# do-mpc/do-mpc

Hardware: AMD Instinct MI355X
Metric: MPC steps/sec (make_step wall-time), industrial_poly robust multi-stage (higher is better)
Workload: dtype f64

## Files before the change

do_mpc_amd/csrc/dompc_driver.h:

```cpp

DOMPC_DEV inline int epsg_off(const KArgs& A) { return A.node_eps_off[0]; }
DOMPC_DEV inline int epsg_n(const KArgs& A) { return A.n_opt_x - A.node_eps_off[0]; }
DOMPC_DEV inline void epsg_grad(const Thr& T, const Prob& Q) {
  const KArgs& A = *Q.A;
  const int o = epsg_off(A), nv = epsg_n(A);
  for (int j = T.tid; j < nv; j += T.nt) {
    double g = 0.0, r = 0.0;
    for (int e = 0; e < A.n_edges; ++e) {
      const int q = j - (A.node_eps_off[A.edge_parent[e]] - o);
      if (q < 0 || q >= NSE) continue;
      g += Q.sf * DOMPC_EPS_PEN[q];
      const double* yd = Q.lam + A.edge_row0[e] + NW + NX;
      for (int i = 0; i < NE; ++i)
        if (nl_slack(i) == q) r -= yd[i] * Q.sgn[e * NE1 + i];
    }
    Q.gf[o + j] = g;
    Q.rd[o + j] = g + r - Q.zl[o + j] + Q.zu[o + j];
  }
  T.sync();
}
DOMPC_DEV inline double epsg_rowsum(const Prob& Q, int j, const double* v, const double* v0) {
  const KArgs& A = *Q.A;
  const int o = epsg_off(A);
  double t = 0.0;
  for (int e = 0; e < A.n_edges; ++e) {
    const int q = j - (A.node_eps_off[A.edge_parent[e]] - o);
    if (q < 0 || q >= NSE) continue;
    const int r0 = A.edge_row0[e] + NW + NX;
    for (int i = 0; i < NE; ++i)
      if (nl_slack(i) == q) t += (v[r0 + i] - (v0 ? v0[r0 + i] : 0.0)) * Q.sgn[e * NE1 + i];
  }
  return t;
}
DOMPC_DEV inline void epsg_residual(const Thr& T, const Prob& Q, const double* v, int j1) {
  const KArgs& A = *Q.A;
  const int o = epsg_off(A);
  for (int e = T.tid; e < A.n_edges; e += T.nt) {
    const int jo = A.node_eps_off[A.edge_parent[e]] - o;
    const int r0 = A.edge_row0[e] + NW + NX;
    for (int i = 0; i < NE; ++i) {
      const int q = nl_slack(i);
      if (q < 0) continue;
      const double ve = v ? v[jo + q] : ((jo + q == j1) ? 1.0 : 0.0);
      Q.c[r0 + i] = Q.ct[r0 + i] - ve * Q.sgn[e * NE1 + i];
    }
  }
  T.sync();
}

DOMPC_DEV inline void solve_problem(const Thr& T, const KArgs& A, int b, int slot) {
  const dompc_options& O = A.opt;
  Prob Q = make_prob(A, slot, A.p + (int64_t)b * A.n_opt_p);
  const double* x0 = A.x0 + (int64_t)b * A.n_opt_x;
  const int nX = A.n_opt_x, nSl = A.n_edges * NE;
  int status = 2, it = 0, n_reg = 0, n_ls_fail = 0, n_sweeps = 0, n_trials = 0, n_soc = 0;

  double cnt[2] = {0.0, 0.0};
  bool singular0;
  {
    double fr[1] = {0.0};
    for (int d = T.tid; d < A.n_dummy; d += T.nt) {
      const int g = A.dummy_idx[d];
      if (!(A.lbx[g] > -INFINITY) && !(A.ubx[g] < INFINITY)) fr[0] += 1.0;
    }
    const int ops[1] = {R_SUM};
    wg_reduce(T, fr, ops);
    singular0 = fr[0] > 0.0;
  }
  for (int g = T.tid; g < nX; g += T.nt) {
    double l = A.lbx[g], u = A.ubx[g];
    if (l > -INFINITY) l -= fmin(O.constr_viol_tol, O.bound_relax_factor * fmax(1.0, fabs(l)));
    if (u < INFINITY) u += fmin(O.constr_viol_tol, O.bound_relax_factor * fmax(1.0, fabs(u)));
    double xv = x0[g];
    const bool hl = l > -INFINITY, hu = u < INFINITY;
    double pl = hl ? O.bound_push * fmax(1.0, fabs(l)) : 0.0;
    double pu = hu ? O.bound_push * fmax(1.0, fabs(u)) : 0.0;
    if (hl && hu) { pl = fmin(pl, O.bound_frac * (u - l)); pu = fmin(pu, O.bound_frac * (u - l)); }
    if (hl) xv = fmax(xv, l + pl);
    if (hu) xv = fmin(xv, u - pu);
    Q.lb_own[g] = l; Q.ub_own[g] = u; Q.x[g] = xv;
    Q.zl[g] = hl ? 1.0 : 0.0; Q.zu[g] = hu ? 1.0 : 0.0;
    if (sh_cnt(A, mk_x(A, g))) cnt[0] += (hl ? 1.0 : 0.0) + (hu ? 1.0 : 0.0);
  }
  for (int r = T.tid; r < A.n_g; r += T.nt) Q.lam[r] = 0.0;
  T.sync();
  for (int d = T.tid; d < A.n_dummy; d += T.nt) {
    const int g = A.dummy_idx[d];
    if (singular0) continue;
    if (sh_cnt(A, mk_x(A, g))) cnt[0] -= (Q.lb_own[g] > -INFINITY ? 1.0 : 0.0) + (Q.ub_own[g] < INFINITY ? 1.0 : 0.0);
    Q.x[g] = fmin(fmax(x0[g], A.lbx[g]), A.ubx[g]);
    Q.lb_own[g] = -INFINITY; Q.ub_own[g] = INFINITY; Q.zl[g] = 0.0; Q.zu[g] = 0.0;
  }
  T.sync();
  if (A.lb_sh) {
    for (int g = T.tid; g < nX; g += T.nt) { A.lb_sh[g] = Q.lb_own[g]; A.ub_sh[g] = Q.ub_own[g]; }
    T.sync();
  }
  auto init_slacks = [&](bool rescale) {
    for (int e = T.tid; e < A.n_edges; e += T.nt) {
      for (int i = 0; i < NE; ++i) { Q.s[e * NE1 + i] = 0.0; if (!rescale) Q.sgn[e * NE1 + i] = 1.0; }
      if (DENSE_EDGE) dae_edge_f(Q, e, Q.x, Q.s, Q.ct); else eval_edge_f(Q, e, Q.x, Q.s, Q.ct);
      for (int i = 0; i < NE; ++i) {
        const int row = A.edge_row0[e] + NW + NX + i, si = e * NE1 + i;
        double l = A.lbg[row], u = A.ubg[row];
        if (l > -INFINITY) l -= fmin(O.constr_viol_tol, O.bound_relax_factor * fmax(1.0, fabs(l)));
        if (u < INFINITY) u += fmin(O.constr_viol_tol, O.bound_relax_factor * fmax(1.0, fabs(u)));
        l *= Q.sgn[si]; u *= Q.sgn[si];
        const bool hl = l > -INFINITY, hu = u < INFINITY;
        double pl = hl ? O.bound_push * fmax(1.0, fabs(l)) : 0.0;
        double pu = hu ? O.bound_push * fmax(1.0, fabs(u)) : 0.0;
        if (hl && hu) { pl = fmin(pl, O.bound_frac * (u - l)); pu = fmin(pu, O.bound_frac * (u - l)); }
        double sv = Q.ct[row];
        if (hl) sv = fmax(sv, l + pl);
        if (hu) sv = fmin(sv, u - pu);
        Q.s[si] = sv; Q.sl[si] = l; Q.su[si] = u;
        Q.zsl[si] = hl ? 1.0 : 0.0; Q.zsu[si] = hu ? 1.0 : 0.0;
        if (!rescale && sh_cnt(A, mk_e(A, e))) cnt[1] += (hl ? 1.0 : 0.0) + (hu ? 1.0 : 0.0);
      }
    }
    T.sync();
  };
  if (NE > 0) init_slacks(false);
  {
    const int ops[2] = {R_SUM, R_SUM};
    wg_reduce(T, cnt, ops);
  }
  const double n_bounds = cnt[0] + cnt[1];
  const double n_dual = (double)(A.n_g - DOMPC_XROW_MASKED) + n_bounds;

  double mu = O.mu_init;
  Q.sf = 1.0;
  long long c_sweep = 0, c_bwd = 0, c_fwd = 0, c_ls = 0, c_meas = 0, c_ftb = 0, c_acc = 0, c_t = 0; const long long c_start = prof_clock();
  unsigned g_sweep = 0, g_bwd = 0, g_fwd = 0, g_ls = 0, g_meas = 0, g_ftb = 0, g_acc = 0, g_t = 0; const unsigned g_start = T.gen;
  if (T.tid == 0) T.fset(6, abort_requested(A));
  auto delta_after = [&](double last) { return last == 0.0 ? O.delta_w_0 : fmax(O.delta_w_min, O.kappa_w_minus * last); };
  const bool ls_init = NE == 0 && O.constr_mult_init_max > 0.0;
  if (ls_init) {
    for (int g = T.tid; g < nX; g += T.nt) {
      if (Q.lb_own[g] > -INFINITY) Q.lb_own[g] = Q.x[g] - 1.0;
      if (Q.ub_own[g] < INFINITY) Q.ub_own[g] = Q.x[g] + 1.0;
      Q.zl[g] = 0.0; Q.zu[g] = 0.0;
    }
    for (int r = T.tid; r < A.n_g; r += T.nt) Q.c[r] = 0.0;
    T.sync();
  }
  auto first_sweep = [&]() {
    ++n_sweeps;
    const int rc = ls_init ? run_sweep(T, Q, b, slot, 1.0, 3, 1.0) : run_sweep(T, Q, b, slot, mu, 0, singular0 ? delta_after(0.0) : 0.0);
    if (EPS_GLOBAL) epsg_grad(T, Q);
    return rc;
  };
  auto epsg_build = [&](double delta) -> int {
    const int o = epsg_off(A), nv = epsg_n(A);
    double* G = Q.gsc;
    for (int g = T.tid; g < A.n_g; g += T.nt) { Q.dlam_e[g] = Q.dlam[g]; Q.ct[g] = Q.c[g]; }
    T.sync();
    int rc = 0;
    for (int j = 0; j < nv && !rc; ++j) {
      epsg_residual(T, Q, nullptr, j);
      ++n_sweeps;
      rc = run_sweep(T, Q, b, slot, mu, 1, delta);
      if (!rc) rc = run_backward(T, Q, b, slot, mu, delta);
      if (!rc) {
        run_forward(T, Q, b, slot, mu, delta);
        for (int jp = T.tid; jp < nv; jp += T.nt) G[jp * NVG_MAX + j] = -epsg_rowsum(Q, jp, Q.dlam, Q.dlam_e);
      }
    }
    epsg_residual(T, Q, nullptr, -1);
    if (T.tid == 0) {
      int ok = rc ? 0 : 1;
      for (int j = 0; j < nv && ok; ++j) {
        const int g = o + j;
        G[j * NVG_MAX + j] += sigma_of(Q.x[g], Q.lb[g], Q.ub[g], Q.zl[g], Q.zu[g]) + delta;
      }
      for (int j = 0; j < nv && ok; ++j) {
        double dj = G[j * NVG_MAX + j];
        for (int k = 0; k < j; ++k) dj -= G[j * NVG_MAX + k] * G[j * NVG_MAX + k];
        if (!(dj > 0.0)) { ok = 0; break; }
        dj = sqrt(dj);
        G[j * NVG_MAX + j] = dj;
        for (int i = j + 1; i < nv; ++i) {
          double t = 0.5 * (G[i * NVG_MAX + j] + G[j * NVG_MAX + i]);
          for (int k = 0; k < j; ++k) t -= G[i * NVG_MAX + k] * G[j * NVG_MAX + k];
          G[i * NVG_MAX + j] = t / dj;
        }
      }
      G[NVG_MAX * NVG_MAX] = ok ? 0.0 : 1.0;
    }
    T.sync();
    return G[NVG_MAX * NVG_MAX] != 0.0;
  };
  auto epsg_apply = [&](double delta, const double* dl) -> int {
    const int o = epsg_off(A), nv = epsg_n(A);
    double* G = Q.gsc;
    double* de = G + NVG_MAX * NVG_MAX + 1;
    for (int j = T.tid; j < nv; j += T.nt) {
      const int g = o + j;
      const double re = Q.rd[g] + Q.zl[g] - Q.zu[g] + bar_grad(Q.x[g], Q.lb[g], Q.ub[g], mu);
      de[j] = -re + epsg_rowsum(Q, j, dl, nullptr);
    }
    for (int g = T.tid; g < A.n_g; g += T.nt) Q.ct[g] = Q.c[g];
    T.sync();
    if (T.tid == 0) {
      for (int i = 0; i < nv; ++i) {
        double t = de[i];
        for (int k = 0; k < i; ++k) t -= G[i * NVG_MAX + k] * de[k];
        de[i] = t / G[i * NVG_MAX + i];
      }
      for (int i = nv - 1; i >= 0; --i) {
        double t = de[i];
        for (int k = i + 1; k < nv; ++k) t -= G[k * NVG_MAX + i] * de[k];
        de[i] = t / G[i * NVG_MAX + i];
      }
    }
    T.sync();
    epsg_residual(T, Q, de, -1);
    ++n_sweeps;
    int rc = run_sweep(T, Q, b, slot, mu, 1, delta);
    if (!rc) rc = run_backward(T, Q, b, slot, mu, delta);
    if (!rc) run_forward(T, Q, b, slot, mu, delta);
    epsg_residual(T, Q, nullptr, -1);
    for (int j = T.tid; j < nv; j += T.nt) Q.dx[o + j] = de[j];
    T.sync();
    return rc;
  };
  int bad = first_sweep();
  if (NE > 0 && O.obj_scaling && !bad) {
    double any[1] = {0.0};
    for (int e = T.tid; e < A.n_edges; e += T.nt) {
      if (!mk_e(A, e)) continue;
      for (int i = 0; i < NE; ++i) {
        double gm = nl_slack(i) >= 0 ? 1.0 : 0.0;
        for (int a = 0; a < NA; ++a) gm = fmax(gm, fabs(Q.EW(e, EW_JD + i * NA + a)));
        if (DENSE_EDGE) for (int c = 0; c < NW; ++c) gm = fmax(gm, fabs(Q.EW(e, EW_JDW + i * NW + c)));
        if (gm > O.nlp_scaling_max_gradient) { Q.sgn[e * NE1 + i] = fmax(O.nlp_scaling_max_gradient / gm, 1e-8); any[0] = 1.0; }
      }
    }
    const int ops[1] = {R_MAX};
    wg_reduce(T, any, ops);
    if (any[0] > 0.0) {
      T.sync();
      init_slacks(true);
      bad = first_sweep();
    }
  }
  if (O.obj_scaling) {
    double gm[1] = {0.0};
    for (int g = T.tid; g < nX; g += T.nt)
      if (sh_cnt(A, mk_x(A, g))) gm[0] = fmax(gm[0], fabs(Q.gf[g]));
    const int ops[1] = {R_MAX};
    wg_reduce(T, gm, ops);
    if (gm[0] > O.nlp_scaling_max_gradient) {
      Q.sf = fmax(O.nlp_scaling_max_gradient / gm[0], 1e-8);
      bad = first_sweep();
    }
  }
  if (ls_init) {
    int ls_bad = bad;
    if (!ls_bad) ls_bad = run_backward(T, Q, b, slot, 1.0, 1.0, 2);
    if (!ls_bad) run_forward(T, Q, b, slot, 1.0, 1.0);
    double ym[1] = {0.0};
    for (int r = T.tid; r < A.n_g; r += T.nt) {
      if (!mk_g(A, r)) continue;
      const double y = Q.dlam[r];
      ym[0] = fmax(ym[0], (y == y) ? fabs(y) : INFINITY);
    }
    {
      const int ops[1] = {R_MAX};
      wg_reduce(T, ym, ops);
// ... 8 lines not shown
      Q.zl[g] = hl ? 1.0 : 0.0; Q.zu[g] = hu ? 1.0 : 0.0;
    }
    T.sync();
    bad = run_sweep(T, Q, b, slot, mu, 0, singular0 ? delta_after(0.0) : 0.0);
    ++n_sweeps;
  }
  const double mu_min = fmin(O.tol, O.compl_inf_tol * Q.sf) / (O.kappa_eps + 1.0);
  double tau = fmax(O.tau_min, 1.0 - mu);
  if (KAPPA_D != 0.0) Q.mu = mu;
  Errs E = measure(T, Q, nullptr);
  const double theta0 = E.theta;
  const double theta_max = 1e4 * fmax(1.0, theta0), theta_min = 1e-4 * fmax(1.0, theta0);
  double bar_sum;
  {
    double bs[1] = {0.0};
    LogAcc La{1.0, 0, 0};
    double lin = 0.0;
    double x_[DOMPC_FW], l_[DOMPC_FW], u2_[DOMPC_FW];
#define L_(u, g) x_[u] = Q.x[g]; l_[u] = Q.lb[g]; u2_[u] = Q.ub[g];
#define B_(u, g)                                                       \
    if (sh_cnt(A, mk_x(A, g))) {                                       \
      if (l_[u] > -INFINITY) logacc_add(La, x_[u] - l_[u]);            \
      if (u2_[u] < INFINITY) logacc_add(La, u2_[u] - x_[u]);           \
      if (KAPPA_D != 0.0) { const double os_ = one_sided(l_[u], u2_[u]); lin += os_ > 0.0 ? x_[u] - l_[u] : (os_ < 0.0 ? u2_[u] - x_[u] : 0.0); } \
    }
    DOMPC_FOR4(nX, L_, B_)
#undef L_
#undef B_
    for (int g = T.tid; g < nSl; g += T.nt) {
      if (!sh_cnt(A, mk_e(A, g / NE1))) continue;
      const int si = (g / NE1) * NE1 + g % NE1;
      if (Q.sl[si] > -INFINITY) logacc_add(La, Q.s[si] - Q.sl[si]);
      if (Q.su[si] < INFINITY) logacc_add(La, Q.su[si] - Q.s[si]);
      if (KAPPA_D != 0.0) { const double os_ = one_sided(Q.sl[si], Q.su[si]); lin += os_ > 0.0 ? Q.s[si] - Q.sl[si] : (os_ < 0.0 ? Q.su[si] - Q.s[si] : 0.0); }
    }
    bs[0] = -logacc_value(La);
    if (KAPPA_D != 0.0) bs[0] += KAPPA_D * lin;
    const int ops[1] = {R_SUM};
    wg_reduce(T, bs, ops);
    bar_sum = bs[0];
  }
  int n_filt = 0;
  double delta_last = 0.0;
  int acc_count = 0;
  const double s_max = 100.0;
  double E0 = 0.0;
  int wd_count = 0, wd_iter = 0, n_watchdog = 0;
  bool in_wd = false, wd_resume = false;
  double wd_theta = 0.0, wd_phi = 0.0, wd_dphi = 0.0, wd_alpha = 0.0, wd_amax = 0.0, wd_az = 0.0, wd_delta = 0.0, wd_delta_last = 0.0, wd_bar = 0.0;
  Errs wd_E = E;
  double delta = 0.0, a_max = 1.0, a_z = 1.0, dphi = 0.0;

  while (true) {
    bool skip_first = false;
    if (wd_resume) {
      for (int g = T.tid; g < nX; g += T.nt) { Q.x[g] = Q.x_wd[g]; Q.zl[g] = Q.zl_wd[g]; Q.zu[g] = Q.zu_wd[g]; Q.dx[g] = Q.dx_sv[g]; }
      for (int g = T.tid; g < A.n_g; g += T.nt) { Q.lam[g] = Q.lam_wd[g]; Q.dlam[g] = Q.dlam_sv[g]; }
      for (int g = T.tid; g < nSl; g += T.nt) { Q.s[g] = Q.s_wd[g]; Q.zsl[g] = Q.zsl_wd[g]; Q.zsu[g] = Q.zsu_wd[g]; Q.ds[g] = Q.ds_sv[g]; }
      T.sync();
      E = wd_E; bar_sum = wd_bar; delta = wd_delta; delta_last = wd_delta_last; a_max = wd_amax; a_z = wd_az; dphi = wd_dphi;
      wd_resume = false;
      skip_first = true;
    } else {
    if (bad) { if (in_wd) { bad = 0; wd_resume = true; in_wd = false; wd_count = 0; continue; } status = 3; break; }
    if (T.fget(6)) { status = 6; break; }
    if (((WIDE_OK && T.nwg > 1) || sh_on(A)) && T.fget(7)) { status = 5; break; }
    const double sd = fmax(s_max, (E.sum_y + E.C.sum_z) / fmax(1.0, n_dual)) / s_max;
    const double sc = fmax(s_max, E.C.sum_z / fmax(1.0, n_bounds)) / s_max;
    const double e_c0 = comp_err(E.C, 0.0);
    E0 = fmax(E.e_d / sd, fmax(E.e_p, e_c0 / sc));
    if (!(E0 == E0) || !(E.obj == E.obj)) { if (in_wd) { wd_resume = true; in_wd = false; wd_count = 0; continue; } status = 4; break; }
    if (E0 <= O.tol && E.e_d <= O.dual_inf_tol && E.e_p <= O.constr_viol_tol && e_c0 <= O.compl_inf_tol) {
      status = 0; break;
    }
    if (E0 <= O.acceptable_tol) {
      if (++acc_count >= O.acceptable_iter) { status = 1; break; }
    } else acc_count = 0;
    if (it >= O.max_iter) { status = 2; break; }

    const double mu_before = mu;
    while (true) {
      const double Emu = fmax(E.e_d / sd, fmax(E.e_p, comp_err(E.C, mu) / sc));
      if (Emu <= O.kappa_eps * mu && mu > mu_min) {
        mu = fmax(mu_min, fmin(O.kappa_mu * mu, pow(mu, O.theta_mu)));
        tau = fmax(O.tau_min, 1.0 - mu);
        n_filt = 0;
        in_wd = false; wd_count = 0;
      } else break;
    }
    if (mu != mu_before) {
      if (QUAD_FWD && forward_adjoint(Q, mu) && !Q.lu_ok) {
        ++n_sweeps;
        if (run_sweep(T, Q, b, slot, mu, 4, Q.dsw)) { if (in_wd) { wd_resume = true; in_wd = false; wd_count = 0; continue; } status = 3; break; }
      } else {
        refresh_mu(T, Q, mu - mu_before);
        Q.rp_mu = mu;
      }
    }

    delta = 0.0;
    bool first_try = true, dir_ok = true, recs_dirty = false;
    while (true) {
      c_t = prof_clock(); g_t = T.gen;
      int fail = (singular0 && delta == 0.0) ? 1 : run_backward(T, Q, b, slot, mu, delta);
      if (EPS_GLOBAL && !fail) {
        run_forward(T, Q, b, slot, mu, delta);
        fail = epsg_build(delta);
        recs_dirty = true;
      }
      c_bwd += prof_clock() - c_t; g_bwd += T.gen - g_t;
      if (!fail) break;
      if (delta == 0.0) {
        delta = delta_after(delta_last);
      } else {
        delta *= (delta_last == 0.0 && first_try) ? O.kappa_w_plus_bar : O.kappa_w_plus;
        first_try = false;
        if (delta > O.delta_w_max) { dir_ok = false; break; }
      }
      if ((NW > 0 && delta != Q.dsw) || (EPS_GLOBAL && recs_dirty)) {
        ++n_sweeps;
        if (run_sweep(T, Q, b, slot, mu, 0, delta)) { dir_ok = false; break; }
        recs_dirty = false;
      }
    }
    if (!dir_ok) { if (in_wd) { wd_resume = true; in_wd = false; wd_count = 0; continue; } status = 3; break; }
    if (delta > 0.0) { delta_last = delta; ++n_reg; }
    c_t = prof_clock(); g_t = T.gen;
    if (EPS_GLOBAL) { if (epsg_apply(delta, Q.dlam_e)) { if (in_wd) { wd_resume = true; in_wd = false; wd_count = 0; continue; } status = 3; break; } }
    else run_forward(T, Q, b, slot, mu, delta);
    c_fwd += prof_clock() - c_t; g_fwd += T.gen - g_t;

    c_t = prof_clock(); g_t = T.gen;
    double r5[5];
    run_step_rules(T, Q, b, slot, mu, r5);
    a_max = (r5[0] > tau) ? tau / r5[0] : 1.0; dphi = r5[2];
    a_z = (r5[1] > tau) ? tau / r5[1] : 1.0;
    c_ftb += prof_clock() - c_t; g_ftb += T.gen - g_t;
    }
    auto step_rules = [&](double (&r5)[5]) { run_step_rules(T, Q, b, slot, mu, r5); };
    const double theta = E.theta;
    const double phi = E.obj + mu * bar_sum;

    c_t = prof_clock(); g_t = T.gen;
    const double gamma_theta = 1e-5, gamma_phi = 1e-8, eta_phi = 1e-8, s_theta = 1.1, s_phi = 2.3, gamma_alpha = 0.05;
    const double kappa_soc = 0.99;
    double a_min;
    if (dphi < 0.0 && theta <= theta_min)
      a_min = (theta > 0.0) ? gamma_alpha * fmin(gamma_theta, fmin(gamma_phi * theta / (-dphi),
                                                                    pow(theta, s_theta) / pow(-dphi, s_phi)))
                            : gamma_alpha * gamma_theta;
    else if (dphi < 0.0) a_min = gamma_alpha * fmin(gamma_theta, gamma_phi * theta / (-dphi));
    else a_min = gamma_alpha * gamma_theta;
    a_min = fmax(a_min, 1e-14);
    auto eval_trial = [&](double al, double& obj_o, double& th_o, double& bar_o) {
      run_eval_trial(T, Q, b, slot, al, obj_o, th_o, bar_o);
      ++n_trials;
    };
    auto acceptable_ref = [&](double th_, double ph_, double al, bool& armijo_case, double theta, double phi, double dphi) -> bool {
      armijo_case = false;
      bool ok = (ph_ == ph_) && (th_ == th_) && fabs(ph_) < INFINITY && th_ <= theta_max;
      if (ok) {
        for (int q = 0; q < n_filt; ++q)
          if (th_ >= T.filt[2 * q] && ph_ >= T.filt[2 * q + 1]) { ok = false; break; }
      }
      if (ok) {
        const bool switching = dphi < 0.0 && al * pow(-dphi, s_phi) > pow(theta, s_theta);
        const double eps_m = 10.0 * 2.220446049250313e-16 * fabs(phi);
        if (theta <= theta_min && switching) {
          armijo_case = true;
          ok = (ph_ - phi - eps_m <= eta_phi * al * dphi);
        } else {
          ok = (th_ <= (1.0 - gamma_theta) * theta) || (ph_ - phi - eps_m <= -gamma_phi * theta);
        }
      }
      return ok;
    };
    auto acceptable = [&](double th_, double ph_, double al, bool& armijo_case) -> bool { return acceptable_ref(th_, ph_, al, armijo_case, theta, phi, dphi); };
    auto soc_residual = [&](double al) {
      double c_[DOMPC_FW], ct_[DOMPC_FW];
#define L_(u, g) c_[u] = Q.c[g]; ct_[u] = Q.ct[g];
#define B_(u, g) if (mk_g(A, g)) Q.c[g] = al * c_[u] + ct_[u];
      DOMPC_FOR4(A.n_g, L_, B_)
#undef L_
#undef B_
      T.sync();
    };
    auto keep_direction = [&](bool restore) {
      for (int g = T.tid; g < nX; g += T.nt) { if (restore) Q.dx[g] = Q.dx_sv[g]; else Q.dx_sv[g] = Q.dx[g]; }
      for (int g = T.tid; g < A.n_g; g += T.nt) { if (restore) Q.dlam[g] = Q.dlam_sv[g]; else Q.dlam_sv[g] = Q.dlam[g]; }
      for (int g = T.tid; g < nSl; g += T.nt) { if (restore) Q.ds[g] = Q.ds_sv[g]; else Q.ds_sv[g] = Q.ds[g]; }
      T.sync();
    };
    double alpha = skip_first ? 0.5 * a_max : a_max;
    bool accepted = false, armijo_used = false, stale = false;
    double th_t = 0.0, obj_t = 0.0, bar_t = bar_sum;
    int n_ls = skip_first ? 1 : 0;
    bool wd_done = false, wd_augment_ref = false, wd_no_augment = false;
    if (O.watchdog_shortened_iter_trigger > 0 && !in_wd && !skip_first && wd_count >= O.watchdog_shortened_iter_trigger) {
      in_wd = true; wd_iter = 0; ++n_watchdog;
      for (int g = T.tid; g < nX; g += T.nt) { Q.x_wd[g] = Q.x[g]; Q.zl_wd[g] = Q.zl[g]; Q.zu_wd[g] = Q.zu[g]; Q.dx_sv[g] = Q.dx[g]; }
      for (int g = T.tid; g < A.n_g; g += T.nt) { Q.lam_wd[g] = Q.lam[g]; Q.dlam_sv[g] = Q.dlam[g]; }
      for (int g = T.tid; g < nSl; g += T.nt) { Q.s_wd[g] = Q.s[g]; Q.zsl_wd[g] = Q.zsl[g]; Q.zsu_wd[g] = Q.zsu[g]; Q.ds_sv[g] = Q.ds[g]; }
      T.sync();
      wd_E = E; wd_bar = bar_sum; wd_delta = delta; wd_delta_last = delta_last; wd_amax = a_max; wd_az = a_z;
      wd_theta = theta; wd_phi = phi; wd_dphi = dphi; wd_alpha = a_max;
    }
    if (in_wd) {
      eval_trial(alpha, obj_t, th_t, bar_t);
      bool armijo_case = false;
      if (acceptable_ref(th_t, obj_t + mu * bar_t, wd_alpha, armijo_case, wd_theta, wd_phi, wd_dphi)) {
        accepted = true; armijo_used = armijo_case; wd_done = true; wd_augment_ref = true;
        in_wd = false; wd_count = 0;
      } else {
        ++wd_iter;
        const double ph_ = obj_t + mu * bar_t;
        if (wd_iter > O.watchdog_trial_iter_max || !(ph_ == ph_) || !(th_t == th_t) || !(fabs(ph_) < INFINITY)) {
          wd_resume = true; in_wd = false; wd_count = 0;
          continue;
        }
        accepted = true; wd_done = true; wd_no_augment = true;
      }
    }
    while (!wd_done) {
      eval_trial(alpha, obj_t, th_t, bar_t);
      stale = false;
      bool armijo_case = false;
      if (acceptable(th_t, obj_t + mu * bar_t, alpha, armijo_case)) { accepted = true; armijo_used = armijo_case; break; }
      if (n_ls == 0 && O.max_soc > 0 && th_t >= theta) {
        double th_old = theta;
        keep_direction(false);
        soc_residual(alpha);
        bool soc_ok = false;
        for (int k = 0; k < O.max_soc; ++k) {
          ++n_soc; ++n_sweeps;
          if (run_sweep(T, Q, b, slot, mu, 1, delta)) break;
          if (run_backward(T, Q, b, slot, mu, delta)) break;
          run_forward(T, Q, b, slot, mu, delta);
          if (EPS_GLOBAL && epsg_apply(delta, Q.dlam)) break;
          double q5[5];
          step_rules(q5);
          const double a_s = (q5[0] > tau) ? tau / q5[0] : 1.0;
          double obj_s = 0.0, th_s = 0.0, bar_s = 0.0;
          eval_trial(a_s, obj_s, th_s, bar_s);
          bool arm_s = false;
          if (acceptable(th_s, obj_s + mu * bar_s, a_s, arm_s)) {
            accepted = true; armijo_used = arm_s; soc_ok = true;
            alpha = a_s;
            a_z = (q5[1] > tau) ? tau / q5[1] : 1.0;
            obj_t = obj_s; th_t = th_s; bar_t = bar_s;
            break;
          }
          if (!(th_s <= kappa_soc * th_old)) break;
          th_old = th_s;
          soc_residual(a_s);
        }
        if (soc_ok) break;
        keep_direction(true);
        stale = true;
      }
      if (!(alpha * 0.5 >= a_min)) break;
      alpha *= 0.5;
      ++n_ls;
    }
    if (bad) { if (in_wd) { bad = 0; wd_resume = true; in_wd = false; wd_count = 0; continue; } status = 3; break; }
    if (!accepted && stale) eval_trial(alpha, obj_t, th_t, bar_t);
    if (!wd_done) wd_count = n_ls > 0 ? wd_count + 1 : 0;
    if (!accepted) {
      ++n_ls_fail;
      n_filt = 0;
    } else if (!armijo_used && !wd_no_augment) {
      if (T.ltid == 0) {
        int q = n_filt < MAX_FILTER ? n_filt : MAX_FILTER - 1;
        T.filt[2 * q] = (1.0 - gamma_theta) * (wd_augment_ref ? wd_theta : theta);
        T.filt[2 * q + 1] = (wd_augment_ref ? wd_phi : phi) - gamma_phi * (wd_augment_ref ? wd_theta : theta);
      }
      if (n_filt < MAX_FILTER) ++n_filt;
      T.lsync();
    }
    bar_sum = bar_t;
    c_ls += prof_clock() - c_t; g_ls += T.gen - g_t;
    c_t = prof_clock(); g_t = T.gen;
    const Comp Cp = run_accept(T, Q, b, slot, alpha, a_z, mu);
    if (A.trace && b == 0 && T.tid == 0 && it < A.trace_cap) {
      double* tr = A.trace + 8 * it;
      tr[0] = it; tr[1] = mu; tr[2] = E0; tr[3] = E.e_p; tr[4] = E.e_d; tr[5] = accepted ? alpha : -alpha;
      tr[6] = delta; tr[7] = E.obj / Q.sf;
    }
    if (T.tid == 0) T.fset(6, abort_requested(A));
    T.sync();
    c_acc += prof_clock() - c_t; g_acc += T.gen - g_t;
    ++it;
    c_t = prof_clock(); g_t = T.gen; bad = run_sweep(T, Q, b, slot, mu, 0, singular0 ? delta_after(delta_last) : 0.0); c_sweep += prof_clock() - c_t; g_sweep += T.gen - g_t;
    ++n_sweeps;
    if (EPS_GLOBAL) epsg_grad(T, Q);
    if (KAPPA_D != 0.0) Q.mu = mu;
    c_t = prof_clock(); g_t = T.gen; E = measure(T, Q, &Cp); c_meas += prof_clock() - c_t; g_meas += T.gen - g_t;
  }

  if (A.trace && b == 0 && T.tid == 0 && A.trace_cap > 8) { double* tr = A.trace + 8 * (A.trace_cap - 1); tr[0] = (double)c_sweep; tr[1] = (double)c_bwd; tr[2] = (double)c_fwd; tr[3] = (double)c_ls; tr[4] = (double)c_meas; tr[5] = (double)(prof_clock() - c_start); tr[6] = (double)c_ftb; tr[7] = (double)c_acc; if (T.prof) { double* t2 = A.trace + 8 * (A.trace_cap - 2); for (int i = 0; i < 8; ++i) t2[i] = (double)T.prof[i]; double* t3 = A.trace + 8 * (A.trace_cap - 3); for (int i = 0; i < 8; ++i) t3[i] = (double)T.prof[8 + i]; double* t4 = A.trace + 8 * (A.trace_cap - 4); for (int i = 0; i < 8; ++i) t4[i] = (double)T.prof[16 + i]; if (A.trace_cap > 12) { double* t5 = A.trace + 8 * (A.trace_cap - 5); for (int i = 0; i < 8; ++i) t5[i] = (double)T.prof[24 + i]; double* t6 = A.trace + 8 * (A.trace_cap - 6); t6[0] = g_sweep; t6[1] = g_bwd; t6[2] = g_fwd; t6[3] = g_ls; t6[4] = g_meas; t6[5] = T.gen - g_start; t6[6] = g_ftb; t6[7] = g_acc; } } }
  const double isf = 1.0 / Q.sf;
  if (A.x_out) for (int g = T.tid; g < nX; g += T.nt) A.x_out[(int64_t)b * nX + g] = sh_cnt(A, mk_x(A, g)) ? Q.x[g] : 0.0;
  if (A.lam_x_out) for (int g = T.tid; g < nX; g += T.nt) A.lam_x_out[(int64_t)b * nX + g] = sh_cnt(A, mk_x(A, g)) ? (Q.zu[g] - Q.zl[g]) * isf : 0.0;
  if (A.lam_g_out) for (int r = T.tid; r < A.n_g; r += T.nt) A.lam_g_out[(int64_t)b * A.n_g + r] = sh_cnt(A, mk_g(A, r)) ? Q.lam[r] * isf : 0.0;
  if (A.lam_g_out && NE > 0) {
    T.sync();
    for (int g = T.tid; g < nSl; g += T.nt) {
      const int e = g / NE1, i = g % NE1;
      if (!sh_cnt(A, mk_e(A, e))) continue;
      const int row = A.edge_row0[e] + NW + NX + i;
      A.lam_g_out[(int64_t)b * A.n_g + row] = Q.lam[row] * Q.sgn[e * NE1 + i] * isf;
    }
  }
  if (A.g_out) {
    for (int r = T.tid; r < A.n_g; r += T.nt) A.g_out[(int64_t)b * A.n_g + r] = sh_cnt(A, mk_g(A, r)) ? Q.c[r] : 0.0;
    T.sync();
    for (int g = T.tid; g < nSl; g += T.nt) {
      const int e = g / NE1, i = g % NE1;
      if (!sh_cnt(A, mk_e(A, e))) continue;
      const int row = A.edge_row0[e] + NW + NX + i;
      A.g_out[(int64_t)b * A.n_g + row] = (Q.c[row] + Q.s[e * NE1 + i]) / Q.sgn[e * NE1 + i];
    }
  }
  if (T.tid == 0) {
    if (A.f_out) A.f_out[b] = E.obj * isf;
    if (A.stats) {
      dompc_stats& S = A.stats[b];
      S.success = (status == 0 || status == 1) ? 1 : 0;
      S.status = status; S.iter_count = it; S.n_reg = n_reg; S.n_ls_fail = n_ls_fail; S.n_sweeps = n_sweeps; S.n_trials = n_trials; S.n_soc = n_soc; S.n_watchdog = n_watchdog; S.reserved0 = 0;
      S.mu = mu; S.obj = E.obj * isf; S.inf_pr = E.e_p; S.inf_du = E.e_d; S.inf_compl = comp_err(E.C, 0.0);
      S.obj_scaling = Q.sf; S.t_wall_total = 0.0;
    }
  }
  T.sync();
}

DOMPC_DEV inline void debug_newton(const Thr& T, const KArgs& A, int b = 0, int slot = 0) {
  const dompc_options& O = A.opt;
  Prob Q = make_prob(A, slot, A.p + (int64_t)b * A.n_opt_p);
  const int nX = A.n_opt_x;
  for (int g = T.tid; g < nX; g += T.nt) {
    Q.x[g] = A.x0[g]; Q.lb[g] = A.lbx[g]; Q.ub[g] = A.ubx[g];
    Q.zl[g] = A.dbg_zl[g]; Q.zu[g] = A.dbg_zu[g];
  }
  for (int r = T.tid; r < A.n_g; r += T.nt) Q.lam[r] = A.dbg_lam[r];
  T.sync();
  if (NE > 0) {
    for (int e = T.tid; e < A.n_edges; e += T.nt) {
      for (int i = 0; i < NE; ++i) { Q.s[e * NE1 + i] = 0.0; Q.sgn[e * NE1 + i] = 1.0; }
      if (DENSE_EDGE) dae_edge_f(Q, e, Q.x, Q.s, Q.ct); else eval_edge_f(Q, e, Q.x, Q.s, Q.ct);
      for (int i = 0; i < NE; ++i) {
        const int row = A.edge_row0[e] + NW + NX + i, si = e * NE1 + i;
        const double l = A.lbg[row], u = A.ubg[row];
        const bool hl = l > -INFINITY, hu = u < INFINITY;
        double pl = hl ? O.bound_push * fmax(1.0, fabs(l)) : 0.0;
        double pu = hu ? O.bound_push * fmax(1.0, fabs(u)) : 0.0;
        if (hl && hu) { pl = fmin(pl, O.bound_frac * (u - l)); pu = fmin(pu, O.bound_frac * (u - l)); }
        double sv = Q.ct[row];
        if (A.dbg_at_solution) {
          const double lr = hl ? l - fmin(O.constr_viol_tol, O.bound_relax_factor * fmax(1.0, fabs(l))) : l;
          const double ur = hu ? u + fmin(O.constr_viol_tol, O.bound_relax_factor * fmax(1.0, fabs(u))) : u;
          const double tiny = 1e-12 * fmax(1.0, fabs(sv));
          if (hl) sv = fmax(sv, lr + tiny);
          if (hu) sv = fmin(sv, ur - tiny);
          Q.s[si] = sv; Q.sl[si] = lr; Q.su[si] = ur;
          Q.zsl[si] = hl ? A.dbg_mu / (sv - lr) : 0.0; Q.zsu[si] = hu ? A.dbg_mu / (ur - sv) : 0.0;
          continue;
        }
        if (hl) sv = fmax(sv, l + pl);
        if (hu) sv = fmin(sv, u - pu);
        Q.s[si] = sv; Q.sl[si] = l; Q.su[si] = u;
        Q.zsl[si] = hl ? 1.0 : 0.0; Q.zsu[si] = hu ? 1.0 : 0.0;
      }
    }
    T.sync();
  }
  Q.sf = 1.0;
  run_sweep(T, Q, b, slot, A.dbg_mu, 0, A.dbg_delta);
  const int fail = run_backward(T, Q, b, slot, A.dbg_mu, A.dbg_delta);
  run_forward(T, Q, b, slot, A.dbg_mu, A.dbg_delta);
  for (int g = T.tid; g < nX; g += T.nt) {
    A.dbg_dx[(int64_t)b * nX + g] = fail ? NAN : Q.dx[g];
    A.dbg_rd[(int64_t)b * nX + g] = Q.rd[g];
  }
  for (int r = T.tid; r < A.n_g; r += T.nt) {
    A.dbg_dlam[(int64_t)b * A.n_g + r] = Q.dlam[r];
    A.dbg_c[(int64_t)b * A.n_g + r] = Q.c[r];
  }
  T.sync();
}

constexpr int SWEEP_BLOCK = NX * NA + NX + NA * NA + NA;

DOMPC_DEV inline void sweep_problem(const Thr& T, const KArgs& A, int b, int slot) {
  Prob Q = make_prob(A, slot, A.p + (int64_t)b * A.n_opt_p);
  const int nX = A.n_opt_x;
  const double* xin = A.sw_x + (int64_t)b * nX;
  const double* lin = A.sw_lam + (int64_t)b * A.n_g;
  for (int g = T.tid; g < nX; g += T.nt) {
    Q.x[g] = xin[g]; Q.lb[g] = -INFINITY; Q.ub[g] = INFINITY; Q.zl[g] = 0.0; Q.zu[g] = 0.0;
  }
  for (int r = T.tid; r < A.n_g; r += T.nt) Q.lam[r] = lin[r];
  for (int g = T.tid; g < A.n_edges * NE; g += T.nt) {
    const int si = (g / NE1) * NE1 + g % NE1;
    Q.s[si] = 0.0; Q.sl[si] = -INFINITY; Q.su[si] = INFINITY; Q.zsl[si] = 0.0; Q.zsu[si] = 0.0; Q.sgn[si] = 1.0;
  }
  T.sync();
  Q.sf = 1.0;
  run_sweep(T, Q, b, slot, 0.0);
  double* gout = A.sw_g + (int64_t)b * A.n_g;
  for (int r = T.tid; r < A.n_g; r += T.nt) gout[r] = Q.c[r];
  double* bl = A.sw_blocks + (int64_t)b * A.n_edges * SWEEP_BLOCK;
  for (int it = T.tid; A.sw_blocks && it < A.n_edges * SWEEP_BLOCK; it += T.nt) {
    const int e = it / SWEEP_BLOCK, i = it % SWEEP_BLOCK;
    const double* S_ = Q.ES(e);
    double v;
    if (i < NX * NA) v = S_[ES_AB + i];
    else if (i < NX * NA + NX) v = S_[ES_CV + i - NX * NA];
    else if (i < NX * NA + NX + NA * NA) v = S_[ES_QT + symi((i - NX * NA - NX) / NA, (i - NX * NA - NX) % NA, NA)];
    else v = S_[ES_QV + i - NX * NA - NX - NA * NA];
    bl[it] = v;
  }
  T.sync();
}
```

do_mpc_amd/csrc/dompc_factor.h:

```cpp

#ifndef DOMPC_HOST_EMU
#ifndef DOMPC_GJ_U
#define DOMPC_GJ_U 0.01
#endif
constexpr int GJ_R = DEG * NX, GJ_RP = ((GJ_R + 3) / 4) * 4, GJ_NRHS = NA + 1;
constexpr int GJ_NC = GJ_RP + GJ_NRHS + GJ_R;
constexpr bool MFMA_GJ = (NI == 1) && (DEG >= 1) && !DENSE_EDGE && (GJ_RP <= 32) && (GJ_NC <= 64);
constexpr int GJ_MT = (GJ_RP + 15) / 16, GJ_NT = (GJ_NC + 15) / 16;
static_assert(!MFMA_GJ || GJ_RP * 4 + 256 <= EL_T1 - EL_MX, "the panel buffer and the dual-residual row share the W | w0 region of the edge working set");

constexpr bool GJ_PACK = (GJ_MT == 2) && (GJ_RP == 20) && (GJ_NT <= 4);
constexpr int GJ_MTF = GJ_PACK ? 1 : GJ_MT;

struct GjCol { int kind, sl, b; };
__device__ inline GjCol gj_col(int ni, int lc) {
  constexpr int R = GJ_R, RP = GJ_RP, NRHS = GJ_NRHS;
  const int col = 16 * ni + lc;
  GjCol c{4, 0, 0};
  if (col < R) { c.kind = 0; c.sl = col / NX; c.b = col - c.sl * NX; }
  else if (col < RP) { c.kind = 4; c.b = col; }
  else if (col < RP + NA) { c.kind = 1; c.b = col - RP; }
  else if (col == RP + NA) { c.kind = 2; }
  else if (col < RP + NRHS + R) { c.kind = 3; c.b = col - (RP + NRHS); }
  return c;
// ... 270 lines not shown
        if (16 * mi + 4 * r < RP) put(16 * mi + 4 * r + lr, ni, T[mi][ni][r]);
    if constexpr (GJ_PACK) put(16 + lr, ni, X[ni]);
  }
  GJ_PH(27)
#undef GJ_PH
  return 0;
}
#else
constexpr bool MFMA_GJ = false;
DOMPC_DEV inline void gj_table_init(ldsd*, int) {}
#endif

constexpr int EF_R = DEG * NX, EF_NCX = 2 * EF_R + NA + 1, EF_CPX = (EF_NCX + GS_C - 1) / GS_C;
template <int MODE>
DOMPC_DEV inline int edge_factor_body(const Prob& Q, int e, double mu, int lane, int GS, ldsd* Ld, const double (&vx)[EF_CPX][5],
                                      const double (&ex)[5], double nu_a) {
  const KArgs& A = *Q.A;
  const int woff = A.edge_w_off[e];
  const double* nu_e = Q.lam + A.edge_row0[e] + NW;
  const double* mo = Q.MO(e);
  (void)mo;
  const ldsd* mol = Ld + EL_MOS;
#define MOV(i) (MO_COMPACT ? (double)mol[(i)] : mo[(i)])
  const bool act = true;
  int fail = 0;
  (void)act;
#if DOMPC_PROFILE && !defined(DOMPC_HOST_EMU)
  const long long pc_ef0 = clock64();
#endif
  constexpr int R = DEG * NX, RA = R > 0 ? R : 1;
  constexpr int NRHS = NA + 1;
  constexpr int NCX = 2 * R + NRHS;
  constexpr int CPX = (NCX + GS_C - 1) / GS_C;
  constexpr double GJ_U = DOMPC_GJ_U;
  double bc[CPX][RA];
  double cd[CPX][DEG > 0 ? DEG : 1];
  unsigned jcol_[CPX];
  auto fetch_cols = [&]() {
#pragma unroll
    for (int q = 0; q < CPX; ++q) {
      const unsigned cx = (unsigned)lane + (unsigned)q * (unsigned)GS;
      const bool isG = cx < (unsigned)R, isY = cx >= (unsigned)R && cx < (unsigned)(R + NA);
      const unsigned jcol = isG ? cx % (unsigned)NX : (isY ? cx - (unsigned)R : 0u);
      const unsigned sl1 = isG ? cx / (unsigned)NX + 1u : 0u;
      jcol_[q] = jcol;
#if !defined(DOMPC_HOST_EMU)
#pragma unroll
      for (int jj = 0; jj < DEG; ++jj) {
        double v = DOMPC_C[jj + 1];
        asm("" : "+v"(v));
#pragma unroll
        for (int s1 = 1; s1 <= DEG; ++s1) {
          double t = DOMPC_C[s1 * (DEG + 1) + jj + 1];
          asm("" : "+v"(t));
          v = (sl1 == (unsigned)s1) ? t : v;
        }
        cd[q][jj] = v;
      }
#else
#pragma unroll
      for (int jj = 0; jj < DEG; ++jj) cd[q][jj] = DOMPC_C[sl1 * (unsigned)(DEG + 1) + (unsigned)(jj + 1)];
#endif
    }
  };
  auto build_cols = [&]() {
#pragma unroll
    for (int q = 0; q < CPX; ++q) {
      const int cx = lane + q * GS;
      const bool isG = cx < R, isY = cx >= R && cx < R + NA, isR = cx == R + NA;
      const int sl = isG ? cx / NX : -1, b = isG ? cx % NX : -1, yb = isY ? cx - R : -1;
      const int unit_row = cx - (R + NRHS);
#pragma unroll
      for (int r = 0; r < R; ++r) {
        const int jj = r / NX, a = r % NX;
        const bool useJ = isG ? (sl == jj) : (isY && yb >= NX);
        const double jv_ = MOV((unsigned)(MO_PT + (r / NX) * PT_STRIDE + NX + (r % NX) * NA) + jcol_[q]);
        double v = useJ ? jv_ : 0.0;
        v -= (a == b) ? cd[q][jj] : 0.0;
        v -= (a == yb) ? DOMPC_C[0 * (DEG + 1) + (jj + 1)] : 0.0;
        v = (unit_row == r) ? 1.0 : v;
        bc[q][r] = v;
      }
      if (isR) {
#pragma unroll
        for (int r = 0; r < R; ++r) bc[q][r] = Ld[EL_T1 + r];
      }
    }
  };
  auto eliminate = [&](bool pivoting) -> int {
    int badl = 0;
#pragma unroll
    for (int kk = 0; kk < R; ++kk) {
      const int qk = kk / GS_C, lk = kk % GS_C;
      if (pivoting) {
        int pr = kk;
        double best = fabs(bc[qk][kk]);
#pragma unroll
        for (int r = kk + 1; r < R; ++r) {
          const double a = fabs(bc[qk][r]);
          if (a > best) { best = a; pr = r; }
        }
        if (lane == lk && !(best > 1e-300)) badl = 1;
#ifndef DOMPC_HOST_EMU
        pr = __builtin_amdgcn_readlane(pr, lk);
#endif
#pragma unroll
        for (int q = 0; q < CPX; ++q) {
          const double t = bc[q][kk];
          double nk = t;
#pragma unroll
          for (int r = kk + 1; r < R; ++r) {
            const bool hit = (r == pr);
            nk = hit ? bc[q][r] : nk;
            bc[q][r] = hit ? t : bc[q][r];
          }
          bc[q][kk] = nk;
        }
      } else {
        double m = 0.0;
#pragma unroll
        for (int r = kk + 1; r < R; ++r) m = fmax(m, fabs(bc[qk][r]));
        const double akk = fabs(bc[qk][kk]);
        if (lane == lk && !(akk >= GJ_U * m && akk > 1e-300)) badl = 1;
      }
      double f[RA];
#pragma unroll
      for (int r = 0; r < R; ++r) f[r] = lane_bcast(bc[qk][r], lk);
      const double pinv = fast_rcp((fabs(f[kk]) > 1e-300) ? f[kk] : 1.0);
#pragma unroll
      for (int q = 0; q < CPX; ++q) {
        const double prow = bc[q][kk] * pinv;
#pragma unroll
        for (int r = 0; r < R; ++r)
          if (r != kk) bc[q][r] = fma(-f[r], prow, bc[q][r]);
        bc[q][kk] = prow;
      }
    }
#ifndef DOMPC_HOST_EMU
    return __ballot(badl) != 0ull;
#else
    return badl;
#endif
  };
  if (MODE != 1) fetch_cols();
  auto dual_pieces = [&](auto col_dot) {
#pragma unroll
    for (int q = 0; q < CPX; ++q) {
      const int cx = lane + q * GS;
      double t = col_dot(q, cx);
      if (cx < R) {
        t -= DOMPC_D[cx / NX + 1] * Ld[EL_T0 + R + cx % NX];
        const int gi = woff + cx;
        const double xv = vx[q][0], l = vx[q][1], u = vx[q][2], zl_ = vx[q][3], zu_ = vx[q][4];
        Q.gf[gi] = 0.0;
        Q.rd[gi] = t - zl_ + zu_;
        Ld[EL_RW + cx] = t + bar_grad(xv, l, u, mu, !(Q.soc & 2));
        Ld[EL_BB + cx] = bar_grad(xv, l, u, 1.0);
        Ld[EL_SG + cx] = sigma_of(xv, l, u, zl_, zu_);
      } else if (cx < R + NA) {
        const int yb = cx - R;
        if (yb < NX) t -= DOMPC_D[0] * Ld[EL_T0 + R + yb];
        Ld[EL_RY + yb] = t;
      }
    }
    for (int a = lane; a < NX; a += GS) {
      const int col = R + a, gi = woff + col;
      const double t = Ld[EL_T0 + R + a] + (GS > 1 ? nu_a : nu_e[a]);
      double xv, l, u, zl_, zu_;
      if (GS > 1) { xv = ex[0]; l = ex[1]; u = ex[2]; zl_ = ex[3]; zu_ = ex[4]; }
      else { xv = Q.x[gi]; l = Q.lb[gi]; u = Q.ub[gi]; zl_ = Q.zl[gi]; zu_ = Q.zu[gi]; }
      Q.gf[gi] = 0.0;
      Q.rd[gi] = t - zl_ + zu_;
      Ld[EL_RW + col] = t + bar_grad(xv, l, u, mu, !(Q.soc & 2));
      Ld[EL_BB + col] = bar_grad(xv, l, u, 1.0);
      Ld[EL_SG + col] = sigma_of(xv, l, u, zl_, zu_);
    }
  };
  if (act && MODE == 0) {
    build_cols();
    dual_pieces([&](int q, int) {
      double t = 0.0;
#pragma unroll
      for (int r = 0; r < R; ++r) t += bc[q][r] * Ld[EL_T0 + r];
      return t;
    });
  }
#ifndef DOMPC_HOST_EMU
  if constexpr (MODE == 1) {
    __builtin_amdgcn_fence(__ATOMIC_ACQ_REL, "wavefront");
    __builtin_amdgcn_wave_barrier();
    if (edge_factor_mfma(Q, e, lane, Ld, [&](const ldsd* du) {
          dual_pieces([&](int, int cx) {
            const int c_ = cx < R ? cx : (cx < R + NA ? GJ_RP + (cx - R) : 0);
            return (double)du[c_] + (double)du[64 + c_] + (double)du[128 + c_] + (double)du[192 + c_];
          });
        })) return 2;
    {
      __builtin_amdgcn_fence(__ATOMIC_ACQ_REL, "wavefront");
      __builtin_amdgcn_wave_barrier();
      for (int it = lane; it < NX * NRHS; it += GS) {
        const int a_ = it / NRHS, c = it % NRHS;
        double t = (c == NA) ? -Ld[EL_T1 + R + a_] : ((c == a_) ? DOMPC_D[0] : 0.0);
#pragma unroll
        for (int s_ = 1; s_ <= DEG; ++s_) t += DOMPC_D[s_] * Ld[EL_MX + ((s_ - 1) * NX + a_) * MX_LD + MX_W + c];
        Ld[EL_MX + (R + a_) * MX_LD + MX_W + c] = t;
      }
      return 0;
    }
  } else if constexpr (MODE == 2) {
    build_cols();
    if (eliminate(true)) fail = 1;
  } else
#endif
  if (act) {
    if (eliminate(false)) {
      fetch_cols();
      build_cols();
      if (eliminate(true)) fail = 1;
    }
  }
  if (act) {
#pragma unroll
    for (int q = 0; q < CPX; ++q) {
      const int cx = lane + q * GS;
      if (cx >= R && cx < R + NRHS) {
        const int col = MX_W + (cx - R);
#pragma unroll
        for (int a_ = 0; a_ < NX; ++a_) {
          const int yb = cx - R;
          double t = (yb == NA) ? Ld[EL_T1 + R + a_] : ((yb == a_) ? -DOMPC_D[0] : 0.0);
#pragma unroll
          for (int r = 1; r <= DEG; ++r) t += DOMPC_D[r] * bc[q][(r - 1) * NX + a_];
          Ld[EL_MX + (R + a_) * MX_LD + col] = -t;
        }
#pragma unroll
        for (int r = 0; r < R; ++r) Ld[EL_MX + r * MX_LD + col] = -bc[q][r];
      } else if (cx >= R + NRHS && cx < NCX) {
        const int col = cx - (R + NRHS);
#pragma unroll
        for (int r = 0; r < R; ++r) Q.EW(e, EW_LU + r * LU_N + col) = bc[q][r];
      }
    }
  }
#undef MOV
  return fail;
}

#ifndef DOMPC_HOST_EMU
__device__ inline KArgs kernel_args(const void* kp);
#define DOMPC_EF_ARGS const void* kp, int slot, int e, int soc, double sf, double mu, double v0, double v1, double v2, double v3, double v4, \
                      double x0, double x1, double x2, double x3, double x4, double nu_a
#define DOMPC_EF_BODY(MODE_)                                                                                     \
  const KArgs A = kernel_args(kp);                                                                               \
  Prob Q = make_prob(A, __builtin_amdgcn_readfirstlane(slot), nullptr);                                          \
  Q.sf = ufl(sf);                                                                                                \
  Q.soc = __builtin_amdgcn_readfirstlane(soc);                                                                   \
  prob_bounds(Q);                                                                                                \
  const int lane = (int)(threadIdx.x & 63u);                                                                     \
  ldsd* Ld = (ldsd*)lds_pool + (int64_t)(threadIdx.x >> 6) * EL_SIZE;                                            \
  const double vx[EF_CPX][5] = {{v0, v1, v2, v3, v4}};                                                           \
  const double ex[5] = {x0, x1, x2, x3, x4};                                                                     \
  return edge_factor_body<MODE_>(Q, __builtin_amdgcn_readfirstlane(e), ufl(mu), lane, 64, Ld, vx, ex, nu_a);
__device__ __attribute__((noinline)) int phase_edge_factor(DOMPC_EF_ARGS) { DOMPC_EF_BODY(MFMA_GJ ? 1 : 0) }
__device__ __attribute__((noinline)) int phase_edge_factor_pivot(DOMPC_EF_ARGS) { DOMPC_EF_BODY(MFMA_GJ ? 2 : 0) }
#undef DOMPC_EF_BODY
#undef DOMPC_EF_ARGS
#endif
DOMPC_DEV inline int run_edge_factor(const Thr& T, const Prob& Q, int e, double mu, int lane, int GS, ldsd* Ld,
                                     const double (&vx)[EF_CPX][5], const double (&ex)[5], double nu_a) {
#ifndef DOMPC_HOST_EMU
  if constexpr (EF_CPX == 1) {
    (void)lane; (void)GS; (void)Ld;
    int rc = phase_edge_factor(T.kp, Q.slot, e, Q.soc, Q.sf, mu, vx[0][0], vx[0][1], vx[0][2], vx[0][3], vx[0][4],
                               ex[0], ex[1], ex[2], ex[3], ex[4], nu_a);
    if (MFMA_GJ && __builtin_amdgcn_readfirstlane(rc) == 2)
      rc = phase_edge_factor_pivot(T.kp, Q.slot, e, Q.soc, Q.sf, mu, vx[0][0], vx[0][1], vx[0][2], vx[0][3], vx[0][4],
                                   ex[0], ex[1], ex[2], ex[3], ex[4], nu_a);
    return rc;
  } else {
    return edge_factor_body<0>(Q, e, mu, lane, GS, Ld, vx, ex, nu_a);
  }
#else
  (void)T;
  return edge_factor_body<0>(Q, e, mu, lane, GS, Ld, vx, ex, nu_a);
#endif
}

#ifndef DOMPC_HOST_EMU
__device__ inline void stage_mo(const Prob& Q, int e, int lane, ldsd* Ld) {
  const double* src = Q.MO(e);
#pragma unroll
  for (int q = 0; q < MOC_STAGE / 128; ++q)
    __builtin_amdgcn_global_load_lds((const __attribute__((address_space(1))) void*)(src + 128 * q + 2 * lane),
                                     (__attribute__((address_space(3))) void*)(Ld + EL_MOC + 128 * q), 16, 0, 0);
}
#endif

DOMPC_PHASE int eval_edge_coop(const Thr& T, const Prob& Q, int e, int e_next, double mu, int lane, int GS, ldsd* Ld, int& staged_e, const MocMap& mm) {
  const KArgs& A = *Q.A;
  const bool act = e >= 0;
  const int ee = act ? e : 0;
  const auto* ep = A.edge_pack + ee * EP_N;
  const int n = ep[EP_PARENT], cn = ep[EP_CHILD], k = ep[EP_LEVEL];
  const double* xn = Q.x + ep[EP_XOFF_PARENT];
  const double* un = Q.x + ep[EP_UOFF_PARENT];
  const double* xc = Q.x + ep[EP_XOFF_CHILD];
  const int woff = ep[EP_WOFF];
  const int eps_off_n = ep[EP_EPSOFF_PARENT];
  const double* pp = Q.P + A.p_off_p + ep[EP_PIDX] * NP;
  const int row0 = ep[EP_ROW0];
  const double om = __builtin_bit_cast(double, ((unsigned long long)(unsigned)ep[EP_OMEGA_HI] << 32) | (unsigned long long)(unsigned)ep[EP_OMEGA_LO]) * Q.sf;
  (void)eps_off_n;
  const double* w = Q.x + woff;
  const double* tvp = Q.P + A.p_off_tvp + k * NTVP;
  const double omh = (Q.soc & 2) ? 0.0 : om;
  const double* lam_e = Q.lam + row0;
  const double* nu_e = Q.lam + row0 + NW;
  const double* yd = Q.lam + row0 + NW + NX;
  double* S_ = Q.ES(ee);
  const double* mo = Q.MO(ee);
  int fail = 0;
  constexpr bool PF = (NI == 1 && M > 0);
  constexpr int RPL = PF ? (NW + GS_C - 1) / GS_C : 1;
  constexpr int APL = PF ? (NA + GS_C - 1) / GS_C : 1, MHL = PF ? (NX * NX + GS_C - 1) / GS_C : 1;
// ... 112 lines not shown
        }
#endif
      }
      DOMPC_PH(4)
      if (act) {
        if constexpr (!TILE_CONDENSE)
          for (int it = lane; it < NCOLL * NA * NA; it += GS)
            Ld[EL_HP + it] = MOV(MO_PT + (it / (NA * NA)) * PT_STRIDE + NX + NX * NA + symi((it % (NA * NA)) / NA, it % NA, NA));
#pragma unroll
        for (int q = 0; q < RPL; ++q) {
          const int it = lane + q * GS;
          if (it < NW) {
            const int jj = it / NX;
            double res;
            if (jj < DEG) {
              const int j = jj + 1;
              double xp = DOMPC_C[0 * (DEG + 1) + j] * pf_xn[q];
#pragma unroll
              for (int r = 1; r <= DEG; ++r) xp += DOMPC_C[r * (DEG + 1) + j] * pf_w[q][r - 1];
              res = MOV(MO_PT + jj * PT_STRIDE + it % NX) - xp;
            } else {
              double xf = DOMPC_D[0] * pf_xn[q];
#pragma unroll
              for (int r = 1; r <= DEG; ++r) xf += DOMPC_D[r] * pf_w[q][r - 1];
              res = pf_wend[q] - xf;
            }
            if (Q.soc) res = pf_c[q];
            else Q.c[row0 + it] = res;
            Ld[EL_T1 + it] = res;
            Ld[EL_T0 + it] = pf_lam[q];
          }
          if (it < NX) {
            const double ce = Q.soc ? pf_cend[q] : pf_wend[q] - pf_xc[q];
            if (!Q.soc) Q.c[row0 + NW + it] = ce;
            Ld[EL_PV + it] = ce;
          }
        }
      }
      DOMPC_PH(5)
      T.gsync();
      DOMPC_PH(6)
      if (act) fail |= run_edge_factor(T, Q, e, mu, lane, GS, Ld, vx, ex, nu_a);
      T.gsync();
#ifndef DOMPC_HOST_EMU
      if (MO_LDS && e_next >= 0) { stage_mo(Q, e_next, lane, Ld); staged_e = e_next; }
#endif
    } else {
    if (act) {
#pragma unroll
      for (int q = 0; q < G_WPL; ++q) {
        const int col = lane + q * GS, gi = woff + (col < NW ? col : 0);
        gp_x[q] = Q.x[gi]; gp_l[q] = Q.lb[gi]; gp_u[q] = Q.ub[gi]; gp_zl[q] = Q.zl[gi]; gp_zu[q] = Q.zu[gi];
      }
#pragma unroll
      for (int q = 0; q < G_XPL; ++q) {
        const int a = lane + q * GS, ac = a < NX ? a : 0;
        gp_ce[q] = Q.soc ? Q.c[row0 + NW + ac] : w[(M - 1) * NX + ac] - xc[ac];
        gp_mg[q] = last_stage ? mo[MO_MT + 1 + ac] : 0.0;
      }
#pragma unroll
      for (int q = 0; q < G_CVL; ++q) {
        const int it = lane + q * GS, a = (it < NX * (NA + 1) ? it : 0) / (NA + 1);
        gp_cv[q] = Q.soc ? Q.c[row0 + NW + a] : w[(M - 1) * NX + a] - xc[a];
      }
#pragma unroll
      for (int q = 0; q < G_APL; ++q) {
        const int a = lane + q * GS;
        gp_ltg[q] = mo[MO_LT + 1 + (a < NA ? a : 0)];
      }
#pragma unroll
      for (int q = 0; q < G_MHL; ++q) {
        const int a = lane + q * GS, ac = a < NX * NX ? a : 0;
        gp_mh[q] = last_stage ? mo[MO_MT + 1 + NX + symi(ac / NX, ac % NX, NX)] : 0.0;
      }
#pragma unroll
      for (int q = 0; q < G_QPL; ++q) {
        const int it = lane + q * GS, itc = it < NA * NA ? it : 0;
        const int ip = symi(itc / NA, itc % NA, NA);
        gp_qlt[q] = mo[MO_LT + 1 + NA + ip];
        gp_qnl[q] = NE > 0 ? mo[MO_NL + NE + NE * NA + ip] : 0.0;
      }
      gp_lt0 = mo[MO_LT];
      gp_mt0 = last_stage ? mo[MO_MT] : 0.0;
    }
    if (act) {
      for (int it = lane; it < NCOLL * NA * NA; it += GS)
        Ld[EL_HP + it] = mo[MO_PT + (it / (NA * NA)) * PT_STRIDE + NX + NX * NA + symi((it % (NA * NA)) / NA, it % NA, NA)];
#pragma unroll
      for (int q2 = 0; q2 < G_RWL; ++q2) {
        const int it = lane + q2 * GS;
        gp_res[q2] = 0.0;
        if (it >= G_ROWS) continue;
        const int i = it / ((DEG + 1) * NX);
        const int rr = it % ((DEG + 1) * NX);
        const int jj = rr / NX, a = rr % NX;
        const double* xi0 = (i == 0) ? xn : w + slot_of(i, 0) * NX;
        const int row = i * (DEG + 1) * NX + jj * NX + a;
        ldsd* Mr = Ld + EL_MX + row * NC;
        if (jj < DEG) {
          const int j = jj + 1, sl = slot_of(i, j), p = i * DEG + jj;
          const double* pt = mo + MO_PT + p * PT_STRIDE;
          double xp = DOMPC_C[0 * (DEG + 1) + j] * xi0[a];
          for (int r = 1; r <= DEG; ++r) xp += DOMPC_C[r * (DEG + 1) + j] * w[slot_of(i, r) * NX + a];
          const double res = Q.soc ? Q.c[row0 + row] : pt[a] - xp;
          gp_res[q2] = res;
          Mr[NW + NA] = res;
          for (int b = 0; b < NX; ++b) Mr[sl * NX + b] += pt[NX + a * NA + b];
          for (int b = 0; b < NU; ++b) Mr[NW + NX + b] = pt[NX + a * NA + NX + b];
          for (int r = 0; r <= DEG; ++r) {
            const double cr = DOMPC_C[r * (DEG + 1) + j];
            if (i == 0 && r == 0) Mr[NW + a] -= cr;
            else Mr[slot_of(i, r) * NX + a] -= cr;
          }
        } else {
          const int ns_ = next_slot(i);
          double xf = DOMPC_D[0] * xi0[a];
          for (int r = 1; r <= DEG; ++r) xf += DOMPC_D[r] * w[slot_of(i, r) * NX + a];
          const double res = Q.soc ? Q.c[row0 + row] : w[ns_ * NX + a] - xf;
          gp_res[q2] = res;
          Mr[NW + NA] = res;
          Mr[ns_ * NX + a] += 1.0;
          for (int r = 0; r <= DEG; ++r) {
            if (i == 0 && r == 0) Mr[NW + a] -= DOMPC_D[0];
            else Mr[slot_of(i, r) * NX + a] -= DOMPC_D[r];
          }
        }
      }
    }
    T.gsync();
    if (act) {
#pragma unroll
      for (int q = 0; q < G_WPL; ++q) {
        const int col = lane + q * GS;
        if (col >= NW) continue;
        double t = 0.0;
#pragma unroll 6
        for (int r = 0; r < NW; ++r) t += Ld[EL_MX + r * NC + col] * Ld[EL_T0 + r];
        if (col >= (M - 1) * NX) t += nu_e[col - (M - 1) * NX];
        const double xv = gp_x[q], l = gp_l[q], u = gp_u[q];
        gp_x[q] = t - gp_zl[q] + gp_zu[q];
        Ld[EL_RW + col] = t + bar_grad(xv, l, u, mu, !(Q.soc & 2));
        Ld[EL_BB + col] = bar_grad(xv, l, u, 1.0);
        Ld[EL_SG + col] = sigma_of(xv, l, u, gp_zl[q], gp_zu[q]);
      }
      for (int b = lane; b < NA; b += GS) {
        double t = 0.0;
#pragma unroll 6
        for (int r = 0; r < NW; ++r) t += Ld[EL_MX + r * NC + NW + b] * Ld[EL_T0 + r];
        Ld[EL_RY + b] = t;
      }
#pragma unroll
      for (int q = 0; q < G_WPL; ++q) {
        const int col = lane + q * GS;
        if (col < NW) { Q.gf[woff + col] = 0.0; Q.rd[woff + col] = gp_x[q]; }
      }
      if (!Q.soc) {
#pragma unroll
        for (int q2 = 0; q2 < G_RWL; ++q2) {
          const int it = lane + q2 * GS;
          if (it < G_ROWS) Q.c[row0 + it] = gp_res[q2];
        }
#pragma unroll
        for (int q = 0; q < G_XPL; ++q) {
          const int a = lane + q * GS;
          if (a < NX) Q.c[row0 + NW + a] = gp_ce[q];
        }
      }
    }
    T.gsync();
    DOMPC_PH(1)
    bool gj_done = false;
#ifndef DOMPC_HOST_EMU
#ifndef DOMPC_REG_GJ
#define DOMPC_REG_GJ 1
#endif
    if constexpr ((DOMPC_REG_GJ != 0) && NC <= 64 && NW <= 40 && NW > NX) {
      if (GS == 64) {
        constexpr int GJ_STEPS = NW - NX;
        constexpr int EL_ROWS = (DEG + 1) * NX;
        const int cc_ = lane < NC ? lane : 0;
        double col[NW1];
#pragma unroll
        for (int r = 0; r < NW; ++r) col[r] = act ? Ld[EL_MX + r * NC + cc_] : 1.0;
        int bad = 0;
#pragma unroll
        for (int kk = 0; kk < GJ_STEPS; ++kk) {
          const int pos = kk % EL_ROWS;
          const int grp0 = kk - pos + (pos < DEG * NX ? 0 : DEG * NX);
          const int grp1 = kk - pos + (pos < DEG * NX ? DEG * NX : EL_ROWS);
          const int hi_ = pos < DEG * NX ? kk - pos + EL_ROWS : (kk - pos + 2 * EL_ROWS < NW ? kk - pos + 2 * EL_ROWS : NW);
          double f[NW1];
#pragma unroll
          for (int r = 0; r < NW; ++r) f[r] = (r >= grp0 && r < hi_) ? lane_bcast(col[r], kk) : 0.0;
          double m = 0.0;
#pragma unroll
          for (int r = 0; r < NW; ++r) if (r > kk && r < grp1) m = fmax(m, fabs(f[r]));
          const double akk = fabs(f[kk]);
          bad |= (int)!(akk >= DOMPC_GJ_U * m && akk > 1e-300);
          const double pinv = fast_rcp(akk > 1e-300 ? f[kk] : 1.0);
          const bool own = lane == kk;
          const double prow = own ? pinv : col[kk] * pinv;
#pragma unroll
          for (int r = 0; r < NW; ++r) if (r >= grp0 && r < hi_ && r != kk) col[r] = fma(-f[r], prow, own ? 0.0 : col[r]);
          col[kk] = prow;
        }
        if (!act) bad = 0;
        if (__builtin_amdgcn_readfirstlane(bad) == 0) {
          if (act && lane < NC) {
#pragma unroll
            for (int r = 0; r < NW; ++r) Ld[EL_MX + r * NC + lane] = col[r];
          }
          T.gsync();
          gj_done = true;
        }
      }
    }
#endif
    if (!gj_done) {
      static_assert(NW <= 128, "row index is packed into 7 bits of the pivot key / 128-bit used mask");
      constexpr int GJ_STEPS = NW - NX;
      constexpr int EL_ROWS = (DEG + 1) * NX;
      constexpr int CPL = (NC + GS_C - 1) / GS_C;
      unsigned long long used = 0ull, used_hi = 0ull;
      {
        for (int kk = 0; kk < GJ_STEPS; ++kk) {
          const int pos = kk % EL_ROWS;
          const int grp0 = kk - pos + (pos < DEG * NX ? 0 : DEG * NX);
          const int grp1 = kk - pos + (pos < DEG * NX ? DEG * NX : EL_ROWS);
          double f[NW1], bcol[CPL][NW1];
          unsigned bestkey = 0u;
          if (act) {
  #pragma unroll
            for (int r = 0; r < NW; ++r) f[r] = Ld[EL_MX + r * NC + kk];
  #pragma unroll
            for (int q = 0; q < CPL; ++q) {
              const int c = lane + q * GS;
              const int cc_ = c < NC ? c : 0;
  #pragma unroll
              for (int r = 0; r < NW; ++r) bcol[q][r] = Ld[EL_MX + r * NC + cc_];
            }
  #pragma unroll
            for (int r = 0; r < NW; ++r) {
              unsigned key = (((unsigned)(__builtin_bit_cast(unsigned long long, f[r]) >> 32)) & (NW > 64 ? 0x7fffff80u : 0x7fffffc0u)) | (unsigned)r;
              const bool taken = (r < 64) ? ((used >> (r & 63)) & 1ull) : ((used_hi >> (r & 63)) & 1ull);
              key = (r >= grp0 && r < grp1 && !taken) ? key : 0u;
              bestkey = key > bestkey ? key : bestkey;
            }
          }
          const int pv = (int)(bestkey & (NW > 64 ? 127u : 63u));
          if (pv < 64) used |= (1ull << pv); else used_hi |= (1ull << (pv - 64));
          if (act && (bestkey >> (NW > 64 ? 7 : 6)) == 0u) fail = 1;
          if (act) {
            if (lane == 0) Ld[EL_PV + kk] = (double)pv;
            const double piv = Ld[EL_MX + pv * NC + kk];
            const double pinv = (fabs(piv) > 1e-300) ? 1.0 / piv : 1.0;
  #pragma unroll
            for (int q = 0; q < CPL; ++q) {
              const int c = lane + q * GS;
              if (c < NC) {
                const double prow = (c == kk) ? pinv : Ld[EL_MX + pv * NC + c] * pinv;
                const double keep = (c == kk) ? 0.0 : 1.0;
  #pragma unroll
                for (int r = 0; r < NW; ++r) Ld[EL_MX + r * NC + c] = fma(-f[r], prow, bcol[q][r] * keep);
                Ld[EL_MX + pv * NC + c] = prow;
              }
            }
          }
          T.gsync();
        }
      }
      double tmp[CPL][NW1];
      if (act) {
        for (int k2 = GJ_STEPS + lane; k2 < NW; k2 += GS) Ld[EL_PV + k2] = (double)k2;
#pragma unroll
        for (int q = 0; q < CPL; ++q) {
          const int c = lane + q * GS;
          const int cc_ = c < NC ? c : 0;
#pragma unroll
          for (int r = 0; r < NW; ++r) tmp[q][r] = Ld[EL_MX + r * NC + cc_];
        }
      }
      T.gsync();
      if (act)
        for (int k2 = lane; k2 < NW; k2 += GS) Ld[EL_T0 + (int)Ld[EL_PV + k2]] = (double)k2;
      T.gsync();
      if (act) {
#pragma unroll
        for (int q = 0; q < CPL; ++q) {
          const int c = lane + q * GS;
          if (c < NC) {
            const int dst = (c < NW) ? (int)Ld[EL_PV + c] : c;
#pragma unroll
            for (int r = 0; r < NW; ++r) Ld[EL_MX + (int)Ld[EL_T0 + r] * NC + dst] = tmp[q][r];
          }
        }
      }
      T.gsync();
    }
    if (act) {
      for (int it = lane; it < NW * (NA + 1); it += GS) {
        const int r = it / (NA + 1), c = it % (NA + 1);
        Ld[EL_MX + r * NC + NW + c] = -Ld[EL_MX + r * NC + NW + c];
      }
    }
    T.gsync();
    }
    DOMPC_PH(2)
// ... 335 lines not shown
```

do_mpc_amd/csrc/dompc_kernel.h:

```cpp
#pragma once
#include <math.h>
#include <stdint.h>
#ifndef DOMPC_HOST_EMU
#include <utility>
#endif
#include "dompc_kargs.h"

namespace dompc {

#ifndef DOMPC_HOST_EMU
#define DOMPC_PHASE __device__ inline
#else
#define DOMPC_PHASE static inline
#endif

constexpr int NX = DOMPC_NX, NU = DOMPC_NU, NP = DOMPC_NP, NTVP = DOMPC_NTVP;
#ifndef DOMPC_EPS_GLOBAL
#define DOMPC_EPS_GLOBAL 0
#endif
constexpr bool EPS_GLOBAL = DOMPC_EPS_GLOBAL != 0 && DOMPC_NS > 0 && DOMPC_NE > 0;
constexpr int NS = EPS_GLOBAL ? 0 : DOMPC_NS;
constexpr int NSE = DOMPC_NS;
constexpr int NVG_MAX = 32;
constexpr int NZ = DOMPC_NZ;
constexpr int DEG = DOMPC_DEG, NI = DOMPC_NI, M = DOMPC_M;
#ifndef DOMPC_NL_COLLOC
#define DOMPC_NL_COLLOC 0
#endif
#ifndef DOMPC_FREE_ROOT
#define DOMPC_FREE_ROOT 0
#endif
#ifndef DOMPC_LT_END
#define DOMPC_LT_END 0
#endif
#ifndef DOMPC_NL_DUP
#define DOMPC_NL_DUP 0
#endif
#if !DOMPC_FREE_ROOT
DOMPC_FN double dompc_aterm_f(const double*, const double*, const double*, const double*) { return 0.0; }
DOMPC_FN void dompc_aterm(const double*, const double*, const double*, const double*, double*, double*, double*) {}
#endif
constexpr bool FREE_ROOT = DOMPC_FREE_ROOT != 0, LT_END = DOMPC_LT_END != 0 && M > 0;
constexpr int NEB = DOMPC_NE;
constexpr int NLP = (DOMPC_NL_COLLOC && M > 0) ? M : 1;
constexpr bool NL_DUP = DOMPC_NL_DUP != 0 && NEB > 0;
constexpr int NLB = NLP + (NL_DUP ? 1 : 0);
constexpr int NE = NEB * NLB;
constexpr bool NL_COLLOC = DOMPC_NL_COLLOC && M > 0 && NEB > 0;
DOMPC_HD constexpr int nl_pt(int blk) { return blk < NLP ? blk : NLP - 1; }
#ifndef DOMPC_FORCE_DENSE
#define DOMPC_FORCE_DENSE 0
#endif
constexpr bool DENSE_EDGE = DOMPC_NZ > 0 || NL_COLLOC || NL_DUP || LT_END || DOMPC_FORCE_DENSE;
DOMPC_HD inline int nl_slack(int i) { return DOMPC_NL_SLACK[NLB == 1 ? i : i % NEB]; }
constexpr int NA = NX + NU;
constexpr int NV = NU + NS;
constexpr int NYT = NA + NV;
constexpr int MZ = NZ > 0 ? (M > 0 ? M : 1) : 0;
constexpr int NWX = M * NX;
constexpr int NW = NWX + MZ * NZ;
constexpr bool RT_CUSTOM = DOMPC_RTERM_CUSTOM != 0;
constexpr int NR = NA + NU, NR_T = NR * (NR + 1) / 2;
constexpr int RT_LEN = RT_CUSTOM ? 1 + NR + NR_T : 0;
constexpr int NF = NX + NZ;
constexpr int NAV = NA + NZ;
constexpr int NCOLL = NI * DEG;
constexpr int RPE = NW + NX + NE;
constexpr int NE1 = NE > 0 ? NE : 1, NEB1 = NEB > 0 ? NEB : 1;
constexpr int NS1 = NS > 0 ? NS : 1;
constexpr int NW1 = NW > 0 ? NW : 1;
constexpr int MAX_FILTER = 48;
#ifndef DOMPC_SHARD
#define DOMPC_SHARD 0
#endif
#ifndef DOMPC_GJ_U
#define DOMPC_GJ_U 0.01
#endif
constexpr int RED_MAX = 12;
#ifndef DOMPC_HOST_EMU
constexpr int GS_C = 64;
#else
constexpr int GS_C = 1;
#endif

constexpr int LU_N = (NI == 1 && DEG > 0 && !DENSE_EDGE) ? DEG * NX : NW;
constexpr int EW_LU = 0;
constexpr int EW_SIGW = EW_LU + LU_N * LU_N;
constexpr int EW_RW = EW_SIGW + NW;
constexpr int EW_JD = EW_RW + NW;
constexpr int EW_W = EW_JD + NE * NA;
constexpr int EW_W0 = EW_W + (DENSE_EDGE ? NW * NA : 0);
constexpr int EW_HW = EW_W0 + (DENSE_EDGE ? NW : 0);
constexpr int EW_EWJ = EW_HW + (DENSE_EDGE ? NW * (NW + NA) : 0);
constexpr int EW_JDW = EW_EWJ + (DENSE_EDGE ? NX * NW : 0);
constexpr int EW_SIZE = ((EW_JDW + (DENSE_EDGE ? NE * NW : 0) + 1 + 7) / 8) * 8;

constexpr int ES_AB = 0;
constexpr int ES_CV = ES_AB + NX * NA;
constexpr int ES_QT = ES_CV + NX;
constexpr int ES_QV = ES_QT + NA * (NA + 1) / 2;
constexpr int ES_RY = ES_QV + NA;
constexpr int ES_GFY = ES_RY + NA;
constexpr int ES_QVB = ES_GFY + NA;
constexpr int ES_MG = ES_QVB + NA;
constexpr int ES_MH = ES_MG + NX;
constexpr int ES_SIGS = ES_MH + NX * NX;
constexpr int ES_RDN = ES_SIGS + NE;
constexpr int ES_RSN = ES_RDN + NE;
constexpr int ES_OBJ = ES_RSN + NE;
constexpr int ES_RTUP = ES_OBJ + 1;
constexpr int ES_RTH = ES_RTUP + (RT_CUSTOM ? NU : 0);
constexpr int ES_SIZE = ((ES_RTH + (RT_CUSTOM ? NR_T : 0) + 7) / 8) * 8;

constexpr int NA_T = NA * (NA + 1) / 2, NX_T = NX * (NX + 1) / 2, NAV_T = NAV * (NAV + 1) / 2;
DOMPC_HD constexpr int symi(int i, int j, int n) { return i <= j ? i * n - i * (i - 1) / 2 + j - i : j * n - j * (j - 1) / 2 + i - j; }
constexpr int PT_STRIDE = NF + NF * NAV + NAV_T;
constexpr int NPT_E = (M == 0) ? 1 : (DENSE_EDGE ? NI * (DEG + 1) : NI * DEG);
constexpr int MO_PT = 0;
constexpr int MO_LT = MO_PT + NPT_E * PT_STRIDE;
constexpr int MO_MT = MO_LT + 1 + NAV + NAV_T;
constexpr int MO_NL = MO_MT + 1 + NX + NX_T;
constexpr int NL_STRIDE = NEB + NEB * NAV + NAV_T;
constexpr int MO_SIZE = ((MO_NL + NLB * NL_STRIDE + 7) / 8) * 8;
constexpr bool MO_COMPACT = (NI == 1) && (M > 0) && !DENSE_EDGE;
constexpr int MOC_LT = NCOLL * DOMPC_DYN_NV;
constexpr int MOC_MT = MOC_LT + DOMPC_LT_NV;
constexpr int MOC_NL = MOC_MT + DOMPC_MT_NV;
constexpr int MOC_N = MOC_NL + DOMPC_NL_NV;
constexpr int MOC_SIZE = ((MOC_N + 7) / 8) * 8 > 0 ? ((MOC_N + 7) / 8) * 8 : 8;
constexpr int MO_REC = MO_COMPACT ? MOC_SIZE : MO_SIZE;

constexpr int ND_P = 0;
constexpr int ND_PV = ND_P + NA * NA;
constexpr int ND_K = ND_PV + NA;
constexpr int ND_KV = ND_K + NV * NA;
constexpr int ND_DXT = ND_KV + NV;
constexpr int ND_AT = ND_DXT + NA;
constexpr int AT_LEN = FREE_ROOT ? 1 + NX + NX * NX : 0;
constexpr int ND_SIZE = ((ND_AT + AT_LEN + 7) / 8) * 8;

struct WsLayout {
  int64_t x, zl, zu, lb, ub, dx, gf, rd, xt, dx_sv;
  int64_t lam, dlam, c, ct, dlam_sv;
  int64_t s, zsl, zsu, sl, su, ds, st, ds_sv;
  int64_t ew, es, nd, mo, gsc, total;
  int64_t x_wd, zl_wd, zu_wd, lam_wd, s_wd, zsl_wd, zsu_wd, dlam_e, sgn;
};

DOMPC_HD inline WsLayout ws_layout(int n_opt_x, int n_g, int n_edges, int e_pad, int n_nodes) {
  WsLayout L;
  int64_t o = 0;
  auto take = [&](int64_t n) { int64_t r = o; o += (n + 7) & ~int64_t(7); return r; };
  L.x = take(n_opt_x); L.zl = take(n_opt_x); L.zu = take(n_opt_x); L.lb = take(n_opt_x); L.ub = take(n_opt_x);
  L.dx = take(n_opt_x); L.gf = take(n_opt_x); L.rd = take(n_opt_x); L.xt = take(n_opt_x);
  L.dx_sv = take(n_opt_x);
  L.lam = take(n_g); L.dlam = take(n_g); L.c = take(n_g); L.ct = take(n_g); L.dlam_sv = take(n_g);
  int64_t nsl = (int64_t)n_edges * NE1;
  L.s = take(nsl); L.zsl = take(nsl); L.zsu = take(nsl); L.sl = take(nsl); L.su = take(nsl);
  L.ds = take(nsl); L.st = take(nsl); L.ds_sv = take(nsl);
  L.ew = take((int64_t)EW_SIZE * e_pad);
  L.es = take((int64_t)ES_SIZE * n_edges);
  L.nd = take((int64_t)ND_SIZE * n_nodes);
  L.mo = take((int64_t)MO_REC * n_edges);
  L.gsc = take(EPS_GLOBAL ? NVG_MAX * (NVG_MAX + 4) : 0);
  L.x_wd = take(n_opt_x); L.zl_wd = take(n_opt_x); L.zu_wd = take(n_opt_x); L.lam_wd = take(n_g);
  L.s_wd = take(nsl); L.zsl_wd = take(nsl); L.zsu_wd = take(nsl);
  L.dlam_e = take(EPS_GLOBAL ? n_g : 0);
  L.sgn = take(nsl);
  o += 256;
  L.total = o;
  return L;
}

#ifndef DOMPC_HOST_EMU
typedef __attribute__((address_space(3))) double ldsd;
#else
typedef double ldsd;
#endif

struct XCtx {
  int on, rank, world;
  double* xbuf;
  volatile uint32_t *req, *ack, *cnt;
  void (*cb)(void* ctx, double* buf, int32_t count);
  void* ctx;
};
DOMPC_HD inline XCtx make_xctx(const KArgs& A) {
  XCtx X;
  X.on = A.x_mask != nullptr; X.rank = A.shard_rank; X.world = A.shard_world; X.xbuf = A.xbuf;
  X.req = A.x_req; X.ack = A.x_ack; X.cnt = A.x_count; X.cb = A.x_callback; X.ctx = A.x_ctx;
  return X;
}

#ifndef DOMPC_NO_WIDE
#define DOMPC_NO_WIDE 0
#endif
constexpr bool WIDE_OK = DOMPC_NO_WIDE == 0;
#ifndef DOMPC_BLOCK_CONST
#define DOMPC_BLOCK_CONST 0
#endif
#if DOMPC_BLOCK_CONST
#define DOMPC_BDIM DOMPC_BLOCK_CONST
#else
#define DOMPC_BDIM ((int)blockDim.x)
#endif
struct Thr {
  int tid, nt;
  ldsd* red;
  ldsd* filt;
  int* flags;
  ldsd* edge_lds;
  long long* prof;
  int gs;
  int ltid, lnt;
  int wg, nwg;
  unsigned* bar;
  double* partials;
  mutable unsigned gen, nred;
  XCtx X;
  mutable unsigned xseq;
  const void* kp;
  mutable bool light = false;
  int pool = 0;
  DOMPC_DEV void fset(int i, int v) const {
#ifndef DOMPC_HOST_EMU
    if (WIDE_OK && nwg > 1) { __hip_atomic_store(flags + i, v, __ATOMIC_RELAXED, __HIP_MEMORY_SCOPE_AGENT); return; }
#endif
    flags[i] = v;
  }
  DOMPC_DEV int fget(int i) const {
#ifndef DOMPC_HOST_EMU
    if (WIDE_OK && nwg > 1) return __hip_atomic_load(flags + i, __ATOMIC_RELAXED, __HIP_MEMORY_SCOPE_AGENT);
#endif
    return flags[i];
  }
  DOMPC_DEV int flag_begin(int i) const {
    sync();
#ifndef DOMPC_HOST_EMU
    if (WIDE_OK && nwg > 1) return (int)(gen & 0x3fffffffu) + 1;
#endif
    if (tid == 0) fset(i, 0);
    sync();
    return 1;
  }
  DOMPC_DEV void sync() const {
#ifndef DOMPC_HOST_EMU
    if (WIDE_OK && nwg > 1) {
      asm volatile("s_waitcnt vmcnt(0)" ::: "memory");
      __syncthreads();
      ++gen;
      if (ltid == 0) {
        if (!light) __builtin_amdgcn_fence(__ATOMIC_RELEASE, "agent");
        asm volatile("s_waitcnt vmcnt(0)" ::: "memory");
        __hip_atomic_fetch_add(bar, 1u, __ATOMIC_RELAXED, __HIP_MEMORY_SCOPE_AGENT);
        const unsigned target = gen * (unsigned)nwg;
        long long spins = 0;
        while (__hip_atomic_load(bar, __ATOMIC_RELAXED, __HIP_MEMORY_SCOPE_AGENT) < target) {
          __builtin_amdgcn_s_sleep(4);
          if (++spins > 40000000ll || __hip_atomic_load(flags + 7, __ATOMIC_RELAXED, __HIP_MEMORY_SCOPE_AGENT)) {
            __hip_atomic_store(flags + 7, 1, __ATOMIC_RELAXED, __HIP_MEMORY_SCOPE_AGENT);
            break;
          }
        }
        __builtin_amdgcn_fence(__ATOMIC_ACQUIRE, "agent");
      }
      __syncthreads();
    } else {
      __syncthreads();
    }
#endif
  }
  DOMPC_DEV void lsync() const {
#ifndef DOMPC_HOST_EMU
    __syncthreads();
#endif
  }
  DOMPC_DEV void gsync() const {
#ifndef DOMPC_HOST_EMU
    __builtin_amdgcn_fence(__ATOMIC_ACQ_REL, "wavefront");
    __builtin_amdgcn_wave_barrier();
#endif
  }
  DOMPC_DEV void xchg(int off, int n) const {
#ifdef DOMPC_HOST_EMU
    if (X.cb) X.cb(X.ctx, X.xbuf + off, n);
#else
    sync();
    ++xseq;
    if (wg == 0 && ltid == 0) {
      __builtin_amdgcn_fence(__ATOMIC_RELEASE, "");
      X.cnt[0] = (unsigned)n;
      X.cnt[1] = (unsigned)off;
      __hip_atomic_store((unsigned*)X.req, xseq, __ATOMIC_RELEASE, __HIP_MEMORY_SCOPE_SYSTEM);
      long long spins = 0;
      const bool dead = __hip_atomic_load(flags + 7, __ATOMIC_RELAXED, __HIP_MEMORY_SCOPE_AGENT) != 0;
      while (!dead && __hip_atomic_load((unsigned*)X.ack, __ATOMIC_RELAXED, __HIP_MEMORY_SCOPE_SYSTEM) != xseq) {
        __builtin_amdgcn_s_sleep(16);
        if (++spins > 4000000ll) {
          __hip_atomic_store(flags + 7, 1, __ATOMIC_RELAXED, __HIP_MEMORY_SCOPE_AGENT);
          break;
        }
      }
      __builtin_amdgcn_fence(__ATOMIC_ACQUIRE, "");
    }
    sync();
#endif
  }
};

#ifndef DOMPC_HOST_EMU
extern __shared__ double lds_pool[];
__shared__ double lds_filt[2 * MAX_FILTER];
__shared__ int lds_flags[8];
__shared__ int lds_b;
#ifndef DOMPC_PROFILE
#define DOMPC_PROFILE 0
#endif
__shared__ long long lds_prof[32];

__device__ inline int slot_of_block(const KArgs& A) {
  const bool wide = (A.mode == 0 && A.wide > 1);
// ... 31 lines not shown
__device__ inline int ufl(int v) { return __builtin_amdgcn_readfirstlane(v); }
__device__ inline unsigned ufl(unsigned v) { return (unsigned)__builtin_amdgcn_readfirstlane((int)v); }
__device__ inline double ufl(double v) {
  const unsigned long long u = __builtin_bit_cast(unsigned long long, v);
  const unsigned lo = ufl((unsigned)u), hi = ufl((unsigned)(u >> 32));
  return __builtin_bit_cast(double, ((unsigned long long)hi << 32) | (unsigned long long)lo);
}
typedef const __attribute__((address_space(4))) KArgs* KArgsCP;
__device__ inline KArgs kernel_args(const void* kp) {
  const unsigned long long u = (unsigned long long)kp;
  const unsigned lo = ufl((unsigned)u), hi = ufl((unsigned)(u >> 32));
  return *(KArgsCP)(((unsigned long long)hi << 32) | (unsigned long long)lo);
}
#endif

constexpr bool SHARD = DOMPC_SHARD != 0;
DOMPC_DEV inline bool sh_on(const KArgs& A) { return SHARD && A.x_mask != nullptr; }
DOMPC_DEV inline int mk_x(const KArgs& A, int g) { return (SHARD && A.x_mask) ? A.x_mask[g] : 1; }
DOMPC_DEV inline int mk_g(const KArgs& A, int r) { return (SHARD && A.g_mask) ? A.g_mask[r] : 1; }
DOMPC_DEV inline int mk_e(const KArgs& A, int e) { return (SHARD && A.e_mask) ? A.e_mask[e] : 1; }
DOMPC_DEV inline int mk_n(const KArgs& A, int n) { return (SHARD && A.n_mask) ? A.n_mask[n] : 1; }
DOMPC_DEV inline bool sh_cnt(const KArgs& A, int m) { return !SHARD || m == 1 || (m == 2 && A.shard_rank == 0); }
DOMPC_DEV inline int cut_of(const KArgs& A, int n) { return (SHARD && A.node_cut) ? A.node_cut[n] : -1; }


DOMPC_DEV inline long long prof_clock() {
#ifndef DOMPC_HOST_EMU
  return (long long)clock64();
#else
  return 0;
#endif
}

DOMPC_DEV inline int abort_requested(const KArgs& A) {
#ifndef DOMPC_HOST_EMU
  return A.abort_flag ? __hip_atomic_load(A.abort_flag, __ATOMIC_RELAXED, __HIP_MEMORY_SCOPE_SYSTEM) : 0;
#else
  return A.abort_flag ? *(const volatile int32_t*)A.abort_flag : 0;
#endif
}

enum RedOp { R_SUM = 0, R_MAX = 1, R_MIN = 2 };

template <int N_>
DOMPC_DEV void wg_reduce(const Thr& T, double (&v)[N_], const int (&op)[N_]) {
  static_assert(N_ <= RED_MAX, "too many values");
  if (T.nt == 1 && !(SHARD && T.X.on)) return;
  for (int i = 0; i < N_; ++i) T.red[i * T.lnt + T.ltid] = v[i];
  T.lsync();
  for (int s = T.lnt >> 1; s > 0; s >>= 1) {
    if (T.ltid < s) {
      for (int i = 0; i < N_; ++i) {
        double a = T.red[i * T.lnt + T.ltid], b = T.red[i * T.lnt + T.ltid + s];
        T.red[i * T.lnt + T.ltid] = op[i] == R_SUM ? a + b : (op[i] == R_MAX ? fmax(a, b) : fmin(a, b));
      }
    }
    T.lsync();
  }
  if (T.nwg > 1) {
    double* buf = T.partials + (T.nred & 1u) * T.nwg * RED_MAX;
    ++T.nred;
    if (T.ltid < N_) buf[T.wg * RED_MAX + T.ltid] = T.red[T.ltid * T.lnt];
    T.sync();
#ifndef DOMPC_HOST_EMU
    const int n_tab = T.nwg * RED_MAX;
    ldsd* tab = T.red + RED_MAX * T.lnt;
    const bool staged = RED_MAX * T.lnt + n_tab <= T.pool;
    if (staged) {
      for (int i = T.ltid; i < n_tab; i += T.lnt) tab[i] = buf[i];
      T.lsync();
    }
#else
    const bool staged = false;
    const double* tab = nullptr;
#endif
    if (T.ltid < N_) {
      double acc = staged ? (double)tab[T.ltid] : buf[T.ltid];
      for (int w = 1; w < T.nwg; ++w) {
        const double b = staged ? (double)tab[w * RED_MAX + T.ltid] : buf[w * RED_MAX + T.ltid];
        acc = op[T.ltid] == R_SUM ? acc + b : (op[T.ltid] == R_MAX ? fmax(acc, b) : fmin(acc, b));
      }
      T.red[T.ltid * T.lnt] = acc;
    }
    T.lsync();
  }
  if (SHARD && T.X.on) {
    const int W = T.X.world, me = T.X.rank;
    double* xb = T.X.xbuf;
    if (T.wg == 0)
      for (int i = T.ltid; i < W * RED_MAX; i += T.lnt) {
        const int w = i / RED_MAX, j = i % RED_MAX;
        xb[i] = (w == me && j < N_) ? T.red[j * T.lnt] : 0.0;
      }
    T.xchg(0, W * RED_MAX);
    for (int i = T.ltid; i < N_; i += T.lnt) {
      double acc = xb[i];
      for (int w = 1; w < W; ++w) {
        const double b = xb[w * RED_MAX + i];
        acc = op[i] == R_SUM ? acc + b : (op[i] == R_MAX ? fmax(acc, b) : fmin(acc, b));
      }
      T.red[i * T.lnt] = acc;
    }
    T.lsync();
  }
  for (int i = 0; i < N_; ++i) v[i] = T.red[i * T.lnt];
  T.lsync();
}

DOMPC_DEV inline void gmm(int lane, int GS, int m, int n, int k, const double* A, int sai, int sal,
                          const double* B, int sbl, int sbj, double beta, double* D, int ldd) {
#ifndef DOMPC_HOST_EMU
  typedef double d4 __attribute__((ext_vector_type(4)));
  (void)GS;
  const int li = lane & 15, lk = lane >> 4;
  for (int ti = 0; ti < m; ti += 16)
    for (int tj = 0; tj < n; tj += 16) {
      d4 acc = {0.0, 0.0, 0.0, 0.0};
      const int ai = ti + li, bj = tj + li;
      for (int kb = 0; kb < k; kb += 4) {
        const int kk = kb + lk;
        const double a = (ai < m && kk < k) ? A[ai * sai + kk * sal] : 0.0;
        const double b = (bj < n && kk < k) ? B[kk * sbl + bj * sbj] : 0.0;
        acc = __builtin_amdgcn_mfma_f64_16x16x4f64(a, b, acc, 0, 0, 0);
      }
      const int col = tj + li;
#pragma unroll
      for (int r = 0; r < 4; ++r) {
        const int row = ti + lk + 4 * r;
        if (row < m && col < n) {
          double* d = D + row * ldd + col;
          *d = (beta == 0.0) ? acc[r] : beta * (*d) + acc[r];
        }
      }
    }
#else
  for (int it = lane; it < m * n; it += GS) {
    const int i = it / n, j = it % n;
    double t = 0.0;
    for (int l = 0; l < k; ++l) t += A[i * sai + l * sal] * B[l * sbl + j * sbj];
    D[i * ldd + j] = (beta == 0.0) ? t : beta * D[i * ldd + j] + t;
  }
#endif
}

struct Prob {
  const KArgs* A;
  const double* P;
  double *x, *zl, *zu, *lb, *ub, *dx, *gf, *rd, *xt, *dx_sv;
  double *lb_own, *ub_own;
  double *lam, *dlam, *c, *ct, *dlam_sv;
  double *s, *zsl, *zsu, *sl, *su, *ds, *st, *ds_sv;
  double *ew, *es, *nd, *mo, *gsc;
  double *x_wd, *zl_wd, *zu_wd, *lam_wd, *s_wd, *zsl_wd, *zsu_wd, *dlam_e, *sgn;
  int e_pad;
  double sf;
  double mu;
  int soc;
  double dsw;
  int slot;
  int rp_soc; double rp_mu;
  int lu_ok;
  DOMPC_DEV double& EW(int e, int i) const { return ew[(int64_t)e * EW_SIZE + i]; }
  DOMPC_DEV double* ES(int e) const { return es + (int64_t)e * ES_SIZE; }
  DOMPC_DEV double* ND(int n) const { return nd + (int64_t)n * ND_SIZE; }
  DOMPC_DEV double* MO(int e) const { return mo + (int64_t)e * MO_REC; }
};

DOMPC_DEV inline Prob make_prob(const KArgs& A, int slot, const double* P) {
  WsLayout L = ws_layout(A.n_opt_x, A.n_g, A.n_edges, A.e_pad, A.n_nodes);
  double* w = A.ws + (int64_t)slot * A.ws_stride;
  Prob p;
  p.A = &A; p.P = P;
  p.x = w + L.x; p.zl = w + L.zl; p.zu = w + L.zu; p.lb_own = w + L.lb; p.ub_own = w + L.ub; p.dx = w + L.dx;
  p.lb = A.lb_sh ? A.lb_sh : p.lb_own; p.ub = A.ub_sh ? A.ub_sh : p.ub_own;
  p.gf = w + L.gf; p.rd = w + L.rd; p.xt = w + L.xt; p.dx_sv = w + L.dx_sv;
  p.lam = w + L.lam; p.dlam = w + L.dlam; p.c = w + L.c; p.ct = w + L.ct; p.dlam_sv = w + L.dlam_sv;
  p.s = w + L.s; p.zsl = w + L.zsl; p.zsu = w + L.zsu; p.sl = w + L.sl; p.su = w + L.su;
  p.ds = w + L.ds; p.st = w + L.st; p.ds_sv = w + L.ds_sv;
  p.ew = w + L.ew; p.es = w + L.es; p.nd = w + L.nd; p.mo = w + L.mo; p.gsc = w + L.gsc;
  p.x_wd = w + L.x_wd; p.zl_wd = w + L.zl_wd; p.zu_wd = w + L.zu_wd; p.lam_wd = w + L.lam_wd;
  p.s_wd = w + L.s_wd; p.zsl_wd = w + L.zsl_wd; p.zsu_wd = w + L.zsu_wd; p.dlam_e = w + L.dlam_e; p.sgn = w + L.sgn;
  p.e_pad = A.e_pad; p.sf = 1.0; p.mu = 0.0; p.soc = 0; p.dsw = 0.0; p.slot = slot; p.lu_ok = 1; p.rp_soc = 0; p.rp_mu = 0.0;
  return p;
}
DOMPC_DEV inline void prob_bounds(Prob& Q) {
  const KArgs& A = *Q.A;
  const bool own = (Q.soc & 2) != 0 || !A.lb_sh;
  Q.lb = own ? Q.lb_own : A.lb_sh;
  Q.ub = own ? Q.ub_own : A.ub_sh;
}

DOMPC_DEV constexpr int slot_of(int i, int r) { return i == 0 ? r - 1 : DEG + (i - 1) * (DEG + 1) + r; }
DOMPC_DEV constexpr int next_slot(int i) { return (i + 1 < NI) ? slot_of(i + 1, 0) : M - 1; }

DOMPC_DEV inline int group_index(int tid, int gs) {
#ifndef DOMPC_HOST_EMU
  return __builtin_amdgcn_readfirstlane(tid / gs);
#else
  return tid / gs;
#endif
}

DOMPC_DEV inline double ldoff(const double* base, unsigned idx) {
#ifndef DOMPC_HOST_EMU
  return *(const double*)((const char*)base + (idx << 3));
#else
  return base[idx];
#endif
}

template <int N>
DOMPC_DEV inline double tab_sel(const double (&tab)[N], int idx, int first = 0, int count = N) {
#ifndef DOMPC_HOST_EMU
  double v = tab[first];
  asm("" : "+v"(v));
#pragma unroll
  for (int i = 1; i < N; ++i) {
    if (i < count) {
      double t = tab[first + i];
      asm("" : "+v"(t));
      v = (idx == first + i) ? t : v;
    }
  }
  return v;
#else
  (void)first; (void)count;
  return tab[idx];
#endif
}

DOMPC_DEV inline double fast_rcp(double x) {
#ifndef DOMPC_HOST_EMU
  double r = __builtin_amdgcn_rcp(x);
  r = fma(fma(-x, r, 1.0), r, r);
  r = fma(fma(-x, r, 1.0), r, r);
  return r;
#else
  return 1.0 / x;
#endif
}

#ifndef DOMPC_KAPPA_D
#define DOMPC_KAPPA_D 1e-5
#endif
constexpr double KAPPA_D = DOMPC_KAPPA_D;
DOMPC_DEV inline double one_sided(double l, double u) {
  const bool hl = l > -INFINITY, hu = u < INFINITY;
  return (hl && !hu) ? 1.0 : ((hu && !hl) ? -1.0 : 0.0);
}
DOMPC_DEV inline double bar_grad(double x, double l, double u, double mu, bool damp = true) {
  double g = 0.0;
  if (l > -INFINITY) g -= mu * fast_rcp(x - l);
  if (u < INFINITY) g += mu * fast_rcp(u - x);
  if (KAPPA_D != 0.0 && damp) g += KAPPA_D * mu * one_sided(l, u);
  return g;
}
DOMPC_DEV inline double sigma_of(double x, double l, double u, double zl, double zu) {
  double sg = 0.0;
  if (l > -INFINITY) sg += zl * fast_rcp(x - l);
  if (u < INFINITY) sg += zu * fast_rcp(u - x);
  return sg;
}

DOMPC_DEV inline double edge_rterm_f(const Prob& Q, int e, const double* xv);
DOMPC_DEV inline void edge_rterm_eval(const Prob& Q, int e, ldsd* dst);
DOMPC_DEV inline void edge_rterm_store(const ldsd* src, double* S_, int lane, int GS);
#ifndef DOMPC_XTRA
#define DOMPC_XTRA 0
#endif
#ifndef DOMPC_XTRA_EW
#define DOMPC_XTRA_EW 0
#endif
#ifndef DOMPC_XROW
#define DOMPC_XROW 0
#define DOMPC_XROW_MASKED 0
#endif
DOMPC_DEV inline void nlcons_f_e(const Prob& Q, int e, const double* xs, const double* us, const double* zs, const double* tvp, const double* pp, double* d) {
  dompc_nlcons_f(xs, us, zs, tvp, pp, d);
#if DOMPC_XROW
  for (int r = 0; r < DOMPC_XROW_SLOTS; ++r) d[DOMPC_XROW_BASE + r] += dompc_xrow_f(DOMPC_XROW_ID[e * DOMPC_XROW_SLOTS + r], xs, us, Q.P);
#endif
  (void)e; (void)Q;
}
DOMPC_DEV inline void nlcons_e(const Prob& Q, int e, const double* xs, const double* us, const double* zs, const double* tvp, const double* pp,
                               const double* lam, double* d, double* Jd, double* H) {
  dompc_nlcons(xs, us, zs, tvp, pp, lam, d, Jd, H);
#if DOMPC_XROW
  for (int r = 0; r < DOMPC_XROW_SLOTS; ++r) dompc_xrow(DOMPC_XROW_ID[e * DOMPC_XROW_SLOTS + r], xs, us, Q.P, lam, d, Jd, H);
#endif
  (void)e; (void)Q;
}
DOMPC_DEV inline double lterm_f_e(const Prob& Q, int e, const double* xs, const double* us, const double* zs, const double* tvp, const double* pp) {
  double v = dompc_lterm_f(xs, us, zs, tvp, pp);
#if DOMPC_XTRA
  v += dompc_xtra_lt_f(DOMPC_XTRA_LT_ID[e], xs, us, Q.P);
#endif
  (void)e; (void)Q;
  return v;
}
DOMPC_DEV inline double mterm_f_e(const Prob& Q, int e, const double* xs, const double* tvp, const double* pp) {
  double v = dompc_mterm_f(xs, tvp, pp);
#if DOMPC_XTRA
  v += dompc_xtra_mt_f(DOMPC_XTRA_MT_ID[e], xs, Q.P);
#endif
  (void)e; (void)Q;
  return v;
}
DOMPC_DEV inline void lterm_e(const Prob& Q, int e, const double* xs, const double* us, const double* zs, const double* tvp, const double* pp,
                              double* val, double* g, double* H) {
  dompc_lterm(xs, us, zs, tvp, pp, val, g, H);
#if DOMPC_XTRA
  dompc_xtra_lt(DOMPC_XTRA_LT_ID[e], xs, us, Q.P, val, g, H);
#endif
  (void)e; (void)Q;
}
DOMPC_DEV inline void mterm_e(const Prob& Q, int e, const double* xs, const double* tvp, const double* pp, double* val, double* g, double* H) {
  dompc_mterm(xs, tvp, pp, val, g, H);
#if DOMPC_XTRA
  dompc_xtra_mt(DOMPC_XTRA_MT_ID[e], xs, Q.P, val, g, H);
#endif
  (void)e; (void)Q;
}

#include "dompc_dae.h"

#include "dompc_edge.h"
#include "dompc_factor.h"
#include "dompc_quad.h"
#include "dompc_node.h"
#include "dompc_riccati.h"
#include "dompc_forward.h"
#include "dompc_sweep.h"
#include "dompc_phases.h"
#include "dompc_driver.h"
}
```

do_mpc_amd/csrc/dompc_phases.h:

```cpp

template <bool FINE>
DOMPC_DEV inline double trial_edges(const Thr& T, const Prob& Q) {
  const KArgs& A = *Q.A;
  double f = 0.0;
  if (FINE && !DENSE_EDGE && M > 0) {
    constexpr int NPC = NI * DEG + 1;
    for (int it = T.tid; it < A.n_edges * NPC; it += T.nt) {
      const int e = it % A.n_edges, q = it / A.n_edges;
      const double fe = eval_edge_f_t<true>(Q, e, Q.xt, Q.st, Q.ct, q == 0 ? NI * DEG : q - 1);
      f += fe;
    }
  } else
  for (int e = T.tid; e < A.n_edges; e += T.nt) {
    const int m = mk_e(A, e);
    if (!m) continue;
    const double fe = DENSE_EDGE ? dae_edge_f(Q, e, Q.xt, Q.st, Q.ct) : eval_edge_f(Q, e, Q.xt, Q.st, Q.ct);
    if (sh_cnt(A, m)) f += fe;
  }
  for (int n = T.tid; n < A.n_nodes; n += T.nt)
    if (sh_cnt(A, mk_n(A, n))) f += node_rterm_f(Q, n, Q.xt);
  return f;
}
DOMPC_DEV inline void step_rules_pass(const Thr& T, const Prob& Q, double mu, double (&r5)[5]) {
  const KArgs& A = *Q.A;
  const int nX = A.n_opt_x, nSl = A.n_edges * NE;
  for (int i = 0; i < 5; ++i) r5[i] = 0.0;
  {
    double x_[DOMPC_FW], l_[DOMPC_FW], u2_[DOMPC_FW], d_[DOMPC_FW], gf_[DOMPC_FW], zl_[DOMPC_FW], zu_[DOMPC_FW];
#define L_(u, g) x_[u] = Q.x[g]; l_[u] = Q.lb[g]; u2_[u] = Q.ub[g]; d_[u] = Q.dx[g]; gf_[u] = Q.gf[g]; zl_[u] = Q.zl[g]; zu_[u] = Q.zu[g];
#define B_(u, g)                                                                               \
    if (sh_cnt(A, mk_x(A, g))) {                                                           \
      const double xv = x_[u], l = l_[u], ub_ = u2_[u], d = d_[u];                         \
      double gphi = gf_[u];                                                                \
      if (l > -INFINITY) {                                                                 \
        const double r = fast_rcp(xv - l);                                                 \
        r5[0] = fmax(r5[0], -d * r);                                \
        r5[1] = fmax(r5[1], 1.0 + r * d - mu * r * fast_rcp(zl_[u]));         \
        gphi -= mu * r;                                                                    \
      }                                                                                    \
      if (ub_ < INFINITY) {                                                                \
        const double r = fast_rcp(ub_ - xv);                                               \
        r5[0] = fmax(r5[0], d * r);                                                        \
        r5[1] = fmax(r5[1], 1.0 - r * d - mu * r * fast_rcp(zu_[u]));                      \
        gphi += mu * r;                                                                    \
      }                                                                                    \
      if (KAPPA_D != 0.0) gphi += KAPPA_D * mu * one_sided(l, ub_);                        \
      r5[2] += gphi * d;                                                                   \
    }
    DOMPC_FOR4(nX, L_, B_)
#undef L_
#undef B_
  }
  for (int g = T.tid; g < nSl; g += T.nt) {
    if (!sh_cnt(A, mk_e(A, g / NE1))) continue;
    const int si = (g / NE1) * NE1 + g % NE1;
    const double sv = Q.s[si], l = Q.sl[si], u = Q.su[si], d = Q.ds[si];
    double gphi = 0.0;
    if (l > -INFINITY) {
      const double r = fast_rcp(sv - l);
      r5[0] = fmax(r5[0], -d * r);
      r5[1] = fmax(r5[1], 1.0 + r * d - mu * r * fast_rcp(Q.zsl[si]));
      gphi -= mu * r;
    }
    if (u < INFINITY) {
      const double r = fast_rcp(u - sv);
      r5[0] = fmax(r5[0], d * r);
      r5[1] = fmax(r5[1], 1.0 - r * d - mu * r * fast_rcp(Q.zsu[si]));
      gphi += mu * r;
    }
    if (KAPPA_D != 0.0) gphi += KAPPA_D * mu * one_sided(l, u);
    r5[2] += gphi * d;
  }
  const int ops[5] = {R_MAX, R_MAX, R_SUM, R_SUM, R_SUM};
  wg_reduce(T, r5, ops);
}
template <bool FINE>
DOMPC_DEV inline void eval_trial_pass(const Thr& T, const Prob& Q, double al, double& obj_o, double& th_o, double& bar_o) {
  const KArgs& A = *Q.A;
  const int nX = A.n_opt_x, nSl = A.n_edges * NE;
  double r3[3] = {0.0, 0.0, 0.0};
  LogAcc La{1.0, 0, 0};
  double lin = 0.0;
  {
    double x_[DOMPC_FW], d_[DOMPC_FW], l_[DOMPC_FW], u2_[DOMPC_FW];
#define L_(u, g) x_[u] = Q.x[g]; d_[u] = Q.dx[g]; l_[u] = Q.lb[g]; u2_[u] = Q.ub[g];
#define B_(u, g)                                                                               \
    if (mk_x(A, g)) {                                                                      \
      const double xt_ = x_[u] + al * d_[u];                                               \
      Q.xt[g] = xt_;                                                                       \
      if (sh_cnt(A, mk_x(A, g))) {                                                         \
        if (l_[u] > -INFINITY) logacc_add(La, xt_ - l_[u]);                                \
        if (u2_[u] < INFINITY) logacc_add(La, u2_[u] - xt_);                               \
        if (KAPPA_D != 0.0) { const double os_ = one_sided(l_[u], u2_[u]); lin += os_ > 0.0 ? xt_ - l_[u] : (os_ < 0.0 ? u2_[u] - xt_ : 0.0); } \
      }                                                                                    \
    }
    DOMPC_FOR4(nX, L_, B_)
#undef L_
#undef B_
  }
  for (int g = T.tid; g < nSl; g += T.nt) {
    if (!mk_e(A, g / NE1)) continue;
    const int si = (g / NE1) * NE1 + g % NE1;
    Q.st[si] = Q.s[si] + al * Q.ds[si];
  }
  T.sync();
  for (int g = T.tid; g < NX; g += T.nt) Q.ct[g] = FREE_ROOT ? 0.0 : Q.xt[A.node_x_off[0] + g] - Q.P[g] / DOMPC_SX[g];
  if (FREE_ROOT && T.tid == 0) r3[0] += Q.sf * dompc_aterm_f(Q.xt + A.node_x_off[0], Q.P, Q.P + A.p_off_tvp, Q.P + A.p_off_p);
  r3[0] += trial_edges<FINE>(T, Q);
  T.sync();
  {
    double c_[DOMPC_FW];
#define L_(u, g) c_[u] = Q.ct[g];
#define B_(u, g) if (sh_cnt(A, mk_g(A, g))) r3[1] += fabs(c_[u]);
    DOMPC_FOR4(A.n_g, L_, B_)
#undef L_
#undef B_
  }
  for (int g = T.tid; g < nSl; g += T.nt) {
    if (!sh_cnt(A, mk_e(A, g / NE1))) continue;
    const int si = (g / NE1) * NE1 + g % NE1;
    if (Q.sl[si] > -INFINITY) logacc_add(La, Q.st[si] - Q.sl[si]);
    if (Q.su[si] < INFINITY) logacc_add(La, Q.su[si] - Q.st[si]);
    if (KAPPA_D != 0.0) { const double os_ = one_sided(Q.sl[si], Q.su[si]); lin += os_ > 0.0 ? Q.st[si] - Q.sl[si] : (os_ < 0.0 ? Q.su[si] - Q.st[si] : 0.0); }
  }
  r3[2] = -logacc_value(La);
  if (KAPPA_D != 0.0) r3[2] += KAPPA_D * lin;
  const int ops[3] = {R_SUM, R_SUM, R_SUM};
  wg_reduce(T, r3, ops);
  obj_o = r3[0]; th_o = r3[1]; bar_o = r3[2];
}
DOMPC_DEV inline Comp accept_pass(const Thr& T, const Prob& Q, double alpha, double a_z, double mu) {
  const KArgs& A = *Q.A;
  const int nX = A.n_opt_x, nSl = A.n_edges * NE;
  const double ks = 1e10;
  Comp Cp{-INFINITY, INFINITY, 0.0};
  {
    double xt_[DOMPC_FW], x_[DOMPC_FW], d_[DOMPC_FW], l_[DOMPC_FW], u2_[DOMPC_FW], zl_[DOMPC_FW], zu_[DOMPC_FW];
#define L_(u, g) xt_[u] = Q.xt[g]; x_[u] = Q.x[g]; d_[u] = Q.dx[g]; l_[u] = Q.lb[g]; u2_[u] = Q.ub[g]; zl_[u] = Q.zl[g]; zu_[u] = Q.zu[g];
#define B_(u, g)                                                                               \
    if (mk_x(A, g)) {                                                                        \
      const double xv = xt_[u], l = l_[u], ub_ = u2_[u];                                     \
      const bool cnt_ = sh_cnt(A, mk_x(A, g));                                               \
      Q.x[g] = xv;                                                                           \
      if (l > -INFINITY) {                                                                   \
        const double ro = fast_rcp(x_[u] - l);                       \
        const double z = zl_[u] + a_z * (mu * ro - zl_[u] - zl_[u] * ro * d_[u]);            \
        const double dd = xv - l, mr = mu * fast_rcp(dd);                                    \
        const double zn = fmax(fmin(z, ks * mr), mr * (1.0 / ks));                           \
        Q.zl[g] = zn;                                                                        \
        if (cnt_) comp_add(Cp, dd * zn, zn);                                                 \
      }                                                                                      \
      if (ub_ < INFINITY) {                                                                  \
        const double ro = fast_rcp(ub_ - x_[u]);                                             \
        const double z = zu_[u] + a_z * (mu * ro - zu_[u] + zu_[u] * ro * d_[u]);            \
        const double dd = ub_ - xv, mr = mu * fast_rcp(dd);                                  \
        const double zn = fmax(fmin(z, ks * mr), mr * (1.0 / ks));                           \
        Q.zu[g] = zn;                                                                        \
        if (cnt_) comp_add(Cp, dd * zn, zn);                                                 \
      }                                                                                      \
    }
    DOMPC_FOR4(nX, L_, B_)
#undef L_
#undef B_
  }
  for (int g = T.tid; g < nSl; g += T.nt) {
    if (!mk_e(A, g / NE1)) continue;
    const int si = (g / NE1) * NE1 + g % NE1;
    const double sv = Q.st[si], so = Q.s[si], dsv = Q.ds[si];
    const bool cnt_ = sh_cnt(A, mk_e(A, g / NE1));
    Q.s[si] = sv;
    const double l = Q.sl[si], u = Q.su[si];
    if (l > -INFINITY) {
      const double z = Q.zsl[si] + a_z * dz_lo(so, l, Q.zsl[si], dsv, mu);
      const double zn = fmax(fmin(z, ks * mu / (sv - l)), mu / (ks * (sv - l)));
      Q.zsl[si] = zn;
      if (cnt_) comp_add(Cp, (sv - l) * zn, zn);
    }
    if (u < INFINITY) {
      const double z = Q.zsu[si] + a_z * dz_up(so, u, Q.zsu[si], dsv, mu);
      const double zn = fmax(fmin(z, ks * mu / (u - sv)), mu / (ks * (u - sv)));
      Q.zsu[si] = zn;
      if (cnt_) comp_add(Cp, (u - sv) * zn, zn);
    }
  }
  {
    double y_[DOMPC_FW], dy_[DOMPC_FW];
#define L_(u, g) y_[u] = Q.lam[g]; dy_[u] = Q.dlam[g];
#define B_(u, g) if (mk_g(A, g)) Q.lam[g] = y_[u] + alpha * dy_[u];
    DOMPC_FOR4(A.n_g, L_, B_)
#undef L_
#undef B_
  }
  return Cp;
}
struct PhaseRet { unsigned gen, nred, xseq; int rc; };
struct PhaseRet3 { unsigned gen, nred, xseq; double v0, v1, v2; };
#ifndef DOMPC_HOST_EMU
#define DOMPC_PHASE_PROLOGUE                                                        \
  const KArgs A = kernel_args(kp);                                                  \
  Thr T = make_thr(A);                                                              \
  T.kp = kp;                                                                        \
  T.gen = ufl(gen); T.nred = ufl(nred); T.xseq = ufl(xseq);                         \
  Prob Q = make_prob(A, ufl(slot), A.p + (int64_t)ufl(b) * A.n_opt_p);              \
  Q.sf = ufl(sf);
__device__ __attribute__((noinline)) PhaseRet phase_sweep(const void* kp, int b, int slot, double sf, double mu, double dsw, int soc, unsigned gen, unsigned nred, unsigned xseq) {
  DOMPC_PHASE_PROLOGUE
  Q.soc = ufl(soc);
  prob_bounds(Q);
  Q.dsw = ufl(dsw);
  const int rc = sweep<false>(T, Q, ufl(mu));
  return PhaseRet{T.gen, T.nred, T.xseq, rc};
}
__device__ __attribute__((noinline)) PhaseRet phase_sweep_fine(const void* kp, int b, int slot, double sf, double mu, double dsw, int soc, unsigned gen, unsigned nred, unsigned xseq) {
  DOMPC_PHASE_PROLOGUE
  Q.soc = ufl(soc);
  prob_bounds(Q);
  Q.dsw = ufl(dsw);
  const int rc = sweep<true>(T, Q, ufl(mu));
  return PhaseRet{T.gen, T.nred, T.xseq, rc};
}
__device__ __attribute__((noinline)) PhaseRet phase_backward(const void* kp, int b, int slot, double sf, double mu, double delta, double dsw, int mode, unsigned gen, unsigned nred, unsigned xseq) {
  DOMPC_PHASE_PROLOGUE
  Q.dsw = ufl(dsw);
  Q.soc = ufl(mode);
  prob_bounds(Q);
  const int rc = riccati_backward(T, Q, ufl(mu), ufl(delta));
  return PhaseRet{T.gen, T.nred, T.xseq, rc};
}
__device__ __attribute__((noinline)) PhaseRet phase_forward(const void* kp, int b, int slot, double sf, double mu, double delta, double dsw, unsigned gen, unsigned nred, unsigned xseq) {
  DOMPC_PHASE_PROLOGUE
  Q.dsw = ufl(dsw);
  riccati_forward_t<false>(T, Q, ufl(mu), ufl(delta));
  return PhaseRet{T.gen, T.nred, T.xseq, 0};
}
__device__ __attribute__((noinline)) PhaseRet phase_forward_adj(const void* kp, int b, int slot, double sf, double mu, double delta, double dsw, unsigned gen, unsigned nred, unsigned xseq) {
  DOMPC_PHASE_PROLOGUE
  Q.dsw = ufl(dsw);
  riccati_forward_t<true>(T, Q, ufl(mu), ufl(delta));
  return PhaseRet{T.gen, T.nred, T.xseq, 0};
}
__device__ __attribute__((noinline)) PhaseRet3 phase_step_rules(const void* kp, int b, int slot, double sf, double mu, unsigned gen, unsigned nred, unsigned xseq) {
  DOMPC_PHASE_PROLOGUE
  double r5[5];
  step_rules_pass(T, Q, ufl(mu), r5);
  return PhaseRet3{T.gen, T.nred, T.xseq, r5[0], r5[1], r5[2]};
}
__device__ __attribute__((noinline)) PhaseRet3 phase_eval_trial(const void* kp, int b, int slot, double sf, double al, unsigned gen, unsigned nred, unsigned xseq) {
  DOMPC_PHASE_PROLOGUE
  double o = 0.0, th = 0.0, br = 0.0;
  eval_trial_pass<false>(T, Q, ufl(al), o, th, br);
  return PhaseRet3{T.gen, T.nred, T.xseq, o, th, br};
}
__device__ __attribute__((noinline)) PhaseRet3 phase_eval_trial_fine(const void* kp, int b, int slot, double sf, double al, unsigned gen, unsigned nred, unsigned xseq) {
  DOMPC_PHASE_PROLOGUE
  double o = 0.0, th = 0.0, br = 0.0;
  eval_trial_pass<true>(T, Q, ufl(al), o, th, br);
  return PhaseRet3{T.gen, T.nred, T.xseq, o, th, br};
}
__device__ __attribute__((noinline)) PhaseRet3 phase_accept(const void* kp, int b, int slot, double sf, double alpha, double a_z, double mu, unsigned gen, unsigned nred, unsigned xseq) {
  DOMPC_PHASE_PROLOGUE
  const Comp C = accept_pass(T, Q, ufl(alpha), ufl(a_z), ufl(mu));
  return PhaseRet3{T.gen, T.nred, T.xseq, C.smax, C.smin, C.sum_z};
}
#undef DOMPC_PHASE_PROLOGUE
#define DOMPC_PHASE_CALL(fn, ...)                                                   \
  const auto r_ = fn(T.kp, b, slot, Q.sf, __VA_ARGS__, T.gen, T.nred, T.xseq);            \
  T.gen = ufl(r_.gen); T.nred = ufl(r_.nred); T.xseq = ufl(r_.xseq);
#endif
#ifndef DOMPC_REPEAT_PHASE
#define DOMPC_REPEAT_PHASE 0
#endif
DOMPC_DEV inline int run_sweep(const Thr& T, Prob& Q, int b, int slot, double mu, int soc = 0, double dsw = 0.0) {
  Q.dsw = dsw;
  Q.lu_ok = lu_store_rule(*Q.A, mu, soc) ? 1 : 0;
  Q.rp_soc = soc; Q.rp_mu = mu;
#ifndef DOMPC_HOST_EMU
  if (fine_items(T, *Q.A)) { DOMPC_PHASE_CALL(phase_sweep_fine, mu, dsw, soc) return ufl(r_.rc); }
  if (DOMPC_REPEAT_PHASE & 1) { DOMPC_PHASE_CALL(phase_sweep, mu, dsw, soc) }
  DOMPC_PHASE_CALL(phase_sweep, mu, dsw, soc)
  return ufl(r_.rc);
#else
  (void)b; (void)slot;
  Q.soc = soc;
  prob_bounds(Q);
  const int rc = fine_items(T, *Q.A) ? sweep<true>(T, Q, mu) : sweep<false>(T, Q, mu);
  Q.soc = 0;
  prob_bounds(Q);
  return rc;
#endif
}
DOMPC_DEV inline int run_backward(const Thr& T, const Prob& Q, int b, int slot, double mu, double delta, int mode = 0) {
#ifndef DOMPC_HOST_EMU
  if (DOMPC_REPEAT_PHASE & 2) {
    { DOMPC_PHASE_CALL(phase_backward, mu, delta, Q.dsw, mode) }
    { DOMPC_PHASE_CALL(phase_sweep, Q.rp_mu, Q.dsw, Q.rp_soc) }
  }
  DOMPC_PHASE_CALL(phase_backward, mu, delta, Q.dsw, mode)
  return ufl(r_.rc);
#else
  (void)b; (void)slot;
  Prob Qm = Q;
  Qm.soc = mode;
  prob_bounds(Qm);
  return riccati_backward(T, Qm, mu, delta);
#endif
}
DOMPC_DEV inline void run_step_rules(const Thr& T, const Prob& Q, int b, int slot, double mu, double (&r5)[5]) {
#ifndef DOMPC_HOST_EMU
  if (DOMPC_REPEAT_PHASE & 16) { DOMPC_PHASE_CALL(phase_step_rules, mu) }
  DOMPC_PHASE_CALL(phase_step_rules, mu)
  r5[0] = ufl(r_.v0); r5[1] = ufl(r_.v1); r5[2] = ufl(r_.v2); r5[3] = 0.0; r5[4] = 0.0;
#else
  (void)b; (void)slot;
  step_rules_pass(T, Q, mu, r5);
#endif
}
DOMPC_DEV inline void run_eval_trial(const Thr& T, const Prob& Q, int b, int slot, double al, double& obj_o, double& th_o, double& bar_o) {
#ifndef DOMPC_HOST_EMU
  if (fine_items(T, *Q.A)) { DOMPC_PHASE_CALL(phase_eval_trial_fine, al) obj_o = ufl(r_.v0); th_o = ufl(r_.v1); bar_o = ufl(r_.v2); return; }
  if (DOMPC_REPEAT_PHASE & 8) { DOMPC_PHASE_CALL(phase_eval_trial, al) }
  DOMPC_PHASE_CALL(phase_eval_trial, al)
  obj_o = ufl(r_.v0); th_o = ufl(r_.v1); bar_o = ufl(r_.v2);
#else
  (void)b; (void)slot;
  if (fine_items(T, *Q.A)) eval_trial_pass<true>(T, Q, al, obj_o, th_o, bar_o); else eval_trial_pass<false>(T, Q, al, obj_o, th_o, bar_o);
#endif
}
DOMPC_DEV inline Comp run_accept(const Thr& T, const Prob& Q, int b, int slot, double alpha, double a_z, double mu) {
#ifndef DOMPC_HOST_EMU
  DOMPC_PHASE_CALL(phase_accept, alpha, a_z, mu)
  return Comp{r_.v0, r_.v1, r_.v2};
#else
  (void)b; (void)slot;
  return accept_pass(T, Q, alpha, a_z, mu);
#endif
}
DOMPC_DEV inline void run_forward(const Thr& T, const Prob& Q, int b, int slot, double mu, double delta) {
#ifndef DOMPC_HOST_EMU
  if (forward_adjoint(Q, mu)) {
    DOMPC_PHASE_CALL(phase_forward_adj, mu, delta, Q.dsw)
  } else {
    if (DOMPC_REPEAT_PHASE & 4) { DOMPC_PHASE_CALL(phase_forward, mu, delta, Q.dsw) }
    DOMPC_PHASE_CALL(phase_forward, mu, delta, Q.dsw)
  }
#else
  (void)b; (void)slot;
  if (forward_adjoint(Q, mu)) riccati_forward_t<true>(T, Q, mu, delta);
  else riccati_forward_t<false>(T, Q, mu, delta);
#endif
}
```

do_mpc_amd/csrc/dompc_quad.h:

```cpp
#if !defined(DOMPC_HOST_EMU) && DOMPC_DEG >= 1 && DOMPC_M >= 1 && DOMPC_NI == 1 && DOMPC_NX + DOMPC_NU + 2 <= 16 && DOMPC_DEG * DOMPC_DEG * DOMPC_NX <= 64

extern "C" __device__ double dompc_dpp_f64(double old, double src, int ctrl, int row_mask, int bank_mask, bool bound_ctrl) __asm("llvm.amdgcn.update.dpp.f64");
template <int L>
__device__ inline double rbc(double v) {
  static_assert(L >= 0 && L < 16, "lane inside a row of 16");
  return dompc_dpp_f64(0.0, v, 0x150 + L, 0xf, 0xf, true);
}
__device__ inline void pin(double& v) { asm volatile("" : "+v"(v)); }
__device__ inline void pin(int& v) { asm volatile("" : "+v"(v)); }
template <int L>
__device__ inline void fmac_rbc(double& d, const double& src, double mul) {
  asm volatile("v_fmac_f64_dpp %0, %1, %2 row_newbcast:%3 row_mask:0xf bank_mask:0xf" : "+v"(d) : "v"(src), "v"(mul), "n"(L));
}
template <class F, int... I>
__device__ inline void sfor_(F&& f, std::integer_sequence<int, I...>) { (f(std::integral_constant<int, I>{}), ...); }
template <int N, class F>
__device__ inline void sfor(F&& f) { sfor_(f, std::make_integer_sequence<int, (N > 0 ? N : 0)>{}); }

struct MoRef { int kind, off; };
constexpr MoRef moref_in(int d, const int* vidx, int nv, const int* cidx, int nc, int base) {
  for (int k = 0; k < nv; ++k) if (vidx[k] == d) return MoRef{2, base + k};
  for (int k = 0; k < nc; ++k) if (cidx[k] == d) return MoRef{1, k};
  return MoRef{0, 0};
}
// ... 111 lines not shown
#pragma unroll
    for (int jj = 0; jj < DEG; ++jj) {
      double xp = DOMPC_C[0 * (DEG + 1) + jj + 1] * xn;
#pragma unroll
      for (int r = 1; r <= DEG; ++r) xp += DOMPC_C[r * (DEG + 1) + jj + 1] * wv[r - 1];
      res[jj] = soc ? cin[jj] : fv[jj] - xp;
    }
    double xf = DOMPC_D[0] * xn;
#pragma unroll
    for (int r = 1; r <= DEG; ++r) xf += DOMPC_D[r] * wv[r - 1];
    rc = soc ? cinc : wv[M - 1] - xf;
    ce = soc ? cine : wv[M - 1] - xc;
  }
  double BGv[M], BBv[M], SGv[M], ZDv[M];
#pragma unroll
  for (int s = 0; s < M; ++s) {
    const double xv = wv[s], l = lbv[s], u = ubv[s];
    BGv[s] = bar_grad(xv, l, u, mu, !(Q.soc & 2));
    BBv[s] = bar_grad(xv, l, u, 1.0);
    SGv[s] = sigma_of(xv, l, u, zlv[s], zuv[s]);
    ZDv[s] = zuv[s] - zlv[s];
  }
#pragma unroll
  for (int s = 0; s < M; ++s) { pin(BGv[s]); pin(BBv[s]); pin(SGv[s]); pin(ZDv[s]); }
#pragma unroll
  for (int jj = 0; jj < DEG; ++jj) pin(res[jj]);
  pin(rc); pin(ce);
  double bc[DEG][R];
  sfor<DEG>([&](auto S_) {
    constexpr int s = S_;
    sfor<R>([&](auto R_) {
      constexpr int r = R_, jj = r / NX, a = r % NX;
      double v = 0.0;
      if constexpr (s == jj)
        sfor<NX>([&](auto B_) {
          constexpr int bb = B_;
          constexpr MoRef rf = moref_dyn(jj, NX + a * NA + bb);
          if constexpr (rf.kind != 0) { const double t_ = mo_dyn_val<rf.kind, rf.off>(rec); v = (j == bb) ? t_ : v; }
        });
      if constexpr (s == 0) {
        sfor<NU>([&](auto K_) {
          constexpr int ku = K_;
          constexpr MoRef rf = moref_dyn(jj, NX + a * NA + NX + ku);
          if constexpr (rf.kind != 0) { const double t_ = mo_dyn_val<rf.kind, rf.off>(rec); v = (j == NX + ku) ? t_ : v; }
        });
        const double rb_ = rbc<a>(res[jj]);
        v = (j == NA) ? rb_ : v;
      }
      v = (j == a) ? v - DOMPC_C[(s + 1) * (DEG + 1) + jj + 1] : v;
      bc[s][r] = v;
    });
  });
  QD_PH(5)
  QD_SB();
  double RWv[M], RDv[M], ry;
  {
    double tcol[M];
#pragma unroll
    for (int s = 0; s < M; ++s) tcol[s] = 0.0;
    double ryu = 0.0;
    sfor<DEG>([&](auto J_) {
      constexpr int jj = J_;
      sfor<NX>([&](auto A_) {
        constexpr int a = A_;
        const double la = rbc<a>(lam[jj]);
        tcol[jj] = fma(la, bc[jj][jj * NX + a], tcol[jj]);
        if constexpr (jj == 0) ryu = fma(la, bc[0][a], ryu);
        else ryu = fma(la, bc[0][jj * NX + a], ryu);
      });
    });
#pragma unroll
    for (int s = 0; s < DEG; ++s) {
      double t = tcol[s];
#pragma unroll
      for (int jj = 0; jj < DEG; ++jj)
        if (jj != s) t = fma(-DOMPC_C[(s + 1) * (DEG + 1) + jj + 1], lam[jj], t);
      tcol[s] = t - DOMPC_D[s + 1] * lamc;
    }
    tcol[M - 1] = lamc + nue;
    double ryx = -DOMPC_D[0] * lamc;
#pragma unroll
    for (int jj = 0; jj < DEG; ++jj) ryx = fma(-DOMPC_C[0 * (DEG + 1) + jj + 1], lam[jj], ryx);
    ry = isx ? ryx : ryu;
#pragma unroll
    for (int s = 0; s < M; ++s) { RWv[s] = tcol[s] + BGv[s]; RDv[s] = tcol[s] + ZDv[s]; }
#pragma unroll
    for (int s = 0; s < M; ++s) { pin(RWv[s]); pin(RDv[s]); }
    pin(ry);
    if (isx) {
      ldsd* Lv = Ld + QL_RW + g * QL_VG;
#pragma unroll
      for (int s = 0; s < M; ++s) { Lv[s * NX + (int)b] = RWv[s]; Lv[NW + s * NX + (int)b] = BBv[s]; }
    }
  }
  QD_PH(6)
  QD_SB();
  int bad = 0;
  double sig[DEG];
#pragma unroll
  for (int s = 0; s < DEG; ++s) sig[s] = 1.0;
  sfor<R>([&](auto K_) {
    constexpr int k = K_, sk = k / NX, bk = k % NX;
    constexpr int rt1 = (4 * (k / 4 + 1) < R) ? 4 * (k / 4 + 1) : R;
    QD_SB();
    const bool own = (j == bk);
    double m = 0.0;
#pragma unroll
    for (int r = k + 1; r < rt1; ++r) m = fmax(m, fabs(bc[sk][r]));
    const double akk = fabs(bc[sk][k]);
    bad |= (int)(own & !(akk >= GJ_U * m && akk > 1e-300));
    const double pl = fast_rcp((akk > 1e-300) ? bc[sk][k] : 1.0);
    const double pinv = rbc<bk>(pl);
    sig[sk] = own ? -pl : sig[sk];
    double pm[DEG];
#pragma unroll
    for (int s = 0; s < DEG; ++s) {
      const double prow = bc[s][k] * pinv;
      pm[s] = (s == sk && own) ? 0.0 : -prow;
      bc[s][k] = (s == sk && own) ? -1.0 : prow;
      pin(pm[s]);
    }
    asm volatile("s_nop 1");
    sfor<R>([&](auto R_) {
      constexpr int r = R_;
      if constexpr (r != k) {
        sfor<DEG>([&](auto S_) { constexpr int s = S_; if constexpr (s != sk) fmac_rbc<bk>(bc[s][r], bc[sk][r], pm[s]); });
        fmac_rbc<bk>(bc[sk][r], bc[sk][r], pm[sk]);
      }
    });
#pragma unroll
    for (int s = 0; s < DEG; ++s)
#pragma unroll
      for (int r = 0; r < R; ++r) pin(bc[s][r]);
  });
  QD_SB();
#pragma unroll
  for (int s = 0; s < DEG; ++s)
#pragma unroll
    for (int r = 0; r < R; ++r) bc[s][r] *= sig[s];
  QD_SB();
  if (__ballot(bad) != 0ull) return 2;
  QD_PH(2)
  QD_SB();
  if (st_x) {
    if (!soc) {
#pragma unroll
      for (int jj = 0; jj < DEG; ++jj) Q.c[pk.row0 + jj * NX + (int)b] = res[jj];
      Q.c[pk.row0 + R + (int)b] = rc;
      Q.c[pk.row0 + NW + (int)b] = ce;
    }
#pragma unroll
    for (int s = 0; s < M; ++s) {
      const int gi = pk.woff + s * NX + (int)b;
      Q.gf[gi] = 0.0;
      Q.rd[gi] = RDv[s];
    }
    double* ew = Q.ew + (int64_t)e * EW_SIZE;
    if (store_lu) {
#pragma unroll
      for (int s = 0; s < DEG; ++s)
#pragma unroll
        for (int r = 0; r < R; ++r) ew[EW_LU + r * LU_N + s * NX + (int)b] = bc[s][r];
    }
#pragma unroll
    for (int s = 0; s < M; ++s) {
      ew[EW_SIGW + s * NX + (int)b] = SGv[s] + Q.dsw;
      ew[EW_RW + s * NX + (int)b] = RWv[s];
    }
  }
  if (e0n >= 0) stage_quad(Q, e0n, lane, Ld, bank ^ 1);
  {
    const int en = (e0n >= 0 ? e0n : e0) + g;
    pkn = qd_pack(A, en < A.n_edges ? en : A.n_edges - 1, Q.sf);
  }
  double Wc[NW];
  {
#pragma unroll
    for (int r = 0; r < R; ++r) {
      double t = (isx ? DOMPC_C[0 * (DEG + 1) + 1] : -1.0) * bc[0][r];
#pragma unroll
      for (int s = 1; s < DEG; ++s) t = fma(isx ? DOMPC_C[0 * (DEG + 1) + s + 1] : 0.0, bc[s][r], t);
      Wc[r] = t;
    }
    sfor<NX>([&](auto A_) {
      constexpr int a = A_;
      const double rcb = rbc<a>(rc);
      double t = (j == NA) ? -rcb : ((j == a) ? DOMPC_D[0] : 0.0);
#pragma unroll
      for (int s = 1; s <= DEG; ++s) t = fma(DOMPC_D[s], Wc[(s - 1) * NX + a], t);
      Wc[R + a] = t;
    });
  }
#pragma unroll
  for (int r = 0; r < NW; ++r) pin(Wc[r]);
  double* S_ = Q.es + (int64_t)e * ES_SIZE;
  {
    double cv = 0.0;
    sfor<NX>([&](auto A_) {
      constexpr int a = A_;
      if (act && j < NA) S_[ES_AB + a * NA + j] = Wc[R + a];
      const double w0a = rbc<NA>(Wc[R + a]);
      cv = (j == a) ? w0a + ce : cv;
    });
    pin(cv);
    if (st_x) S_[ES_CV + (int)b] = cv;
  }
  QD_PH(7)
  QD_SB();
  double acc[NA];
#pragma unroll
  for (int i = 0; i < NA; ++i) acc[i] = 0.0;
  {
    const double ind = (j >= NA) ? 1.0 : 0.0;
    ldsd* Wb = Ld + QL_WB + g * QL_WBG;
    const ldsd* Lvec = Ld + QL_RW + g * QL_VG + (j == NA + 1 ? NW : 0);
    sfor<M>([&](auto P_) {
      constexpr int p = P_;
      __builtin_amdgcn_fence(__ATOMIC_ACQ_REL, "wavefront");
      __builtin_amdgcn_wave_barrier();
      if (j <= NA) {
#pragma unroll
        for (int k = 0; k < NX; ++k) Wb[k * QL_WS + j] = Wc[p * NX + k];
      }
      __builtin_amdgcn_fence(__ATOMIC_ACQ_REL, "wavefront");
      __builtin_amdgcn_wave_barrier();
      double Zc[NX], Tv[NA];
#pragma unroll
      for (int k = 0; k < NX; ++k) Zc[k] = (j <= NA) ? Wc[p * NX + k] : 0.0;
#pragma unroll
      for (int i = 0; i < NA; ++i) Tv[i] = 0.0;
      if constexpr (p < DEG) {
        sfor<NA>([&](auto I_) {
          constexpr int i = I_;
          sfor<NA - i>([&](auto D_) {
            constexpr int k = i + D_;
            constexpr MoRef rf = moref_dyn(p, MOH_H0 + symi(i, k, NA));
            if constexpr (rf.kind != 0) {
              const double h = mo_dyn_val<rf.kind, rf.off>(rec);
              if constexpr (k < NX) {
                Tv[i] = fma(h, Zc[k], Tv[i]);
                if constexpr (i != k) Tv[k] = fma(h, Zc[i], Tv[k]);
              } else {
                Tv[i] += (j == k) ? h : 0.0;
                if constexpr (i != k) {
                  if constexpr (i < NX) Tv[k] = fma(h, Zc[i], Tv[k]);
                  else Tv[k] += (j == i) ? h : 0.0;
                }
              }
            }
          });
        });
      }
      sfor<NX>([&](auto K_) {
        constexpr int k = K_;
        const double sg = rbc<k>(SGv[p]) + Q.dsw;
        Tv[k] = fma(sg, Zc[k], Tv[k]);
        Tv[k] = fma(ind, Lvec[p * NX + k], Tv[k]);
      });
      sfor<(NX + 1) / 2>([&](auto K2_) {
        constexpr int k0 = 2 * K2_;
        QD_SB();
        double wr[2][NA];
#pragma unroll
        for (int kk = 0; kk < 2; ++kk)
#pragma unroll
          for (int i = 0; i < NA; ++i) wr[kk][i] = (k0 + kk < NX) ? (double)Wb[(k0 + kk) * QL_WS + i] : 0.0;
#pragma unroll
        for (int kk = 0; kk < 2; ++kk)
          if (k0 + kk < NX) {
#pragma unroll
            for (int i = 0; i < NA; ++i) acc[i] = fma(wr[kk][i], Tv[k0 + kk], acc[i]);
          }
      });
      if constexpr (p < DEG) {
#pragma unroll
        for (int ku = 0; ku < NU; ++ku) acc[NX + ku] += Tv[NX + ku];
      }
#pragma unroll
      for (int i = 0; i < NA; ++i) asm volatile("" : "+v"(acc[i]));
      QD_SB();
    });
  }
  sfor<NA>([&](auto I_) {
    constexpr int i = I_;
    sfor<NA - i>([&](auto D_) {
      constexpr int k = i + D_;
      constexpr MoRef rf = moref_lt(1 + NA + symi(i, k, NA));
      if constexpr (rf.kind != 0) {
        const double h = omh * mo_lt_val<rf.kind, rf.off>(rec);
        acc[i] += (j == k) ? h : 0.0;
        if constexpr (i != k) acc[k] += (j == i) ? h : 0.0;
      }
    });
  });
  if constexpr (NE > 0) {
    sfor<NA>([&](auto I_) {
      constexpr int i = I_;
      sfor<NA - i>([&](auto D_) {
        constexpr int k = i + D_;
        constexpr MoRef rf = moref_nl(NE + NE * NA + symi(i, k, NA));
        if constexpr (rf.kind != 0) {
          const double h = mo_nl_val<rf.kind, rf.off>(rec);
          acc[i] += (j == k) ? h : 0.0;
          if constexpr (i != k) acc[k] += (j == i) ? h : 0.0;
        }
      });
    });
// ... 473 lines not shown
```

do_mpc_amd/csrc/dompc_runtime.cpp:

```cpp
#include <chrono>
#include <cstdio>
#include <cstdlib>
#include <cstring>
#include <dlfcn.h>
#include <cmath>
#include <string>
#include <thread>
#include <vector>

#include "dompc_kargs.h"

#ifndef DOMPC_HOST_EMU
#include <hip/hip_runtime.h>
#else
extern "C" void dompc_hostemu_model_info(const int32_t* in, int64_t* out, char* hash);
extern "C" void dompc_hostemu_run(const dompc::KArgs* A);
#endif

static thread_local std::string g_create_error;
static const int BATCH_ONE_WAVE = 4096;

struct dompc_handle {
  dompc_problem_desc d;
  std::string error;
// ... 310 lines not shown
    int32_t* in_d; int64_t* out_d; char* hash_d;
    if (dev_alloc(h, (void**)&in_d, sizeof(in_h)) || dev_alloc(h, (void**)&out_d, sizeof(info)) ||
        dev_alloc(h, (void**)&hash_d, sizeof(hash))) return 1;
    if (h2d(h, in_d, in_h, sizeof(in_h))) return 1;
    if (dev_zero(h, out_d, sizeof(info), h->stream)) return 1;
    struct { const int32_t* a; int64_t* b; char* c; } args = {in_d, out_d, hash_d};
    size_t sz = sizeof(args);
    void* cfg[] = {HIP_LAUNCH_PARAM_BUFFER_POINTER, &args, HIP_LAUNCH_PARAM_BUFFER_SIZE, &sz, HIP_LAUNCH_PARAM_END};
    if (hipModuleLaunchKernel(fn, 1, 1, 1, 64, 1, 1, 0, h->stream, nullptr, cfg) != hipSuccess) {
      h->error = "launch of dompc_model_info_kernel failed"; return 1;
    }
    if (d2h(h, info_o, out_d, sizeof(info)) || d2h(h, hash_o, hash_d, sizeof(hash)) || dev_sync(h)) return 1;
    return 0;
  };
  if (query_info(h->fn_info, info, hash)) return fail(1);
  if (h->fn_solve_batch) {
    int64_t info_b[20] = {0};
    char hash_b[64] = {0};
    hipFunction_t fn_info_b = nullptr;
    bool same = hipModuleGetFunction(&fn_info_b, h->module_batch, "dompc_model_info_kernel") == hipSuccess && !query_info(fn_info_b, info_b, hash_b);
    for (int i = 0; same && i < 20; ++i) same = info_b[i] == info[i];
    same = same && strncmp(hash, hash_b, 63) == 0;
    if (!same) {
      hipModuleUnload(h->module_batch);
      h->module_batch = nullptr;
      h->fn_solve_batch = nullptr;
      h->batch_object_stale = true;
      h->error.clear();
    }
  }
#else
  dompc_hostemu_model_info(in_h, info, hash);
#endif
  const int64_t want[9] = {d.nx, d.nu, d.np, d.ntvp, d.ne, d.ns, d.M == 0 ? 0 : d.deg, d.M == 0 ? 1 : d.ni, d.M};
  for (int i = 0; i < 9; ++i)
    if (info[i] != want[i]) {
      char buf[256];
      snprintf(buf, sizeof(buf), "code object was built for different model dimensions (field %d: %lld vs %lld)", i,
               (long long)info[i], (long long)want[i]);
      h->error = buf;
      return fail(1);
    }
  if (info[11] != (int64_t)sizeof(dompc::KArgs)) { h->error = "KArgs layout mismatch between runtime and code object"; return fail(1); }
  if (d.model_hash && strncmp(d.model_hash, hash, 63) != 0) {
    h->error = std::string("model hash mismatch: code object ") + hash + " vs description " + d.model_hash;
    return fail(1);
  }
  h->ws_stride = info[9];
  h->sweep_block = info[10];
  for (int i = 0; i < 4; ++i) h->xlayout[i] = info[12 + i];
  h->shard_capable = info[16] != 0;
  h->el_size = info[17];
  h->edges_per_wave = info[19] > 0 ? info[19] : 1;
  int max_batch = d.max_batch > 0 ? d.max_batch : 1;
  auto resident_at = [&](int block) -> int {
    int resident = 512 * (256 / block);
#ifndef DOMPC_HOST_EMU
    const int64_t per_wave = (int64_t)(block / 64) * h->el_size, red = h->xlayout[0] * (int64_t)block;
    const size_t lds = sizeof(double) * (size_t)(per_wave > red ? per_wave : red);
    int occ = 0, cus = 0;
    if (hipModuleOccupancyMaxActiveBlocksPerMultiprocessor(&occ, h->fn_solve, block, lds) == hipSuccess &&
        hipDeviceGetAttribute(&cus, hipDeviceAttributeMultiprocessorCount, d.device) == hipSuccess && occ > 0 && cus > 0)
      resident = occ * cus;
    h->occupancy = occ;
#endif
    return resident;
  };
  h->slots64 = resident_at(64);
  h->slots256 = resident_at(fit_block(h, 256));
  {
    const int resident = h->block_auto ? (max_batch >= BATCH_ONE_WAVE ? h->slots64 : h->slots256) : resident_at(h->block);
    h->n_slots = d.n_slots > 0 ? d.n_slots : (max_batch < resident ? max_batch : resident);
  }
  if (const char* se = getenv("DOMPC_SLOTS")) { const int v = atoi(se); if (v >= 1) h->n_slots = v; }
  if (h->n_slots < 1) h->n_slots = 1;
#ifdef DOMPC_HOST_EMU
  h->n_slots = 1;
#endif
  dompc::KArgs& A = h->base;
  memset(&A, 0, sizeof(A));
  int rc = 0;
  rc |= upload(h, &A.level_node_start, d.level_node_start, d.N + 2);
  rc |= upload(h, &A.node_level, d.node_level, d.n_nodes);
  rc |= upload(h, &A.node_x_off, d.node_x_off, d.n_nodes);
  rc |= upload(h, &A.node_u_off, d.node_u_off, d.n_nodes);
  rc |= upload(h, &A.node_eps_off, d.node_eps_off, d.n_nodes);
  rc |= upload(h, &A.node_child_start, d.node_child_start, d.n_nodes);
  rc |= upload(h, &A.node_child_count, d.node_child_count, d.n_nodes);
  rc |= upload(h, &A.node_parent, d.node_parent, d.n_nodes);
  rc |= upload(h, &A.node_in_edge, d.node_in_edge, d.n_nodes);
  rc |= upload(h, &A.edge_parent, d.edge_parent, d.n_edges);
  rc |= upload(h, &A.edge_child, d.edge_child, d.n_edges);
  rc |= upload(h, &A.edge_pidx, d.edge_pidx, d.n_edges);
  rc |= upload(h, &A.edge_w_off, d.edge_w_off, d.n_edges);
  rc |= upload(h, &A.edge_row0, d.edge_row0, d.n_edges);
  rc |= upload(h, &A.edge_level, d.edge_level, d.n_edges);
  rc |= upload(h, &A.edge_omega, d.edge_omega, d.n_edges);
  rc |= upload(h, &A.dummy_idx, d.dummy_idx, d.n_dummy);
  if (rc) return fail(1);
  {
    std::vector<int32_t> pack((size_t)d.n_edges * dompc::EP_N, 0);
    for (int e = 0; e < d.n_edges; ++e) {
      int32_t* q = pack.data() + (size_t)e * dompc::EP_N;
      const int n = d.edge_parent[e], cn = d.edge_child[e];
      q[dompc::EP_PARENT] = n; q[dompc::EP_CHILD] = cn; q[dompc::EP_LEVEL] = d.edge_level[e]; q[dompc::EP_WOFF] = d.edge_w_off[e];
      q[dompc::EP_PIDX] = d.edge_pidx[e]; q[dompc::EP_ROW0] = d.edge_row0[e];
      q[dompc::EP_XOFF_PARENT] = d.node_x_off[n]; q[dompc::EP_UOFF_PARENT] = d.node_u_off[n]; q[dompc::EP_XOFF_CHILD] = d.node_x_off[cn];
      q[dompc::EP_EPSOFF_PARENT] = d.node_eps_off ? d.node_eps_off[n] : -1;
      int64_t ob;
      memcpy(&ob, &d.edge_omega[e], sizeof ob);
      q[dompc::EP_OMEGA_LO] = (int32_t)(uint32_t)(ob & 0xffffffffll); q[dompc::EP_OMEGA_HI] = (int32_t)(uint32_t)((uint64_t)ob >> 32);
    }
    if (upload(h, &A.edge_pack, pack.data(), pack.size())) return fail(1);
  }
  A.N = d.N; A.n_nodes = d.n_nodes; A.n_edges = d.n_edges; A.n_dummy = d.n_dummy;
  A.n_opt_x = d.n_opt_x; A.n_opt_p = d.n_opt_p; A.n_g = d.n_g; A.e_pad = h->e_pad;
  A.p_off_tvp = d.p_off_tvp; A.p_off_p = d.p_off_p; A.p_off_uprev = d.p_off_uprev;
  {
    const int32_t* ls = desc->level_node_start;
    const int S = ls[d.N + 1] - ls[d.N];
    h->n_leaves = S > 0 ? S : 1;
    int cl = d.N;
    for (int k = d.N - 1; k >= 0; --k) {
      bool ok = (ls[k + 1] - ls[k]) == S;
      for (int s = 0; ok && s < S; ++s) {
        const int n = ls[k] + s;
        ok = desc->node_child_count[n] == 1 && desc->edge_child[desc->node_child_start[n]] == ls[k + 1] + s &&
             desc->node_child_start[n] == desc->node_child_start[ls[k]] + s;
      }
      if (!ok) break;
      cl = k;
    }
    A.chain_level = cl;
  }
  A.opt = d.opts;
  if (const char* mi = getenv("DOMPC_MAX_ITER")) A.opt.max_iter = atoi(mi);
  if (const char* lf = getenv("DOMPC_LDS_FILL")) {
    double v = 0.0; int lo = 0, hi = 1 << 30;
    sscanf(lf, "%lf,%d,%d", &v, &lo, &hi);
    A.lds_fill = v; A.lds_fill_lo = lo; A.lds_fill_hi = hi;
  }
  A.n_slots = h->n_slots;
  A.ws_stride = h->ws_stride;
#ifndef DOMPC_HOST_EMU
  {
    void* dw = nullptr;
    if (hipHostGetDevicePointer(&dw, h->abort_word, 0) != hipSuccess) { h->error = "hipHostGetDevicePointer failed"; return fail(1); }
    A.abort_flag = (const int32_t*)dw;
  }
#else
  A.abort_flag = h->abort_word;
#endif
  if (dev_alloc(h, (void**)&A.ws, sizeof(double) * (size_t)h->ws_stride * h->n_slots)) return fail(1);
#ifndef DOMPC_HOST_EMU
  if (const char* fill = getenv("DOMPC_WS_FILL")) {
    if (hipMemset(A.ws, atoi(fill), sizeof(double) * (size_t)h->ws_stride * h->n_slots) != hipSuccess) { h->error = "hipMemset failed"; return fail(1); }
  }
#endif
  if (dev_alloc(h, (void**)&A.work_counter, 64)) return fail(1);
  A.lb_sh = A.ub_sh = nullptr;
  {
    const char* sb = getenv("DOMPC_SHARED_BOUNDS");
    if (!sb || atoi(sb) != 0) {
      if (dev_alloc(h, (void**)&A.lb_sh, sizeof(double) * (size_t)d.n_opt_x)) return fail(1);
      if (dev_alloc(h, (void**)&A.ub_sh, sizeof(double) * (size_t)d.n_opt_x)) return fail(1);
    }
  }
  if (dev_alloc(h, (void**)&A.wide_bar, sizeof(uint32_t) * dompc::WIDE_BAR_STRIDE * 64)) return fail(1);
  if (dev_alloc(h, (void**)&A.wide_flags, sizeof(int32_t) * 8 * 64)) return fail(1);
  if (dev_alloc(h, (void**)&A.wide_partials, sizeof(double) * 64 * 2 * 32 * 12)) return fail(1);
  for (int i = 0; i < 8; ++i)
    if (dev_alloc(h, (void**)&h->s_dbg[i], sizeof(double) * (size_t)(d.n_opt_x > d.n_g ? d.n_opt_x : d.n_g))) return fail(1);
  if (dev_alloc(h, (void**)&h->s_trace, sizeof(double) * 8 * h->trace_cap)) return fail(1);
  A.trace = h->s_trace; A.trace_cap = h->trace_cap;
  if (const char* xt = getenv("DOMPC_EXTRA_TRAFFIC")) A.trace_pad = atoi(xt);
  if (dev_sync(h)) return fail(1);
  h->d.level_node_start = nullptr;
  *out = h;
  return 0;
}

extern "C" int64_t dompc_workspace_bytes(const dompc_handle* h) { return h ? (int64_t)sizeof(double) * h->ws_stride * h->n_slots : 0; }
extern "C" int32_t dompc_num_slots(const dompc_handle* h) { return h ? h->n_slots : 0; }
extern "C" int64_t dompc_sweep_block_doubles(const dompc_handle* h) { return h ? h->sweep_block : 0; }

extern "C" int64_t dompc_exchange_doubles(const dompc_handle* h, int32_t world, int32_t n_cut) {
  if (!h || world < 1 || n_cut < 0) return 0;
  const int64_t* L = h->xlayout;
  return (int64_t)world * L[0] + (int64_t)n_cut * (L[1] + L[2] + L[3]) + 2 * (int64_t)world;
}

#ifndef DOMPC_HOST_EMU
static int rccl_open(dompc_handle* h, const char* path) {
  if (h->rccl_lib) return 0;
  h->rccl_lib = dlopen(path && *path ? path : "librccl.so", RTLD_NOW | RTLD_GLOBAL);
  if (!h->rccl_lib) { h->error = std::string("dlopen(librccl) failed: ") + dlerror(); return 1; }
  h->nccl_get_unique_id = (int (*)(dompc_handle::RcclUid*))dlsym(h->rccl_lib, "ncclGetUniqueId");
  h->nccl_comm_init_rank = (int (*)(void**, int, dompc_handle::RcclUid, int))dlsym(h->rccl_lib, "ncclCommInitRank");
  h->nccl_all_reduce = (int (*)(const void*, void*, size_t, int, int, void*, hipStream_t))dlsym(h->rccl_lib, "ncclAllReduce");
  h->nccl_comm_destroy = (int (*)(void*))dlsym(h->rccl_lib, "ncclCommDestroy");
  h->nccl_error_string = (const char* (*)(int))dlsym(h->rccl_lib, "ncclGetErrorString");
  if (!h->nccl_get_unique_id || !h->nccl_comm_init_rank || !h->nccl_all_reduce || !h->nccl_comm_destroy) {
    h->error = "librccl does not export the expected nccl* entry points"; return 1;
  }
  return 0;
}
#define NCCLCHK(h, expr)                                                                                       \
  do {                                                                                                         \
    const int _r = (expr);                                                                                     \
    if (_r != 0) {                                                                                             \
      (h)->error = std::string(#expr) + ": " + ((h)->nccl_error_string ? (h)->nccl_error_string(_r) : "rccl error"); \
      return 1;                                                                                                \
    }                                                                                                          \
  } while (0)
#endif

extern "C" int dompc_rccl_unique_id(dompc_handle* h, const char* librccl_path, uint8_t id[128]) {
  if (!h || !id) return 1;
#ifndef DOMPC_HOST_EMU
  if (rccl_open(h, librccl_path)) return 1;
  dompc_handle::RcclUid u;
  NCCLCHK(h, h->nccl_get_unique_id(&u));
  memcpy(id, u.internal, 128);
  return 0;
#else
  (void)librccl_path; h->error = "no RCCL in the host emulation"; return 1;
#endif
}

extern "C" int dompc_rccl_init(dompc_handle* h, const char* librccl_path, const uint8_t id[128], int32_t rank, int32_t world) {
  if (!h || !id) return 1;
#ifndef DOMPC_HOST_EMU
  if (rccl_open(h, librccl_path)) return 1;
  HIPCHK(h, hipSetDevice(h->d.device));
  if (h->rccl_comm) { h->nccl_comm_destroy(h->rccl_comm); h->rccl_comm = nullptr; }
  dompc_handle::RcclUid u;
  memcpy(u.internal, id, 128);
  NCCLCHK(h, h->nccl_comm_init_rank(&h->rccl_comm, world, u, rank));
  if (!h->rccl_stream) HIPCHK(h, hipStreamCreateWithFlags(&h->rccl_stream, hipStreamNonBlocking));
  return 0;
#else
  (void)librccl_path; (void)rank; (void)world; h->error = "no RCCL in the host emulation"; return 1;
#endif
}

extern "C" int dompc_set_sharding(dompc_handle* h, const dompc_shard_desc* s) {
  if (!h) return 1;
  dompc::KArgs& A = h->base;
  if (!s) {
    A.x_mask = A.g_mask = A.e_mask = A.n_mask = nullptr; A.node_cut = nullptr;
    A.n_cut = 0; A.cut_level = 0; A.shard_rank = 0; A.shard_world = 1; A.xbuf = nullptr; A.xbuf_len = 0;
    A.x_callback = nullptr; A.x_ctx = nullptr;
    h->sharded = false;
    return 0;
  }
  const dompc_problem_desc& d = h->d;
  if (!h->shard_capable) { h->error = "this code object was built without tree-sharding support (-DDOMPC_SHARD=1)"; return 1; }
  if (s->world < 1 || s->rank < 0 || s->rank >= s->world || s->cut_level < 1 || s->n_cut < 1) { h->error = "invalid shard description"; return 1; }
  if (!s->x_mask || !s->g_mask || !s->edge_mask || !s->node_mask || !s->node_cut || !s->xbuf) { h->error = "null pointer in shard description"; return 1; }
#ifndef DOMPC_HOST_EMU
  if (!s->allreduce && !h->rccl_comm) { h->error = "no collective: pass allreduce or call dompc_rccl_init first"; return 1; }
#else
  if (!s->allreduce) { h->error = "the host emulation needs an allreduce callback"; return 1; }
#endif
#ifndef DOMPC_HOST_EMU
  HIPCHK(h, hipSetDevice(d.device));
#endif
  if (s->xbuf_doubles < dompc_exchange_doubles(h, s->world, s->n_cut)) { h->error = "exchange buffer too small (dompc_exchange_doubles)"; return 1; }
  int rc = 0;
  rc |= upload(h, &A.x_mask, s->x_mask, d.n_opt_x);
  rc |= upload(h, &A.g_mask, s->g_mask, d.n_g);
  rc |= upload(h, &A.e_mask, s->edge_mask, d.n_edges);
  rc |= upload(h, &A.n_mask, s->node_mask, d.n_nodes);
  rc |= upload(h, &A.node_cut, s->node_cut, d.n_nodes);
  if (rc) return 1;
  A.n_cut = s->n_cut; A.cut_level = s->cut_level; A.shard_rank = s->rank; A.shard_world = s->world;
  A.xbuf = s->xbuf; A.xbuf_len = (int32_t)dompc_exchange_doubles(h, s->world, s->n_cut);
  h->allreduce = s->allreduce; h->allreduce_ctx = s->ctx;
#ifndef DOMPC_HOST_EMU
  if (!h->x_words) {
    HIPCHK(h, hipHostMalloc((void**)&h->x_words, 64, hipHostMallocMapped));
    memset(h->x_words, 0, 64);
  }
  if (!h->shard_stream) {
    int least = 0, greatest = 0;
    HIPCHK(h, hipDeviceGetStreamPriorityRange(&least, &greatest));
    HIPCHK(h, hipStreamCreateWithPriority(&h->shard_stream, hipStreamNonBlocking, least));
  }
  void* dw = nullptr;
  HIPCHK(h, hipHostGetDevicePointer(&dw, h->x_words, 0));
  A.x_req = (volatile uint32_t*)dw; A.x_ack = (volatile uint32_t*)dw + 1; A.x_count = (volatile uint32_t*)dw + 2;
  A.x_callback = nullptr; A.x_ctx = nullptr;
#else
  A.x_callback = s->allreduce; A.x_ctx = s->ctx;
#endif
  if (dev_sync(h)) return 1;
  h->sharded = true;
  return 0;
}

#ifndef DOMPC_HOST_EMU
static int serve_exchanges(dompc_handle* h, hipStream_t st) {
  hipEvent_t done;
  HIPCHK(h, hipEventCreateWithFlags(&done, hipEventDisableTiming));
  HIPCHK(h, hipEventRecord(done, st));
  volatile uint32_t* w = h->x_words;
  uint32_t served = 0;
  int rc = 0;
  const auto t0 = std::chrono::steady_clock::now();
  bool raised = false;
  unsigned polls = 0;
// ... 290 lines not shown
```

Before: 10550.

## Compute trial duals in line search and ping-pong iterate buffers instead of copying

The bound-multiplier update and complementarity reduction move from the accept pass into the trial evaluation pass, which already loads x, dx and the bounds. The accepted trial point is then adopted by swapping pointers between current and trial buffers (a parity bit in the slot index) rather than copying xt into x. The accept pass now only updates lambda. The per-element gf zeroing in the factor and quad kernels is moved to initialization. The cost is extra dual computation on every rejected trial and new workspace arrays for the trial duals.

```diff
diff --git a/do_mpc_amd/csrc/dompc_driver.h b/do_mpc_amd/csrc/dompc_driver.h
--- a/do_mpc_amd/csrc/dompc_driver.h
+++ b/do_mpc_amd/csrc/dompc_driver.h
@@ -79,6 +79,7 @@
     if (hl) xv = fmax(xv, l + pl);
     if (hu) xv = fmin(xv, u - pu);
     Q.lb_own[g] = l; Q.ub_own[g] = u; Q.x[g] = xv;
+    Q.gf[g] = 0.0;
     Q.zl[g] = hl ? 1.0 : 0.0; Q.zu[g] = hu ? 1.0 : 0.0;
     if (sh_cnt(A, mk_x(A, g))) cnt[0] += (hl ? 1.0 : 0.0) + (hu ? 1.0 : 0.0);
   }
@@ -92,6 +93,7 @@
     Q.lb_own[g] = -INFINITY; Q.ub_own[g] = INFINITY; Q.zl[g] = 0.0; Q.zu[g] = 0.0;
   }
   T.sync();
+  for (int g = T.tid; g < nX; g += T.nt) { Q.xt[g] = Q.x[g]; Q.zl_t[g] = Q.zl[g]; Q.zu_t[g] = Q.zu[g]; }
   if (A.lb_sh) {
     for (int g = T.tid; g < nX; g += T.nt) { A.lb_sh[g] = Q.lb_own[g]; A.ub_sh[g] = Q.ub_own[g]; }
     T.sync();
@@ -115,6 +117,7 @@
         if (hu) sv = fmin(sv, u - pu);
         Q.s[si] = sv; Q.sl[si] = l; Q.su[si] = u;
         Q.zsl[si] = hl ? 1.0 : 0.0; Q.zsu[si] = hu ? 1.0 : 0.0;
+        Q.st[si] = sv; Q.zsl_t[si] = Q.zsl[si]; Q.zsu_t[si] = Q.zsu[si];
         if (!rescale && sh_cnt(A, mk_e(A, e))) cnt[1] += (hl ? 1.0 : 0.0) + (hu ? 1.0 : 0.0);
       }
     }
@@ -429,8 +432,9 @@
     else if (dphi < 0.0) a_min = gamma_alpha * fmin(gamma_theta, gamma_phi * theta / (-dphi));
     else a_min = gamma_alpha * gamma_theta;
     a_min = fmax(a_min, 1e-14);
-    auto eval_trial = [&](double al, double& obj_o, double& th_o, double& bar_o) {
-      run_eval_trial(T, Q, b, slot, al, obj_o, th_o, bar_o);
+    Comp Cp_t{-INFINITY, INFINITY, 0.0};
+    auto eval_trial = [&](double al, double az, double& obj_o, double& th_o, double& bar_o) {
+      run_eval_trial(T, Q, b, slot, al, az, mu, obj_o, th_o, bar_o, Cp_t);
       ++n_trials;
     };
     auto acceptable_ref = [&](double th_, double ph_, double al, bool& armijo_case, double theta, double phi, double dphi) -> bool {
@@ -483,7 +487,7 @@
       wd_theta = theta; wd_phi = phi; wd_dphi = dphi; wd_alpha = a_max;
     }
     if (in_wd) {
-      eval_trial(alpha, obj_t, th_t, bar_t);
+      eval_trial(alpha, a_z, obj_t, th_t, bar_t);
       bool armijo_case = false;
       if (acceptable_ref(th_t, obj_t + mu * bar_t, wd_alpha, armijo_case, wd_theta, wd_phi, wd_dphi)) {
         accepted = true; armijo_used = armijo_case; wd_done = true; wd_augment_ref = true;
@@ -499,7 +503,7 @@
       }
     }
     while (!wd_done) {
-      eval_trial(alpha, obj_t, th_t, bar_t);
+      eval_trial(alpha, a_z, obj_t, th_t, bar_t);
       stale = false;
       bool armijo_case = false;
       if (acceptable(th_t, obj_t + mu * bar_t, alpha, armijo_case)) { accepted = true; armijo_used = armijo_case; break; }
@@ -517,13 +521,14 @@
           double q5[5];
           step_rules(q5);
           const double a_s = (q5[0] > tau) ? tau / q5[0] : 1.0;
+          const double a_zs = (q5[1] > tau) ? tau / q5[1] : 1.0;
           double obj_s = 0.0, th_s = 0.0, bar_s = 0.0;
-          eval_trial(a_s, obj_s, th_s, bar_s);
+          eval_trial(a_s, a_zs, obj_s, th_s, bar_s);
           bool arm_s = false;
           if (acceptable(th_s, obj_s + mu * bar_s, a_s, arm_s)) {
             accepted = true; armijo_used = arm_s; soc_ok = true;
             alpha = a_s;
-            a_z = (q5[1] > tau) ? tau / q5[1] : 1.0;
+            a_z = a_zs;
             obj_t = obj_s; th_t = th_s; bar_t = bar_s;
             break;
           }
@@ -540,7 +545,7 @@
       ++n_ls;
     }
     if (bad) { if (in_wd) { bad = 0; wd_resume = true; in_wd = false; wd_count = 0; continue; } status = 3; break; }
-    if (!accepted && stale) eval_trial(alpha, obj_t, th_t, bar_t);
+    if (!accepted && stale) eval_trial(alpha, a_z, obj_t, th_t, bar_t);
     if (!wd_done) wd_count = n_ls > 0 ? wd_count + 1 : 0;
     if (!accepted) {
       ++n_ls_fail;
@@ -557,7 +562,9 @@
     bar_sum = bar_t;
     c_ls += prof_clock() - c_t; g_ls += T.gen - g_t;
     c_t = prof_clock(); g_t = T.gen;
-    const Comp Cp = run_accept(T, Q, b, slot, alpha, a_z, mu);
+    run_accept(T, Q, b, slot, alpha);
+    flip_iterate(Q);
+    const Comp Cp = Cp_t;
     if (A.trace && b == 0 && T.tid == 0 && it < A.trace_cap) {
       double* tr = A.trace + 8 * it;
       tr[0] = it; tr[1] = mu; tr[2] = E0; tr[3] = E.e_p; tr[4] = E.e_d; tr[5] = accepted ? alpha : -alpha;
@@ -616,7 +623,7 @@
   Prob Q = make_prob(A, slot, A.p + (int64_t)b * A.n_opt_p);
   const int nX = A.n_opt_x;
   for (int g = T.tid; g < nX; g += T.nt) {
-    Q.x[g] = A.x0[g]; Q.lb[g] = A.lbx[g]; Q.ub[g] = A.ubx[g];
+    Q.x[g] = A.x0[g]; Q.lb[g] = A.lbx[g]; Q.ub[g] = A.ubx[g]; Q.gf[g] = 0.0;
     Q.zl[g] = A.dbg_zl[g]; Q.zu[g] = A.dbg_zu[g];
   }
   for (int r = T.tid; r < A.n_g; r += T.nt) Q.lam[r] = A.dbg_lam[r];
@@ -674,7 +681,7 @@
   const double* xin = A.sw_x + (int64_t)b * nX;
   const double* lin = A.sw_lam + (int64_t)b * A.n_g;
   for (int g = T.tid; g < nX; g += T.nt) {
-    Q.x[g] = xin[g]; Q.lb[g] = -INFINITY; Q.ub[g] = INFINITY; Q.zl[g] = 0.0; Q.zu[g] = 0.0;
+    Q.x[g] = xin[g]; Q.lb[g] = -INFINITY; Q.ub[g] = INFINITY; Q.zl[g] = 0.0; Q.zu[g] = 0.0; Q.gf[g] = 0.0;
   }
   for (int r = T.tid; r < A.n_g; r += T.nt) Q.lam[r] = lin[r];
   for (int g = T.tid; g < A.n_edges * NE; g += T.nt) {
diff --git a/do_mpc_amd/csrc/dompc_factor.h b/do_mpc_amd/csrc/dompc_factor.h
--- a/do_mpc_amd/csrc/dompc_factor.h
+++ b/do_mpc_amd/csrc/dompc_factor.h
@@ -446,7 +446,6 @@
         t -= DOMPC_D[cx / NX + 1] * Ld[EL_T0 + R + cx % NX];
         const int gi = woff + cx;
         const double xv = vx[q][0], l = vx[q][1], u = vx[q][2], zl_ = vx[q][3], zu_ = vx[q][4];
-        Q.gf[gi] = 0.0;
         Q.rd[gi] = t - zl_ + zu_;
         Ld[EL_RW + cx] = t + bar_grad(xv, l, u, mu, !(Q.soc & 2));
         Ld[EL_BB + cx] = bar_grad(xv, l, u, 1.0);
@@ -463,7 +462,6 @@
       double xv, l, u, zl_, zu_;
       if (GS > 1) { xv = ex[0]; l = ex[1]; u = ex[2]; zl_ = ex[3]; zu_ = ex[4]; }
       else { xv = Q.x[gi]; l = Q.lb[gi]; u = Q.ub[gi]; zl_ = Q.zl[gi]; zu_ = Q.zu[gi]; }
-      Q.gf[gi] = 0.0;
       Q.rd[gi] = t - zl_ + zu_;
       Ld[EL_RW + col] = t + bar_grad(xv, l, u, mu, !(Q.soc & 2));
       Ld[EL_BB + col] = bar_grad(xv, l, u, 1.0);
@@ -882,7 +880,7 @@
 #pragma unroll
       for (int q = 0; q < G_WPL; ++q) {
         const int col = lane + q * GS;
-        if (col < NW) { Q.gf[woff + col] = 0.0; Q.rd[woff + col] = gp_x[q]; }
+        if (col < NW) Q.rd[woff + col] = gp_x[q];
       }
       if (!Q.soc) {
 #pragma unroll
diff --git a/do_mpc_amd/csrc/dompc_kernel.h b/do_mpc_amd/csrc/dompc_kernel.h
--- a/do_mpc_amd/csrc/dompc_kernel.h
+++ b/do_mpc_amd/csrc/dompc_kernel.h
@@ -145,6 +145,7 @@
   int64_t s, zsl, zsu, sl, su, ds, st, ds_sv;
   int64_t ew, es, nd, mo, gsc, total;
   int64_t x_wd, zl_wd, zu_wd, lam_wd, s_wd, zsl_wd, zsu_wd, dlam_e, sgn;
+  int64_t zl_t, zu_t, zsl_t, zsu_t;
 };
 
 DOMPC_HD inline WsLayout ws_layout(int n_opt_x, int n_g, int n_edges, int e_pad, int n_nodes) {
@@ -167,6 +168,7 @@
   L.s_wd = take(nsl); L.zsl_wd = take(nsl); L.zsu_wd = take(nsl);
   L.dlam_e = take(EPS_GLOBAL ? n_g : 0);
   L.sgn = take(nsl);
+  L.zl_t = take(n_opt_x); L.zu_t = take(n_opt_x); L.zsl_t = take(nsl); L.zsu_t = take(nsl);
   o += 256;
   L.total = o;
   return L;
@@ -504,6 +506,7 @@
   double *s, *zsl, *zsu, *sl, *su, *ds, *st, *ds_sv;
   double *ew, *es, *nd, *mo, *gsc;
   double *x_wd, *zl_wd, *zu_wd, *lam_wd, *s_wd, *zsl_wd, *zsu_wd, *dlam_e, *sgn;
+  double *zl_t, *zu_t, *zsl_t, *zsu_t;
   int e_pad;
   double sf;
   double mu;
@@ -518,17 +521,23 @@
   DOMPC_DEV double* MO(int e) const { return mo + (int64_t)e * MO_REC; }
 };
 
+constexpr int PAR_BIT = 1 << 30;
 DOMPC_DEV inline Prob make_prob(const KArgs& A, int slot, const double* P) {
   WsLayout L = ws_layout(A.n_opt_x, A.n_g, A.n_edges, A.e_pad, A.n_nodes);
-  double* w = A.ws + (int64_t)slot * A.ws_stride;
+  double* w = A.ws + (int64_t)(slot & (PAR_BIT - 1)) * A.ws_stride;
+  const bool odd = (slot & PAR_BIT) != 0;
   Prob p;
   p.A = &A; p.P = P;
-  p.x = w + L.x; p.zl = w + L.zl; p.zu = w + L.zu; p.lb_own = w + L.lb; p.ub_own = w + L.ub; p.dx = w + L.dx;
+  p.x = w + (odd ? L.xt : L.x); p.zl = w + (odd ? L.zl_t : L.zl); p.zu = w + (odd ? L.zu_t : L.zu);
+  p.xt = w + (odd ? L.x : L.xt); p.zl_t = w + (odd ? L.zl : L.zl_t); p.zu_t = w + (odd ? L.zu : L.zu_t);
+  p.lb_own = w + L.lb; p.ub_own = w + L.ub; p.dx = w + L.dx;
   p.lb = A.lb_sh ? A.lb_sh : p.lb_own; p.ub = A.ub_sh ? A.ub_sh : p.ub_own;
-  p.gf = w + L.gf; p.rd = w + L.rd; p.xt = w + L.xt; p.dx_sv = w + L.dx_sv;
+  p.gf = w + L.gf; p.rd = w + L.rd; p.dx_sv = w + L.dx_sv;
   p.lam = w + L.lam; p.dlam = w + L.dlam; p.c = w + L.c; p.ct = w + L.ct; p.dlam_sv = w + L.dlam_sv;
-  p.s = w + L.s; p.zsl = w + L.zsl; p.zsu = w + L.zsu; p.sl = w + L.sl; p.su = w + L.su;
-  p.ds = w + L.ds; p.st = w + L.st; p.ds_sv = w + L.ds_sv;
+  p.s = w + (odd ? L.st : L.s); p.zsl = w + (odd ? L.zsl_t : L.zsl); p.zsu = w + (odd ? L.zsu_t : L.zsu);
+  p.st = w + (odd ? L.s : L.st); p.zsl_t = w + (odd ? L.zsl : L.zsl_t); p.zsu_t = w + (odd ? L.zsu : L.zsu_t);
+  p.sl = w + L.sl; p.su = w + L.su;
+  p.ds = w + L.ds; p.ds_sv = w + L.ds_sv;
   p.ew = w + L.ew; p.es = w + L.es; p.nd = w + L.nd; p.mo = w + L.mo; p.gsc = w + L.gsc;
   p.x_wd = w + L.x_wd; p.zl_wd = w + L.zl_wd; p.zu_wd = w + L.zu_wd; p.lam_wd = w + L.lam_wd;
   p.s_wd = w + L.s_wd; p.zsl_wd = w + L.zsl_wd; p.zsu_wd = w + L.zsu_wd; p.dlam_e = w + L.dlam_e; p.sgn = w + L.sgn;
@@ -540,6 +549,17 @@
   const bool own = (Q.soc & 2) != 0 || !A.lb_sh;
   Q.lb = own ? Q.lb_own : A.lb_sh;
   Q.ub = own ? Q.ub_own : A.ub_sh;
+}
+
+DOMPC_DEV inline void flip_iterate(Prob& Q) {
+  double* t;
+  t = Q.x; Q.x = Q.xt; Q.xt = t;
+  t = Q.zl; Q.zl = Q.zl_t; Q.zl_t = t;
+  t = Q.zu; Q.zu = Q.zu_t; Q.zu_t = t;
+  t = Q.s; Q.s = Q.st; Q.st = t;
+  t = Q.zsl; Q.zsl = Q.zsl_t; Q.zsl_t = t;
+  t = Q.zsu; Q.zsu = Q.zsu_t; Q.zsu_t = t;
+  Q.slot ^= PAR_BIT;
 }
 
 DOMPC_DEV constexpr int slot_of(int i, int r) { return i == 0 ? r - 1 : DEG + (i - 1) * (DEG + 1) + r; }
diff --git a/do_mpc_amd/csrc/dompc_phases.h b/do_mpc_amd/csrc/dompc_phases.h
--- a/do_mpc_amd/csrc/dompc_phases.h
+++ b/do_mpc_amd/csrc/dompc_phases.h
@@ -75,23 +75,43 @@
   wg_reduce(T, r5, ops);
 }
 template <bool FINE>
-DOMPC_DEV inline void eval_trial_pass(const Thr& T, const Prob& Q, double al, double& obj_o, double& th_o, double& bar_o) {
+DOMPC_DEV inline void eval_trial_pass(const Thr& T, const Prob& Q, double al, double a_z, double mu, double& obj_o, double& th_o, double& bar_o, Comp& Cp) {
   const KArgs& A = *Q.A;
   const int nX = A.n_opt_x, nSl = A.n_edges * NE;
+  const double ks = 1e10;
   double r3[3] = {0.0, 0.0, 0.0};
   LogAcc La{1.0, 0, 0};
   double lin = 0.0;
+  Cp = Comp{-INFINITY, INFINITY, 0.0};
   {
-    double x_[DOMPC_FW], d_[DOMPC_FW], l_[DOMPC_FW], u2_[DOMPC_FW];
-#define L_(u, g) x_[u] = Q.x[g]; d_[u] = Q.dx[g]; l_[u] = Q.lb[g]; u2_[u] = Q.ub[g];
+    double x_[DOMPC_FW], d_[DOMPC_FW], l_[DOMPC_FW], u2_[DOMPC_FW], zl_[DOMPC_FW], zu_[DOMPC_FW];
+#define L_(u, g) x_[u] = Q.x[g]; d_[u] = Q.dx[g]; l_[u] = Q.lb[g]; u2_[u] = Q.ub[g]; zl_[u] = Q.zl[g]; zu_[u] = Q.zu[g];
 #define B_(u, g)                                                                               \
     if (mk_x(A, g)) {                                                                      \
       const double xt_ = x_[u] + al * d_[u];                                               \
+      const double l = l_[u], ub_ = u2_[u];                                                \
+      const bool cnt_ = sh_cnt(A, mk_x(A, g));                                             \
       Q.xt[g] = xt_;                                                                       \
-      if (sh_cnt(A, mk_x(A, g))) {                                                         \
-        if (l_[u] > -INFINITY) logacc_add(La, xt_ - l_[u]);                                \
-        if (u2_[u] < INFINITY) logacc_add(La, u2_[u] - xt_);                               \
-        if (KAPPA_D != 0.0) { const double os_ = one_sided(l_[u], u2_[u]); lin += os_ > 0.0 ? xt_ - l_[u] : (os_ < 0.0 ? u2_[u] - xt_ : 0.0); } \
+      if (cnt_) {                                                                          \
+        if (l > -INFINITY) logacc_add(La, xt_ - l);                                        \
+        if (ub_ < INFINITY) logacc_add(La, ub_ - xt_);                                     \
+        if (KAPPA_D != 0.0) { const double os_ = one_sided(l, ub_); lin += os_ > 0.0 ? xt_ - l : (os_ < 0.0 ? ub_ - xt_ : 0.0); } \
+      }                                                                                    \
+      if (l > -INFINITY) {                                                                 \
+        const double ro = fast_rcp(x_[u] - l);                       \
+        const double z = zl_[u] + a_z * (mu * ro - zl_[u] - zl_[u] * ro * d_[u]);          \
+        const double dd = xt_ - l, mr = mu * fast_rcp(dd);                                 \
+        const double zn = fmax(fmin(z, ks * mr), mr * (1.0 / ks));                         \
+        Q.zl_t[g] = zn;                                                                    \
+        if (cnt_) comp_add(Cp, dd * zn, zn);                                               \
+      }                                                                                    \
+      if (ub_ < INFINITY) {                                                                \
+        const double ro = fast_rcp(ub_ - x_[u]);                                           \
+        const double z = zu_[u] + a_z * (mu * ro - zu_[u] + zu_[u] * ro * d_[u]);          \
+        const double dd = ub_ - xt_, mr = mu * fast_rcp(dd);                               \
+        const double zn = fmax(fmin(z, ks * mr), mr * (1.0 / ks));                         \
+        Q.zu_t[g] = zn;                                                                    \
+        if (cnt_) comp_add(Cp, dd * zn, zn);                                               \
       }                                                                                    \
     }
     DOMPC_FOR4(nX, L_, B_)
@@ -101,7 +121,23 @@
   for (int g = T.tid; g < nSl; g += T.nt) {
     if (!mk_e(A, g / NE1)) continue;
     const int si = (g / NE1) * NE1 + g % NE1;
-    Q.st[si] = Q.s[si] + al * Q.ds[si];
+    const double so = Q.s[si], dsv = Q.ds[si];
+    const double sv = so + al * dsv;
+    const bool cnt_ = sh_cnt(A, mk_e(A, g / NE1));
+    Q.st[si] = sv;
+    const double l = Q.sl[si], u = Q.su[si];
+    if (l > -INFINITY) {
+      const double z = Q.zsl[si] + a_z * dz_lo(so, l, Q.zsl[si], dsv, mu);
+      const double zn = fmax(fmin(z, ks * mu / (sv - l)), mu / (ks * (sv - l)));
+      Q.zsl_t[si] = zn;
+      if (cnt_) comp_add(Cp, (sv - l) * zn, zn);
+    }
+    if (u < INFINITY) {
+      const double z = Q.zsu[si] + a_z * dz_up(so, u, Q.zsu[si], dsv, mu);
+      const double zn = fmax(fmin(z, ks * mu / (u - sv)), mu / (ks * (u - sv)));
+      Q.zsu_t[si] = zn;
+      if (cnt_) comp_add(Cp, (u - sv) * zn, zn);
+    }
   }
   T.sync();
   for (int g = T.tid; g < NX; g += T.nt) Q.ct[g] = FREE_ROOT ? 0.0 : Q.xt[A.node_x_off[0] + g] - Q.P[g] / DOMPC_SX[g];
@@ -129,72 +165,18 @@
   wg_reduce(T, r3, ops);
   obj_o = r3[0]; th_o = r3[1]; bar_o = r3[2];
 }
-DOMPC_DEV inline Comp accept_pass(const Thr& T, const Prob& Q, double alpha, double a_z, double mu) {
+DOMPC_DEV inline void accept_pass(const Thr& T, const Prob& Q, double alpha) {
   const KArgs& A = *Q.A;
-  const int nX = A.n_opt_x, nSl = A.n_edges * NE;
-  const double ks = 1e10;
-  Comp Cp{-INFINITY, INFINITY, 0.0};
-  {
-    double xt_[DOMPC_FW], x_[DOMPC_FW], d_[DOMPC_FW], l_[DOMPC_FW], u2_[DOMPC_FW], zl_[DOMPC_FW], zu_[DOMPC_FW];
-#define L_(u, g) xt_[u] = Q.xt[g]; x_[u] = Q.x[g]; d_[u] = Q.dx[g]; l_[u] = Q.lb[g]; u2_[u] = Q.ub[g]; zl_[u] = Q.zl[g]; zu_[u] = Q.zu[g];
-#define B_(u, g)                                                                               \
-    if (mk_x(A, g)) {                                                                        \
-      const double xv = xt_[u], l = l_[u], ub_ = u2_[u];                                     \
-      const bool cnt_ = sh_cnt(A, mk_x(A, g));                                               \
-      Q.x[g] = xv;                                                                           \
-      if (l > -INFINITY) {                                                                   \
-        const double ro = fast_rcp(x_[u] - l);                       \
-        const double z = zl_[u] + a_z * (mu * ro - zl_[u] - zl_[u] * ro * d_[u]);            \
-        const double dd = xv - l, mr = mu * fast_rcp(dd);                                    \
-        const double zn = fmax(fmin(z, ks * mr), mr * (1.0 / ks));                           \
-        Q.zl[g] = zn;                                                                        \
-        if (cnt_) comp_add(Cp, dd * zn, zn);                                                 \
-      }                                                                                      \
-      if (ub_ < INFINITY) {                                                                  \
-        const double ro = fast_rcp(ub_ - x_[u]);                                             \
-        const double z = zu_[u] + a_z * (mu * ro - zu_[u] + zu_[u] * ro * d_[u]);            \
-        const double dd = ub_ - xv, mr = mu * fast_rcp(dd);                                  \
-        const double zn = fmax(fmin(z, ks * mr), mr * (1.0 / ks));                           \
-        Q.zu[g] = zn;                                                                        \
-        if (cnt_) comp_add(Cp, dd * zn, zn);                                                 \
-      }                                                                                      \
-    }
-    DOMPC_FOR4(nX, L_, B_)
+  double y_[DOMPC_FW], dy_[DOMPC_FW];
+#define L_(u, g) y_[u] = Q.lam[g]; dy_[u] = Q.dlam[g];
+#define B_(u, g) if (mk_g(A, g)) Q.lam[g] = y_[u] + alpha * dy_[u];
+  DOMPC_FOR4(A.n_g, L_, B_)
 #undef L_
 #undef B_
-  }
-  for (int g = T.tid; g < nSl; g += T.nt) {
-    if (!mk_e(A, g / NE1)) continue;
-    const int si = (g / NE1) * NE1 + g % NE1;
-    const double sv = Q.st[si], so = Q.s[si], dsv = Q.ds[si];
-    const bool cnt_ = sh_cnt(A, mk_e(A, g / NE1));
-    Q.s[si] = sv;
-    const double l = Q.sl[si], u = Q.su[si];
-    if (l > -INFINITY) {
-      const double z = Q.zsl[si] + a_z * dz_lo(so, l, Q.zsl[si], dsv, mu);
-      const double zn = fmax(fmin(z, ks * mu / (sv - l)), mu / (ks * (sv - l)));
-      Q.zsl[si] = zn;
-      if (cnt_) comp_add(Cp, (sv - l) * zn, zn);
-    }
-    if (u < INFINITY) {
-      const double z = Q.zsu[si] + a_z * dz_up(so, u, Q.zsu[si], dsv, mu);
-      const double zn = fmax(fmin(z, ks * mu / (u - sv)), mu / (ks * (u - sv)));
-      Q.zsu[si] = zn;
-      if (cnt_) comp_add(Cp, (u - sv) * zn, zn);
-    }
-  }
-  {
-    double y_[DOMPC_FW], dy_[DOMPC_FW];
-#define L_(u, g) y_[u] = Q.lam[g]; dy_[u] = Q.dlam[g];
-#define B_(u, g) if (mk_g(A, g)) Q.lam[g] = y_[u] + alpha * dy_[u];
-    DOMPC_FOR4(A.n_g, L_, B_)
-#undef L_
-#undef B_
-  }
-  return Cp;
 }
 struct PhaseRet { unsigned gen, nred, xseq; int rc; };
 struct PhaseRet3 { unsigned gen, nred, xseq; double v0, v1, v2; };
+struct PhaseRet6 { unsigned gen, nred, xseq; double v0, v1, v2, c0, c1, c2; };
 #ifndef DOMPC_HOST_EMU
 #define DOMPC_PHASE_PROLOGUE                                                        \
   const KArgs A = kernel_args(kp);                                                  \
@@ -245,26 +227,28 @@
   step_rules_pass(T, Q, ufl(mu), r5);
   return PhaseRet3{T.gen, T.nred, T.xseq, r5[0], r5[1], r5[2]};
 }
-__device__ __attribute__((noinline)) PhaseRet3 phase_eval_trial(const void* kp, int b, int slot, double sf, double al, unsigned gen, unsigned nred, unsigned xseq) {
+__device__ __attribute__((noinline)) PhaseRet6 phase_eval_trial(const void* kp, int b, int slot, double sf, double al, double a_z, double mu, unsigned gen, unsigned nred, unsigned xseq) {
   DOMPC_PHASE_PROLOGUE
   double o = 0.0, th = 0.0, br = 0.0;
-  eval_trial_pass<false>(T, Q, ufl(al), o, th, br);
-  return PhaseRet3{T.gen, T.nred, T.xseq, o, th, br};
-}
-__device__ __attribute__((noinline)) PhaseRet3 phase_eval_trial_fine(const void* kp, int b, int slot, double sf, double al, unsigned gen, unsigned nred, unsigned xseq) {
+  Comp C;
+  eval_trial_pass<false>(T, Q, ufl(al), ufl(a_z), ufl(mu), o, th, br, C);
+  return PhaseRet6{T.gen, T.nred, T.xseq, o, th, br, C.smax, C.smin, C.sum_z};
+}
+__device__ __attribute__((noinline)) PhaseRet6 phase_eval_trial_fine(const void* kp, int b, int slot, double sf, double al, double a_z, double mu, unsigned gen, unsigned nred, unsigned xseq) {
   DOMPC_PHASE_PROLOGUE
   double o = 0.0, th = 0.0, br = 0.0;
-  eval_trial_pass<true>(T, Q, ufl(al), o, th, br);
-  return PhaseRet3{T.gen, T.nred, T.xseq, o, th, br};
-}
-__device__ __attribute__((noinline)) PhaseRet3 phase_accept(const void* kp, int b, int slot, double sf, double alpha, double a_z, double mu, unsigned gen, unsigned nred, unsigned xseq) {
-  DOMPC_PHASE_PROLOGUE
-  const Comp C = accept_pass(T, Q, ufl(alpha), ufl(a_z), ufl(mu));
-  return PhaseRet3{T.gen, T.nred, T.xseq, C.smax, C.smin, C.sum_z};
+  Comp C;
+  eval_trial_pass<true>(T, Q, ufl(al), ufl(a_z), ufl(mu), o, th, br, C);
+  return PhaseRet6{T.gen, T.nred, T.xseq, o, th, br, C.smax, C.smin, C.sum_z};
+}
+__device__ __attribute__((noinline)) PhaseRet phase_accept(const void* kp, int b, int slot, double sf, double alpha, unsigned gen, unsigned nred, unsigned xseq) {
+  DOMPC_PHASE_PROLOGUE
+  accept_pass(T, Q, ufl(alpha));
+  return PhaseRet{T.gen, T.nred, T.xseq, 0};
 }
 #undef DOMPC_PHASE_PROLOGUE
 #define DOMPC_PHASE_CALL(fn, ...)                                                   \
-  const auto r_ = fn(T.kp, b, slot, Q.sf, __VA_ARGS__, T.gen, T.nred, T.xseq);            \
+  const auto r_ = fn(T.kp, b, Q.slot, Q.sf, __VA_ARGS__, T.gen, T.nred, T.xseq);          \
   T.gen = ufl(r_.gen); T.nred = ufl(r_.nred); T.xseq = ufl(r_.xseq);
 #endif
 #ifndef DOMPC_REPEAT_PHASE
@@ -315,24 +299,23 @@
   step_rules_pass(T, Q, mu, r5);
 #endif
 }
-DOMPC_DEV inline void run_eval_trial(const Thr& T, const Prob& Q, int b, int slot, double al, double& obj_o, double& th_o, double& bar_o) {
-#ifndef DOMPC_HOST_EMU
-  if (fine_items(T, *Q.A)) { DOMPC_PHASE_CALL(phase_eval_trial_fine, al) obj_o = ufl(r_.v0); th_o = ufl(r_.v1); bar_o = ufl(r_.v2); return; }
-  if (DOMPC_REPEAT_PHASE & 8) { DOMPC_PHASE_CALL(phase_eval_trial, al) }
-  DOMPC_PHASE_CALL(phase_eval_trial, al)
-  obj_o = ufl(r_.v0); th_o = ufl(r_.v1); bar_o = ufl(r_.v2);
-#else
-  (void)b; (void)slot;
-  if (fine_items(T, *Q.A)) eval_trial_pass<true>(T, Q, al, obj_o, th_o, bar_o); else eval_trial_pass<false>(T, Q, al, obj_o, th_o, bar_o);
-#endif
-}
-DOMPC_DEV inline Comp run_accept(const Thr& T, const Prob& Q, int b, int slot, double alpha, double a_z, double mu) {
-#ifndef DOMPC_HOST_EMU
-  DOMPC_PHASE_CALL(phase_accept, alpha, a_z, mu)
-  return Comp{r_.v0, r_.v1, r_.v2};
-#else
-  (void)b; (void)slot;
-  return accept_pass(T, Q, alpha, a_z, mu);
+DOMPC_DEV inline void run_eval_trial(const Thr& T, const Prob& Q, int b, int slot, double al, double a_z, double mu, double& obj_o, double& th_o, double& bar_o, Comp& Cp) {
+#ifndef DOMPC_HOST_EMU
+  if (fine_items(T, *Q.A)) { DOMPC_PHASE_CALL(phase_eval_trial_fine, al, a_z, mu) obj_o = ufl(r_.v0); th_o = ufl(r_.v1); bar_o = ufl(r_.v2); Cp = Comp{r_.c0, r_.c1, r_.c2}; return; }
+  if (DOMPC_REPEAT_PHASE & 8) { DOMPC_PHASE_CALL(phase_eval_trial, al, a_z, mu) }
+  DOMPC_PHASE_CALL(phase_eval_trial, al, a_z, mu)
+  obj_o = ufl(r_.v0); th_o = ufl(r_.v1); bar_o = ufl(r_.v2); Cp = Comp{r_.c0, r_.c1, r_.c2};
+#else
+  (void)b; (void)slot;
+  if (fine_items(T, *Q.A)) eval_trial_pass<true>(T, Q, al, a_z, mu, obj_o, th_o, bar_o, Cp); else eval_trial_pass<false>(T, Q, al, a_z, mu, obj_o, th_o, bar_o, Cp);
+#endif
+}
+DOMPC_DEV inline void run_accept(const Thr& T, const Prob& Q, int b, int slot, double alpha) {
+#ifndef DOMPC_HOST_EMU
+  DOMPC_PHASE_CALL(phase_accept, alpha)
+#else
+  (void)b; (void)slot;
+  accept_pass(T, Q, alpha);
 #endif
 }
 DOMPC_DEV inline void run_forward(const Thr& T, const Prob& Q, int b, int slot, double mu, double delta) {
diff --git a/do_mpc_amd/csrc/dompc_quad.h b/do_mpc_amd/csrc/dompc_quad.h
--- a/do_mpc_amd/csrc/dompc_quad.h
+++ b/do_mpc_amd/csrc/dompc_quad.h
@@ -287,7 +287,6 @@
 #pragma unroll
     for (int s = 0; s < M; ++s) {
       const int gi = pk.woff + s * NX + (int)b;
-      Q.gf[gi] = 0.0;
       Q.rd[gi] = RDv[s];
     }
     double* ew = Q.ew + (int64_t)e * EW_SIZE;
diff --git a/do_mpc_amd/csrc/dompc_runtime.cpp b/do_mpc_amd/csrc/dompc_runtime.cpp
--- a/do_mpc_amd/csrc/dompc_runtime.cpp
+++ b/do_mpc_amd/csrc/dompc_runtime.cpp
@@ -486,11 +486,13 @@
   A.abort_flag = h->abort_word;
 #endif
   if (dev_alloc(h, (void**)&A.ws, sizeof(double) * (size_t)h->ws_stride * h->n_slots)) return fail(1);
-#ifndef DOMPC_HOST_EMU
   if (const char* fill = getenv("DOMPC_WS_FILL")) {
+#ifndef DOMPC_HOST_EMU
     if (hipMemset(A.ws, atoi(fill), sizeof(double) * (size_t)h->ws_stride * h->n_slots) != hipSuccess) { h->error = "hipMemset failed"; return fail(1); }
-  }
-#endif
+#else
+    memset(A.ws, atoi(fill), sizeof(double) * (size_t)h->ws_stride * h->n_slots);
+#endif
+  }
   if (dev_alloc(h, (void**)&A.work_counter, 64)) return fail(1);
   A.lb_sh = A.ub_sh = nullptr;
   {
```

Result: slower. 10440 (-1.0%).
